# GAMES-UChile/mogptk

Hardware: AMD Instinct MI355X
Metric: log-marginal-likelihood+grad evals/sec, MOSM C=4 N=8192; 1/2/4/8 GPU (higher is better)
Workload: dtype f64

## Files before the change

### mogptk_amd/csrc/exact.hip

```cpp
#include "mogp_model.h"
#include <cstdlib>
#include <limits>

using namespace mogp;

static int wait_stream(hipStream_t st) {
    static const bool spin = !(std::getenv("MOGP_SPIN_WAIT") && std::atoi(std::getenv("MOGP_SPIN_WAIT")) == 0);
    if (!spin) { HIP_TRY(hipStreamSynchronize(st)); return 0; }
    for (;;) {
        const hipError_t e = hipStreamQuery(st);
        if (e == hipSuccess) return 0;
        if (e != hipErrorNotReady) return hip_fail(e, "hipStreamQuery", __FILE__, __LINE__);
    }
}

static hipEvent_t prof_event(mogp_model* m, int idx) {
    if (!m->profiling) return nullptr;
    while ((int)m->ev.size() <= idx) { hipEvent_t e; if (hipEventCreate(&e) != hipSuccess) return nullptr; m->ev.push_back(e); }
    return m->ev[idx];
}

static void kinv_block_ranges(mogp_model* m) {
    std::vector<int> blk;
    tile_blocks(m->sx.off, m->C, blk);
    const int nblk = (int)blk.size() / 2, D = m->D;
    m->blk_cen.assign((size_t)D * nblk, 0.0); m->blk_half.assign((size_t)D * nblk, 0.0);
    for (int b = 0; b < nblk; ++b)
        for (int d = 0; d < D; ++d) {
            const double* x = m->sx.xs.data() + (size_t)d * m->sx.Mpad + blk[2 * b];
            double lo = x[0], hi = x[0];
            for (int i = 1; i < blk[2 * b + 1]; ++i) { lo = std::fmin(lo, x[i]); hi = std::fmax(hi, x[i]); }
            m->blk_cen[(size_t)d * nblk + b] = 0.5 * (lo + hi); m->blk_half[(size_t)d * nblk + b] = 0.5 * (hi - lo);
        }
}

static int kinv_plan(mogp_model* m, bool want) {
    static const bool full = std::getenv("MOGP_FULL_INVERSE") && std::atoi(std::getenv("MOGP_FULL_INVERSE")) != 0;
    m->kinv_sparse = false; m->kinv_fraction = 1.0;
    if (!want || full || m->sh_n > 1 || m->tiles.empty() || m->radial) return 0;
    const int nb = m->nb, D = m->D, T = m->T, W = m->Wt;
    const int64_t ld = m->Npad;
    if (m->blk_cen.empty()) kinv_block_ranges(m);
    const int nblk = (int)(m->blk_cen.size() / std::max(D, 1));
    std::vector<char> need((size_t)nb * nb, 0);
    for (const GTile& t : m->tiles) {
        const double* tab = m->table.data() + (size_t)t.pair * T * W;
        bool read = false;
        for (int k = 0; k < T && !read; ++k) {
            const double* row = tab + (size_t)k * W;
            double emin = 0.0;
            for (int d = 0; d < D; ++d) {
                const double sd = (m->blk_cen[(size_t)d * nblk + t.rb] - m->blk_cen[(size_t)d * nblk + t.cb]) + row[2 + 2 * D + d];
                const double mu = std::fmax(0.0, std::fabs(sd) - m->blk_half[(size_t)d * nblk + t.rb] - m->blk_half[(size_t)d * nblk + t.cb]);
                emin += row[2 + d] * mu * mu;
            }
            read = !(0.5 * emin > 52.0);
        }
        if (!read) continue;
        const int i0 = t.r0 / MOGP_TILE, i1 = (t.r0 + t.nr - 1) / MOGP_TILE, j0 = t.c0 / MOGP_TILE, j1 = (t.c0 + t.nc - 1) / MOGP_TILE;
        for (int i = i0; i <= i1; ++i) for (int j = j0; j <= j1; ++j) if (j <= i) need[(size_t)i * nb + j] = 1;
    }
    for (int i = 0; i < nb; ++i) need[(size_t)i * nb + i] = 1;
    std::vector<GemmTask> acc, lau;
    std::vector<int> prefix(nb + 1, 0);
    for (int i = 0; i < nb; ++i) {
        for (int j = 0; j <= i; ++j) {
            if (!need[(size_t)i * nb + j]) continue;
            GemmTask a;
            a.a_off = (int64_t)i * MOGP_TILE; a.b_off = (int64_t)j * MOGP_TILE; a.c_off = (int64_t)i * MOGP_TILE * ld + (int64_t)j * MOGP_TILE;
            a.kt = 4 * MOGP_TILE / 16; a.pad = i + 1;
            acc.push_back(a);
            GemmTask l;
            l.a_off = (int64_t)i * MOGP_TILE * ld + (int64_t)i * MOGP_TILE; l.b_off = (int64_t)i * MOGP_TILE * ld + (int64_t)j * MOGP_TILE;
            l.c_off = a.c_off; l.kt = (int)((ld - (int64_t)i * MOGP_TILE) / 16); l.pad = 0;
            lau.push_back(l);
        }
        prefix[i + 1] = (int)acc.size();
    }
    const double frac = (double)acc.size() / ((double)nb * (nb + 1) / 2);
    m->kinv_fraction = frac;
    if (frac > 0.85) return 0;
    const bool same = acc.size() == m->kinv_acc_tasks.size() && (acc.empty() || std::memcmp(acc.data(), m->kinv_acc_tasks.data(), acc.size() * sizeof(GemmTask)) == 0);
    if (!same || m->d_kinv_acc.n < acc.size()) {
        int rc;
        if ((rc = m->d_kinv_acc.ensure(std::max<size_t>(acc.size(), 1)))) return rc;
        if ((rc = m->d_kinv_lauum.ensure(std::max<size_t>(lau.size(), 1)))) return rc;
        HIP_TRY(hipMemcpyAsync(m->d_kinv_acc.p, acc.data(), acc.size() * sizeof(GemmTask), hipMemcpyHostToDevice, m->st));
        HIP_TRY(hipMemcpyAsync(m->d_kinv_lauum.p, lau.data(), lau.size() * sizeof(GemmTask), hipMemcpyHostToDevice, m->st));
        HIP_TRY(hipStreamSynchronize(m->st));
        m->kinv_acc_tasks.swap(acc); m->kinv_lauum_tasks.swap(lau);
    }
    m->kinv_prefix.swap(prefix);
    m->kinv_sparse = true;
    return 0;
}

static int pin_ensure(mogp_model* m, size_t n) {
    if (n <= m->h_pin_n) return 0;
    if (m->h_pin) { hipError_t e = hipHostFree(m->h_pin); (void)e; m->h_pin = nullptr; m->h_pin_n = 0; }
    HIP_TRY(hipHostMalloc(reinterpret_cast<void**>(&m->h_pin), n * sizeof(double), hipHostMallocDefault));
    m->h_pin_n = n;
    return 0;
}
struct PinLayout {
    size_t nzz, logdet = 0, zz, info, moments, diagG, pivots, total, score, mu, var, fold_info;
    PinLayout(int nb, int64_t Npad, int C, int T, int Wt) : nzz((size_t)((Npad + 3) / 4)) {
        zz = (size_t)nb; info = zz + nzz; moments = info + 1; diagG = moments + (size_t)(C * (C + 1) / 2) * T * Wt; pivots = diagG + C; total = pivots + 2;
        score = total; mu = score + 1; var = mu + (size_t)Npad; fold_info = var + (size_t)Npad;
    }
    explicit PinLayout(const mogp_model* m) : PinLayout(m->nb, m->Npad, m->C, m->T, m->Wt) {}
    size_t held_out_total(bool folds) const { return fold_info + (folds ? 1 : 0); }
};

namespace mogp {
int begin_call(mogp_model* m, int64_t* info, bool one_gpu) {
    m->mean_w = nullptr;
    if (int rc = use_device(m->ctx)) return rc;
    if (info) *info = 0;
    if (one_gpu) one_gpu_call(m);
    return 0;
}

int exact_begin(mogp_model* m, const double* noise_var, const double* data_var, double jitter, GramArgs& ga, double& jabs) {
    const int C = m->C;
    const int64_t N = m->N, Npad = m->Npad;
    if (m->T <= 0) return fail(MOGP_EINVAL, "mogp_model_set_terms must be called before an evaluation");
    if (!noise_var) return fail(MOGP_EINVAL, "noise_var is null");
    { int r__ = ensure_system(m); if (r__) return r__; }
    m->have_W = m->have_Kinv = false;
    m->gemm_ev_used = 0; m->gemm_launches = 0; m->gemm_flops = 0.0;

    double dsum = 0.0;
    if (!m->point_diag.empty()) {
        for (int c = 0; c < C; ++c)
            for (int k = m->sx.off[c]; k < m->sx.off[c + 1]; ++k) dsum += m->point_diag[k] + noise_var[c];
    } else if (m->radial && m->point_kinds) {
        dsum = table_diag_points(m, m->sx);
        for (int c = 0; c < C; ++c) dsum += (double)(m->sx.off[c + 1] - m->sx.off[c]) * noise_var[c];
    } else
    for (int c = 0; c < C; ++c) dsum += (double)(m->sx.off[c + 1] - m->sx.off[c]) * (table_diag(m, c) + noise_var[c]);
    if (data_var) {
        std::vector<double> dv(Npad, 0.0);
        for (int64_t pos = 0; pos < N; ++pos) { dv[pos] = data_var[m->sx.perm[pos]]; dsum += dv[pos]; }
        { int r__ = m->d_dvar.ensure(Npad); if (r__) return r__; }
        HIP_TRY(hipMemcpyAsync(m->d_dvar.p, dv.data(), Npad * sizeof(double), hipMemcpyHostToDevice, m->st));
    }
    jabs = jitter * dsum / (double)N;
    HIP_TRY(hipMemcpyAsync(m->d_noise.p, noise_var, C * sizeof(double), hipMemcpyHostToDevice, m->st));
    static const unsigned long long big = std::numeric_limits<unsigned long long>::max();
    HIP_TRY(hipMemcpyAsync(m->d_info.p, &big, sizeof(big), hipMemcpyHostToDevice, m->st));
    int rc;
    if ((rc = mark(m, 0))) return rc;
    ga = GramArgs{};
    ga.tiles = m->d_tiles.p; ga.xr = m->d_x.p; ga.xc = m->d_x.p; ga.ldxr = ga.ldxc = Npad; ga.nrows = ga.ncols = N;
    if ((rc = m->ph_xx.prepare(m->sx.off, m->sx.off, C, m->T, Npad, Npad, m->st, ga.ph))) return rc;
    ga.table = m->d_table.p; ga.T = m->T; ga.D = m->D; ga.C = C; ga.W = m->Wt;
    ga.out = m->k.A.p; ga.ldo = Npad; ga.noise = m->d_noise.p; ga.dvar = data_var ? m->d_dvar.p : nullptr;
    ga.jitter_abs = jabs; ga.mirror = 0;
    if (m->radial) { ga.kind = m->d_kind.p; ga.shape = m->d_shape.p; }
    return 0;
}
}

namespace mogp { int chain_fallback(mogp_model* m) {
    if (m->flow_ran) {
        m->no_flow = true; m->flow_ran = false;
        m->flow_timeouts++;
        m->flow_retry_at = m->n_fact + m->flow_backoff;
        m->flow_backoff = std::min(m->flow_backoff * 4, 16384);
        for (hipStream_t q : {m->st, m->st2, m->st3, m->st4, m->ctx->st5, m->st_priv}) if (q) HIP_TRY(hipStreamSynchronize(q));
        static bool said_flow = false;
        if (!said_flow) {
            said_flow = true;
            unsigned code = 0;
            if (m->k.flow_flags.p && m->k.flow_cur && m->k.flow_cur->base_err > 0) { hipError_t e = hipMemcpy(&code, m->k.flow_flags.p + m->k.flow_cur->base_err, sizeof(code), hipMemcpyDeviceToHost); (void)e; }
            fprintf(stderr, "mogp: the dataflow kernel timed out (wait 0x%x; GPU shared with another process?); using the stream schedule for the next %d evaluations (said once)\n", code, (int)(m->flow_retry_at - m->n_fact));
            fprintf(stderr, "mogp: the host enqueued that evaluation in %.0f us (longest so far %.0f us)\n", m->flow_enqueue_us, m->flow_enqueue_us_max);
        }
        if (std::getenv("MOGP_FLOW_DEBUG")) { fprintf(stderr, "mogp: dataflow time-out %d of this model\n", m->flow_timeouts); flow_debug_dump(m); }
        return 0;
    }
    if (m->no_chain) return fail(MOGP_EHIP, "chain kernel: a hand-off timed out although the model is on the launch-per-step chain");
    m->no_chain = true;
    for (hipStream_t q : {m->st, m->st2, m->st3, m->st4, m->ctx->st5, m->st_priv}) if (q) HIP_TRY(hipStreamSynchronize(q));
    static bool said = false;
    if (!said) { said = true; fprintf(stderr, "mogp: the persistent chain kernel timed out (GPU shared with another process?); using the launch-per-step chain\n"); }
    return 0;
} }

template <typename F> static int retry_on_streams(mogp_model* m, int rc, F again) {
    if (rc != MOGP_RETRY_NO_CHAIN) return rc;
    if ((rc = chain_fallback(m))) return rc;
    return again();
}

namespace mogp { int report_not_pd(unsigned long long hinfo, int64_t* info) {
    if (info) *info = (int64_t)hinfo;
    return fail(MOGP_ENOTPD, "linalg.cholesky: The factorization could not be completed because the input is not "
                             "positive-definite (the leading minor of order " + std::to_string(hinfo) + " is not positive-definite).");
} }

static int factorize_finish(mogp_model* m, const GramArgs& ga, double* lml, int64_t* info) {
    const int64_t N = m->N, Npad = m->Npad;
    const PinLayout pl(m);
    const unsigned long long big = std::numeric_limits<unsigned long long>::max();
    unsigned long long hinfo = 0;
    std::memcpy(&hinfo, m->h_pin + pl.info, sizeof(hinfo));
    int rc;
    if (hinfo == MOGP_INFO_CHAIN_TIMEOUT) return MOGP_RETRY_NO_CHAIN;
    if (hinfo != big) {
        if (info) *info = (int64_t)hinfo;
        int flag = 0;
        HIP_TRY(hipMemsetAsync(m->d_flag.p, 0, sizeof(int), m->st));
        if ((rc = launch_gram(ga, (int)m->tiles.size(), m->st, m->radial ? m->gate_kinds : 0))) return rc;
        if ((rc = launch_nonfinite_scan(m->k.A.p, Npad, N, m->d_flag.p, m->st))) return rc;
        HIP_TRY(hipMemcpyAsync(&flag, m->d_flag.p, sizeof(int), hipMemcpyDeviceToHost, m->st));
        HIP_TRY(hipStreamSynchronize(m->st));
        if (flag & 1) return fail(MOGP_ENONFINITE, "linalg.cholesky: kernel matrix has NaNs!");
        if (flag & 2) return fail(MOGP_ENONFINITE, "linalg.cholesky: kernel matrix has infinities!");
        return report_not_pd(hinfo, info);
    }
    m->pivot_min = m->h_pin[pl.pivots]; m->pivot_max = m->h_pin[pl.pivots + 1];
    double logdet = 0.0, zz = 0.0;
    for (int i = 0; i < m->nb; ++i) logdet += m->h_pin[pl.logdet + i];
    for (size_t i = 0; i < pl.nzz; ++i) zz += m->h_pin[pl.zz + i];
    if (lml) *lml = -0.5 * (double)N * std::log(2.0 * M_PI) - logdet - 0.5 * zz;
    m->have_W = !m->factor_only && !m->accurate_ran;
    return 0;
}

struct FactorPlan {
    enum Schedule { Fused, Phases, FactorOnly } schedule = Phases;
    bool defer = false;
    bool want_inverse = true;
    bool refine = false;
};

static int factorize(mogp_model* m, const double* noise_var, const double* data_var, double jitter, const FactorPlan& plan,
                     double* lml, double* jitter_abs, int64_t* info, GramArgs* ga_out = nullptr) {
    const bool fuse_inverse = plan.schedule == FactorPlan::Fused, factor_only = plan.schedule == FactorPlan::FactorOnly;
    const int64_t N = m->N, Npad = m->Npad;
    GramArgs ga{};
    double jabs = 0.0;
    int rc = exact_begin(m, noise_var, data_var, jitter, ga, jabs);
    if (rc) return rc;
    if (jitter_abs) *jitter_abs = jabs;
    m->n_fact++;
    if (m->no_flow && m->n_fact >= m->flow_retry_at) m->no_flow = false;
    m->factor_only = factor_only;
    ga.ev0 = prof_event(m, 7); ga.ev1 = prof_event(m, 8);
    m->strip.attach(ga);
    const bool split = fuse_inverse && flow_enabled(m, m->k) && !m->tiles_head.empty() && !m->tiles_tail.empty() && m->st2;
    if (split) {
        GramArgs gh = ga, gt = ga;
        gh.tiles = m->d_tiles_head.p; m->strip_head.attach(gh); gh.ev1 = nullptr;
        gt.tiles = m->d_tiles_tail.p; m->strip_tail.attach(gt); gt.ev0 = nullptr; gt.phases_ready = 1;
        if ((rc = launch_gram(gh, (int)m->tiles_head.size(), m->st, m->radial ? m->gate_kinds : 0))) return rc;
        if ((rc = launch_pad_identity(m->k.A.p, Npad, N, Npad, m->st))) return rc;
        if (!m->gram_ev) HIP_TRY(hipEventCreateWithFlags(&m->gram_ev, hipEventDisableTiming));
        HIP_TRY(hipEventRecord(m->gram_ev, m->st));
        HIP_TRY(hipStreamWaitEvent(m->st2, m->gram_ev, 0));
        if ((rc = launch_gram(gt, (int)m->tiles_tail.size(), m->st2, m->radial ? m->gate_kinds : 0))) return rc;
        if (!m->gram_tail_ev) HIP_TRY(hipEventCreateWithFlags(&m->gram_tail_ev, hipEventDisableTiming));
        HIP_TRY(hipEventRecord(m->gram_tail_ev, m->st2));
        m->k.tail_ready = m->gram_tail_ev;
    } else {
        if ((rc = launch_gram(ga, (int)m->tiles.size(), m->st, m->radial ? m->gate_kinds : 0))) return rc;
        if ((rc = launch_pad_identity(m->k.A.p, Npad, N, Npad, m->st))) return rc;
    }
    ga.ev0 = ga.ev1 = nullptr;
    if ((rc = mark(m, 1))) return rc;

    const PinLayout pl(m);
    if ((rc = pin_ensure(m, pl.total))) return rc;
    if ((rc = m->d_pivots.ensure(2))) return rc;
    if (m->accurate && (rc = m->acc_rhs.ensure((size_t)Npad * MOGP_TILE))) return rc;
    m->k.flow_used = false;
    m->flow_ran = false;
    m->k.want_vec = fuse_inverse;
    m->k.vec_y = m->d_y.p; m->k.vec_z = m->d_z.p; m->k.vec_zz = m->d_zz.p; m->k.vec_part = m->d_alpha.p + Npad;
    const bool accurate = m->accurate && plan.schedule == FactorPlan::Phases;
    m->accurate_ran = accurate;
    m->k.keep_L = m->k.refine_panels = plan.refine || accurate;
    if (factor_only && m->rhs_job && flow_enabled(m, m->k)) rc = spd_potri_flow(m, m->k, m->rhs_job);
    else rc = fuse_inverse ? spd_potri_fused(m, m->k) : spd_potrf(m, m->k);
    m->k.keep_L = m->k.refine_panels = false;
    m->k.want_vec = false; m->k.tail_ready = nullptr;
    if (rc) return rc;
    if ((rc = mark(m, 2))) return rc;
    if (accurate) {
        hipStream_t ms = (plan.want_inverse && m->st2u) ? m->st2u : m->st;
        if (plan.want_inverse) {
            if (ms != m->st) {
                while ((int)m->k.inv_ev.size() < 4) { hipEvent_t e; HIP_TRY(hipEventCreateWithFlags(&e, hipEventDisableTiming)); m->k.inv_ev.push_back(e); }
                HIP_TRY(hipEventRecord(m->k.inv_ev[0], m->st));
                HIP_TRY(hipStreamWaitEvent(ms, m->k.inv_ev[0], 0));
            }
            if ((rc = m->k.Wm.ensure((size_t)Npad * Npad))) return rc;
            HIP_TRY(hipMemsetAsync(m->k.Wm.p, 0, (size_t)Npad * Npad * sizeof(double), ms));
            if ((rc = launch_add_diag(m->k.Wm.p, Npad, Npad, 1.0, ms))) return rc;
            if ((rc = trsm_lower(m, m->k.A.p, Npad, m->nb, m->k.Wm.p, Npad, Npad, false, ms, true))) return rc;
            GemmArgs g{};
            g.A = m->k.Wm.p; g.lda = Npad; g.a_kmajor = 1; g.B = m->k.Wm.p; g.ldb = Npad; g.b_kmajor = 1;
            g.C = m->k.B.p; g.ldc = Npad; g.alpha = 1.0; g.beta = 0.0; g.mode = GM_LAUUM; g.mt = g.nt = m->nb; g.K = (int)Npad;
            if ((rc = gemm_call(m, g, gemm_flops(g, nullptr), ms))) return rc;
            if (ms != m->st) HIP_TRY(hipEventRecord(m->k.inv_ev[1], ms));
        }
        HIP_TRY(hipMemsetAsync(m->acc_rhs.p, 0, (size_t)Npad * MOGP_TILE * sizeof(double), m->st));
        if ((rc = launch_copy2d(m->acc_rhs.p, MOGP_TILE, m->d_y.p, 1, Npad, 1, 1.0, m->st))) return rc;
        if ((rc = trsm_lower(m, m->k.A.p, Npad, m->nb, m->acc_rhs.p, MOGP_TILE, MOGP_TILE, false))) return rc;
        if ((rc = launch_copy2d(m->d_z.p, 1, m->acc_rhs.p, MOGP_TILE, Npad, 1, 1.0, m->st))) return rc;
        HIP_TRY(hipMemsetAsync(m->d_zz.p, 0, pl.nzz * sizeof(double), m->st));
        if ((rc = launch_gemv_rows(m->d_z.p, Npad, 1, Npad, m->d_z.p, m->d_zz.p, m->st))) return rc;
        if ((rc = trsm_lower(m, m->k.A.p, Npad, m->nb, m->acc_rhs.p, MOGP_TILE, MOGP_TILE, true))) return rc;
        if ((rc = launch_copy2d(m->d_alpha.p, 1, m->acc_rhs.p, MOGP_TILE, Npad, 1, 1.0, m->st))) return rc;
        if (plan.want_inverse && ms != m->st) HIP_TRY(hipStreamWaitEvent(m->st, m->k.inv_ev[1], 0));
    } else if (plan.schedule == FactorPlan::Phases && (rc = spd_trtri(m, m->k))) return rc;
    if ((rc = mark(m, 3))) return rc;

    if (factor_only) {
        HIP_TRY(hipMemsetAsync(m->d_zz.p, 0, pl.nzz * sizeof(double), m->st));
    } else if (!accurate) {
        const double* Wp = fuse_inverse ? m->k.Wm.p : m->k.A.p;
        m->w_in_Wm = fuse_inverse;
        if (fuse_inverse && m->k.flow_used && m->k.vec_done) {
            if ((rc = launch_flow_alpha_sum(m->k, m->d_alpha.p, m->st))) return rc;
        } else {
            if ((rc = launch_trmv_lower(Wp, Npad, Npad, m->d_y.p, m->d_z.p, m->d_zz.p, m->st))) return rc;
            if ((rc = launch_trmv_lower_t(Wp, Npad, Npad, m->d_z.p, m->d_alpha.p, m->st))) return rc;
        }
    }
    if (fuse_inverse && (rc = spd_potri_fused_finish(m, m->k))) return rc;
    if ((rc = mark(m, 4))) return rc;
    {
        static const bool fault = std::getenv("MOGP_FLOW_FAULT") && std::atoi(std::getenv("MOGP_FLOW_FAULT")) != 0;
        static const unsigned long long timed_out = MOGP_INFO_CHAIN_TIMEOUT;
        if (fault && m->k.flow_used) HIP_TRY(hipMemcpyAsync(m->d_info.p, &timed_out, sizeof(timed_out), hipMemcpyHostToDevice, m->st));
    }

    const int nzz = (int)pl.nzz;
    if ((rc = launch_pivot_range(m->k.invd.p, N, m->d_pivots.p, m->st))) return rc;
    HIP_TRY(hipMemcpyAsync(m->h_pin + pl.pivots, m->d_pivots.p, 2 * sizeof(double), hipMemcpyDeviceToHost, m->st));
    HIP_TRY(hipMemcpyAsync(m->h_pin + pl.logdet, m->k.logdet.p, m->nb * sizeof(double), hipMemcpyDeviceToHost, m->st));
    constexpr int zz_piece = 2048;
    for (int o = 0; o < nzz; o += zz_piece)
        HIP_TRY(hipMemcpyAsync(m->h_pin + pl.zz + o, m->d_zz.p + o, std::min(zz_piece, nzz - o) * sizeof(double), hipMemcpyDeviceToHost, m->st));
    HIP_TRY(hipMemcpyAsync(m->h_pin + pl.info, m->d_info.p, sizeof(unsigned long long), hipMemcpyDeviceToHost, m->st));
    if (ga_out) *ga_out = ga;
    if (plan.defer) return 0;
    HIP_TRY(hipStreamSynchronize(m->st));
    return factorize_finish(m, ga, lml, info);
}

namespace mogp { void collect_timing(mogp_model* m, int last_mark) {
    if (!m->profiling) return;
    auto el = [&](int a, int b) { float t = 0.f; if (hipEventElapsedTime(&t, m->ev[a], m->ev[b]) != hipSuccess) t = 0.f; return (double)t; };
    std::fill(m->ms, m->ms + MOGP_ST_COUNT, 0.0);
    m->ms[MOGP_ST_GRAM] = el(0, 1);
    m->ms[MOGP_ST_POTRF] = el(1, 2);
    m->ms[MOGP_ST_TRTRI] = el(2, 3);
    m->ms[MOGP_ST_SOLVE] = el(3, 4);
    if (last_mark >= 6) { m->ms[MOGP_ST_LAUUM] = el(4, 5); m->ms[MOGP_ST_MOMENTS] = el(5, 6); }
    m->ms[MOGP_ST_TOTAL] = el(0, last_mark);
    if ((int)m->ev.size() > 8) m->ms[MOGP_ST_GRAM_KERNEL] = el(7, 8);
    if (last_mark >= 6 && (int)m->ev.size() > 10) m->ms[MOGP_ST_MOMENT_KERNEL] = el(9, 10);
    double gsum = 0.0;
    for (size_t i = 0; i + 1 < m->gemm_ev_used; i += 2) {
        float t = 0.f;
        if (hipEventElapsedTime(&t, m->gemm_ev[i], m->gemm_ev[i + 1]) == hipSuccess) gsum += t;
    }
    m->ms[MOGP_ST_GEMM_KERNEL] = gsum;
}

int moment_pass_device(mogp_model* m, const double* kinv, double ksign) {
    const int C = m->C, D = m->D, W = m->Wt, T = m->T, P = C * (C + 1) / 2;
    const int64_t Npad = m->Npad;
    const int rm = m->sh_n > 1 ? m->sh_n : 0;
    const bool own = m->sh_n > 1 && m->own_n == m->sh_n && m->own_rank == m->sh_rank;
    int rc;
    MomentArgs ma{};
    ma.tiles = own ? m->d_tiles_own.p : m->d_tiles.p; ma.ntiles = (int)(own ? m->tiles_own.size() : m->tiles.size());
    ma.x = m->d_x.p; ma.ldx = Npad; ma.nrows = ma.ncols = m->N;
    if ((rc = m->ph_xx.prepare(m->sx.off, m->sx.off, C, T, Npad, Npad, m->st, ma.ph))) return rc;
    ma.table = m->d_table.p; ma.T = T; ma.D = D; ma.C = C; ma.W = W; ma.kinv = kinv; ma.kinv_sign = ksign; ma.ld = Npad; ma.alpha = m->d_alpha.p;
    ma.row_mod = rm; ma.row_rem = m->sh_rank;
    if (m->radial) { ma.kind = m->d_kind.p; ma.shape = m->d_shape.p; }
    ma.partial = m->d_partial.p;
    ma.phases_ready = 1;
    ma.ev0 = prof_event(m, 9); ma.ev1 = prof_event(m, 10);
    if ((rc = launch_moments(ma, m->st, m->radial ? m->gate_kinds : 0))) return rc;
    if ((rc = launch_moment_reduce(m->d_partial.p, own ? m->d_pair_start_own.p : m->d_pair_start.p, P, T, W, D, m->d_moments.p, m->st))) return rc;
    if ((rc = launch_diagG(kinv, Npad, m->d_alpha.p, m->d_chan_off.p, C, m->d_diagG.p, m->st, ksign, rm, m->sh_rank))) return rc;
    if ((rc = mean_grad_enqueue(m, m->d_alpha.p, -1.0))) return rc;
    return mark(m, 6);
}

int moment_pass(mogp_model* m, const double* kinv, double ksign, double* moments, double* diagG) {
    const int C = m->C, W = m->Wt, T = m->T, P = C * (C + 1) / 2;
    int rc;
    if ((rc = moment_pass_device(m, kinv, ksign))) return rc;
    HIP_TRY(hipMemcpyAsync(moments, m->d_moments.p, (size_t)P * T * W * sizeof(double), hipMemcpyDeviceToHost, m->st));
    HIP_TRY(hipMemcpyAsync(diagG, m->d_diagG.p, C * sizeof(double), hipMemcpyDeviceToHost, m->st));
    HIP_TRY(hipStreamSynchronize(m->st));
    return 0;
}

int test_side(mogp_model* m, int64_t S, const double* Xs, const double* kss_diag, int64_t extra_rows, hipStream_t st, TestSide& ts, GramArgs& ga, int R, bool point_diag) {
    const int C = m->C, D = m->D;
    const int64_t Npad = m->Npad;
    SortedX& ss = ts.ss;
    int rc;
    if ((rc = sort_inputs(Xs, S, D, C, MOGP_TILE, ss))) return rc;
    const int64_t Spad = ts.Spad = ss.Mpad, Srow = R * Spad + extra_rows;
    std::vector<GTile> pt;
    build_rect_tiles(ss.off, m->sx.off, C, pt);
    ts.ntiles = (int)pt.size();
    if ((rc = m->d_xs.ensure((size_t)D * Spad))) return rc;
    if ((rc = m->d_Ksf.ensure((size_t)Srow * Npad))) return rc;
    if ((rc = m->d_mu.ensure((size_t)R * Spad))) return rc;
    if ((rc = m->d_kdiag.ensure((size_t)R * Spad))) return rc;
    if ((rc = m->d_ptiles.ensure(std::max<size_t>(pt.size(), 1)))) return rc;
    std::vector<double> kd((size_t)R * Spad, 0.0);
    const bool per_point = point_diag || m->Wt > 2 + 3 * D || (m->radial && m->point_kinds);
    for (int r = 0; r < R; ++r) {
        const double* kr = kss_diag + (size_t)r * (per_point ? S : C);
        for (int c = 0; c < C; ++c)
            for (int pos = ss.off[c]; pos < ss.off[c + 1]; ++pos) kd[(size_t)r * Spad + pos] = per_point ? kr[ss.perm[pos]] : kr[c];
    }
    HIP_TRY(hipMemcpyAsync(m->d_xs.p, ss.xs.data(), (size_t)D * Spad * sizeof(double), hipMemcpyHostToDevice, st));
    HIP_TRY(hipMemcpyAsync(m->d_kdiag.p, kd.data(), (size_t)R * Spad * sizeof(double), hipMemcpyHostToDevice, st));
    HIP_TRY(hipMemcpyAsync(m->d_ptiles.p, pt.data(), pt.size() * sizeof(GTile), hipMemcpyHostToDevice, st));
    HIP_TRY(hipMemsetAsync(m->d_Ksf.p, 0, (size_t)Srow * Npad * sizeof(double), st));
    ga = GramArgs{};
    ga.tiles = m->d_ptiles.p; ga.xr = m->d_xs.p; ga.ldxr = Spad; ga.xc = m->d_x.p; ga.ldxc = Npad; ga.nrows = S; ga.ncols = m->N;
    if ((rc = m->ph_sx.prepare(ss.off, m->sx.off, C, m->T, Spad, Npad, st, ga.ph))) return rc;
    ga.table = m->d_table.p; ga.T = m->T; ga.D = D; ga.C = C; ga.W = m->Wt; ga.out = m->d_Ksf.p; ga.ldo = Npad;
    ga.noise = nullptr; ga.dvar = nullptr; ga.jitter_abs = 0.0; ga.mirror = 0;
    if (m->radial) { ga.kind = m->d_kind.p; ga.shape = m->d_shape.p; }
    return 0;
}
}

static const std::string& grad_path_env() {
    static const std::string grad_path = []() { const char* e = std::getenv("MOGP_GRAD_PATH"); return std::string(e ? e : ""); }();
    return grad_path;
}

static int enqueue_inverse(mogp_model* m, const double* noise_var, const double* data_var, double jitter, bool inverse, bool banded,
                           double* lml, double* jitter_abs, int64_t* info, GramArgs& ga) {
    const std::string& grad_path = grad_path_env();
    int rc;
    if ((rc = ensure_system(m))) return rc;
    if ((rc = kinv_plan(m, inverse && banded && !m->accurate))) return rc;
    const int fused_max = flow_enabled(m, m->k) ? 112 : 80;
    const bool fused = inverse && !m->accurate && (grad_path == "fused" || (grad_path != "phases" && m->nb <= fused_max));
    FactorPlan plan;
    plan.schedule = fused ? FactorPlan::Fused : FactorPlan::Phases; plan.defer = inverse; plan.want_inverse = inverse;
    if ((rc = factorize(m, noise_var, data_var, jitter, plan, lml, jitter_abs, info, &ga))) return rc;
    if (!inverse) return 0;
    if (!fused && !m->accurate_ran && (rc = spd_lauum(m, m->k))) return rc;
    return mark(m, 5);
}

static int grad_enqueue(mogp_model* m, const PinLayout& pl) {
    HIP_TRY(hipMemcpyAsync(m->h_pin + pl.moments, m->d_moments.p, (pl.diagG - pl.moments) * sizeof(double), hipMemcpyDeviceToHost, m->st));
    HIP_TRY(hipMemcpyAsync(m->h_pin + pl.diagG, m->d_diagG.p, m->C * sizeof(double), hipMemcpyDeviceToHost, m->st));
    return 0;
}
static void grad_finish(mogp_model* m, const double* diagG, double* trG) {
    double tr = 0.0;
    for (int c = 0; c < m->C; ++c) tr += diagG[c];
    *trG = tr;
    mean_grad_collect(m);
    collect_timing(m, 6);
}
static void grad_collect(mogp_model* m, const PinLayout& pl, double* moments, double* diagG, double* trG) {
    std::memcpy(moments, m->h_pin + pl.moments, (pl.diagG - pl.moments) * sizeof(double));
    std::memcpy(diagG, m->h_pin + pl.diagG, m->C * sizeof(double));
    grad_finish(m, diagG, trG);
}

static int held_out_eval(mogp_model* m, const double* noise_var, const double* data_var, double jitter, int flags, const int32_t* fold, int64_t nfolds,
                         double* score, double* mu, double* var, double* moments, double* diagG, double* trG, double* jitter_abs, int64_t* info) {
    const bool grad = (flags & MOGP_EVAL_GRAD) != 0, folds = fold != nullptr;
    int rc;
    if ((rc = begin_call(m, info, true))) return rc;
    auto again = [&]() {
        return folds ? mogp_exact_cv(m, noise_var, data_var, jitter, flags, fold, nfolds, score, mu, var, moments, diagG, trG, jitter_abs, info)
                     : mogp_exact_loo(m, noise_var, data_var, jitter, flags, score, mu, var, moments, diagG, trG, jitter_abs, info);
    };
    if ((rc = ensure_system(m))) return rc;
    if ((rc = folds ? cv_workspace(m, fold, nfolds, grad) : loo_workspace(m, grad))) return rc;
    const PinLayout pl(m);
    if ((rc = pin_ensure(m, pl.held_out_total(folds)))) return rc;
    const int64_t N = m->N, Npad = m->Npad;
    GramArgs ga{};
    if ((rc = enqueue_inverse(m, noise_var, data_var, jitter, true, false, nullptr, jitter_abs, info, ga))) return retry_on_streams(m, rc, again);
    if ((rc = held_out_points(m, m->k.B.p, folds, grad))) return rc;
    if (grad) {
        m->have_W = false;
        if ((rc = held_out_adjoint(m, m->k.B.p, m->k.A.p, folds))) return rc;
        if ((rc = loo_moment_pass(m))) return rc;
        if ((rc = grad_enqueue(m, pl))) return rc;
    }
    const double* v = m->loo.vec.p;
    double* h = m->h_pin;
    HIP_TRY(hipMemcpyAsync(h + pl.score, v + LOO_SUM * Npad, sizeof(double), hipMemcpyDeviceToHost, m->st));
    HIP_TRY(hipMemcpyAsync(h + pl.mu, v + LOO_MU * Npad, N * sizeof(double), hipMemcpyDeviceToHost, m->st));
    HIP_TRY(hipMemcpyAsync(h + pl.var, v + LOO_VAR * Npad, N * sizeof(double), hipMemcpyDeviceToHost, m->st));
    if (folds) HIP_TRY(hipMemcpyAsync(h + pl.fold_info, m->d_info.p, sizeof(unsigned long long), hipMemcpyDeviceToHost, m->st));
    if ((rc = wait_stream(m->st))) return rc;
    if ((rc = factorize_finish(m, ga, nullptr, info))) return retry_on_streams(m, rc, again);
    if (grad) m->have_W = false;
    if (folds) {
        unsigned long long finfo = 0;
        std::memcpy(&finfo, h + pl.fold_info, sizeof(finfo));
        if (finfo != std::numeric_limits<unsigned long long>::max()) {
            if (info) *info = (int64_t)(finfo - 1) / 256;
            return fail(MOGP_ENOTPD, "mogp_exact_cv: the block of Kj^-1 over fold " + std::to_string((finfo - 1) / 256) + " is not positive definite (pivot " +
                                     std::to_string((finfo - 1) % 256 + 1) + " of its factorisation): Kj is too ill-conditioned for this fold");
        }
        for (int64_t pos = 0; pos < N; ++pos)
            if (m->cv.label[pos] < 0) h[pl.mu + pos] = h[pl.var + pos] = std::numeric_limits<double>::quiet_NaN();
    }
    *score = h[pl.score];
    scatter_by_perm(m->sx, h + pl.mu, mu);
    scatter_by_perm(m->sx, h + pl.var, var);
    m->have_Kinv = true;
    m->kinv_in_A = false;
    if (!grad) { collect_timing(m, 5); return MOGP_OK; }
    grad_collect(m, pl, moments, diagG, trG);
    return MOGP_OK;
}

extern "C" {

int mogp_exact_eval(mogp_model* m, const double* noise_var, const double* data_var, double jitter, int flags,
                    double* lml, double* moments, double* diagG, double* trG, double* jitter_abs, int64_t* info) {
    if (!m) return fail(MOGP_EINVAL, "mogp_exact_eval: model is null");
    int rc;
    if ((rc = begin_call(m, info, true))) return rc;
    const std::string& grad_path = grad_path_env();
    const bool sweep = grad_path == "sweep" && (flags & MOGP_EVAL_GRAD);
    const bool grad = (flags & MOGP_EVAL_GRAD) != 0;
    GramArgs ga{};
    auto again = [&]() { return mogp_exact_eval(m, noise_var, data_var, jitter, flags, lml, moments, diagG, trG, jitter_abs, info); };
    if (grad && (!moments || !diagG || !trG)) return fail(MOGP_EINVAL, "mogp_exact_eval: gradient outputs are null");
    if (sweep) {
        if ((rc = ensure_system(m))) return rc;
        if ((rc = kinv_plan(m, false))) return rc;
        m->pivot_min = m->pivot_max = 0.0;
        if ((rc = eval_sweep(m, noise_var, data_var, jitter, lml, jitter_abs, info))) return retry_on_streams(m, rc, again);
    }
    else if ((rc = enqueue_inverse(m, noise_var, data_var, jitter, grad, true, lml, jitter_abs, info, ga))) return retry_on_streams(m, rc, again);
    if (!grad) { collect_timing(m, 4); return MOGP_OK; }

    const double* kinv = sweep ? m->k.A.p : m->k.B.p;
    const double ksign = sweep ? -1.0 : 1.0;
    const PinLayout pl(m);
    if (sweep && (rc = mark(m, 5))) return rc;
    if (sweep) {
        if ((rc = moment_pass(m, kinv, ksign, moments, diagG))) return rc;
    } else {
        if ((rc = moment_pass_device(m, kinv, ksign))) return rc;
        if ((rc = grad_enqueue(m, pl))) return rc;
        if ((rc = wait_stream(m->st))) return rc;
        if ((rc = factorize_finish(m, ga, lml, info))) return retry_on_streams(m, rc, again);
    }
    m->have_Kinv = true;
    m->kinv_in_A = sweep;
    if (sweep) grad_finish(m, diagG, trG);
    else grad_collect(m, pl, moments, diagG, trG);
    return MOGP_OK;
}

int mogp_exact_loo(mogp_model* m, const double* noise_var, const double* data_var, double jitter, int flags,
                   double* loo, double* mu, double* var, double* moments, double* diagG, double* trG, double* jitter_abs, int64_t* info) {
    if (!m) return fail(MOGP_EINVAL, "mogp_exact_loo: model is null");
    if (!loo || !mu || !var) return fail(MOGP_EINVAL, "mogp_exact_loo: loo, mu or var is null");
    if ((flags & MOGP_EVAL_GRAD) && (!moments || !diagG || !trG)) return fail(MOGP_EINVAL, "mogp_exact_loo: gradient outputs are null");
    return held_out_eval(m, noise_var, data_var, jitter, flags, nullptr, 0, loo, mu, var, moments, diagG, trG, jitter_abs, info);
}

int mogp_exact_cv(mogp_model* m, const double* noise_var, const double* data_var, double jitter, int flags, const int32_t* fold, int64_t nfolds,
                  double* cv, double* mu, double* var, double* moments, double* diagG, double* trG, double* jitter_abs, int64_t* info) {
    if (!m) return fail(MOGP_EINVAL, "mogp_exact_cv: model is null");
    if (!fold || !cv || !mu || !var) return fail(MOGP_EINVAL, "mogp_exact_cv: fold, cv, mu or var is null");
    if ((flags & MOGP_EVAL_GRAD) && (!moments || !diagG || !trG)) return fail(MOGP_EINVAL, "mogp_exact_cv: gradient outputs are null");
    return held_out_eval(m, noise_var, data_var, jitter, flags, fold, nfolds, cv, mu, var, moments, diagG, trG, jitter_abs, info);
}

int mogp_model_loo_bytes(mogp_model* m, int64_t* bytes) {
    if (!m || !bytes) return fail(MOGP_EINVAL, "mogp_model_loo_bytes: bad argument");
    *bytes = (int64_t)((m->loo.G.n + m->loo.vec.n) * sizeof(double) + cv_bytes(m));
    return MOGP_OK;
}

struct RowBlocks { int R; const double* tables; const char* psi_same; bool jacobian; };
static int predict_core(mogp_model* m, const double* noise_var, const double* data_var, double jitter,
                        const double* kss_diag, int64_t S, const double* Xs, int full,
                        double* mu, double* var, int64_t* info, const double* mean_w, const RowBlocks* blocks = nullptr) {
    int rc;
    if ((rc = begin_call(m, info, true))) return rc;
    const int R = blocks ? blocks->R : 1;
    const bool jac = blocks && blocks->jacobian;
    const RowBlocks* parts = blocks && blocks->tables ? blocks : nullptr;
    if (jac && mean_w) return fail(MOGP_EINVAL, "predict_core: Jacobian row blocks have no mean weights");
    const size_t tab_n = (size_t)m->C * m->C * m->T * m->Wt;
    const int C = m->C, nb = m->nb;
    const int64_t Npad = m->Npad;
    hipStream_t sv = m->st3 ? m->st3 : m->st;
    for (auto& e : m->pred_ev) if (!e) HIP_TRY(hipEventCreateWithFlags(&e, hipEventDisableTiming));
    HIP_TRY(hipEventRecord(m->pred_ev[0], m->st));
    HIP_TRY(hipStreamWaitEvent(sv, m->pred_ev[0], 0));
    TestSide ts; GramArgs ga{};
    if ((rc = test_side(m, S, Xs, kss_diag, MOGP_TILE, sv, ts, ga, R, jac))) return rc;
    const SortedX& ss = ts.ss;
    const int64_t Spad = ts.Spad, Sall = R * Spad, Srow = Sall + MOGP_TILE;
    if ((rc = m->d_Vt.ensure((size_t)Srow * Npad))) return rc;
    if ((rc = m->d_var.ensure(Sall))) return rc;
    if (parts) {
        if ((rc = m->d_parts.ensure(R * tab_n))) return rc;
        HIP_TRY(hipMemcpyAsync(m->d_parts.p, parts->tables, R * tab_n * sizeof(double), hipMemcpyHostToDevice, sv));
    }
    HIP_TRY(hipMemcpyAsync(m->d_Ksf.p + Sall * Npad, m->d_y.p, Npad * sizeof(double), hipMemcpyDeviceToDevice, sv));
    if (jac) {
        if ((rc = launch_gram_dx(ga, ts.ntiles, Spad * Npad, sv))) return rc;
    } else
    for (int p = 0; p < R; ++p) {
        GramArgs gp = ga;
        if (parts) { gp.table = m->d_parts.p + p * tab_n; gp.out = m->d_Ksf.p + (int64_t)p * Spad * Npad; gp.phases_ready = p > 0 && parts->psi_same[p]; }
        if ((rc = launch_gram(gp, ts.ntiles, sv, m->radial ? m->gate_kinds : 0))) return rc;
    }
    if (mean_w) {
        std::vector<double> hw(Npad, 0.0);
        for (int64_t pos = 0; pos < m->N; ++pos) hw[pos] = mean_w[m->sx.perm[pos]];
        if ((rc = m->d_z.ensure(Npad))) return rc;
        HIP_TRY(dev_upload(m->d_z.p, hw.data(), Npad * sizeof(double)));
        if ((rc = launch_gemv_rows(m->d_Ksf.p, Npad, Spad, Npad, m->d_z.p, m->d_mu.p, sv))) return rc;
    }

    if ((rc = ensure_system(m))) return rc;
    const char* fpe = std::getenv("MOGP_FLOW_PREDICT");
    int fp_lo = 48, fp_hi = 160;
    if (fpe && std::strchr(fpe, ':')) { fp_lo = std::atoi(fpe); fp_hi = std::atoi(std::strchr(fpe, ':') + 1); }
    else if (fpe) fp_hi = std::atoi(fpe);
    const bool acc = m->accurate;
    const bool as_flow = !acc && fp_hi > 0 && nb >= fp_lo && nb <= fp_hi && Srow / MOGP_TILE <= 4096 && flow_enabled(m, m->k) && !m->kinv_sparse;
    FlowRhs job{m->d_Ksf.p, m->d_Vt.p, (int)(Srow / MOGP_TILE), nullptr};
    if (as_flow) {
        HIP_TRY(hipEventRecord(m->pred_ev[1], sv));
        job.ready = m->pred_ev[1];
        m->rhs_job = &job;
    }
    GramArgs gaK{};
    FactorPlan plan;
    plan.schedule = FactorPlan::FactorOnly; plan.defer = true; plan.refine = acc;
    rc = factorize(m, noise_var, data_var, jitter, plan, nullptr, nullptr, info, &gaK);
    m->rhs_job = nullptr;
    if (rc) return rc;
    const bool flowed = as_flow && m->k.flow_used;

    if (!flowed) {
        constexpr int OB = MOGP_OUTER, KD = OB * MOGP_TILE;
        const int nouter = (nb + OB - 1) / OB, mt = (int)(Srow / MOGP_TILE);
        Spd& w = m->k;
        if (w.Wd.n < (size_t)nouter * KD * KD) {
            if ((rc = w.Wd.ensure((size_t)nouter * KD * KD))) return rc;
            HIP_TRY(hipMemsetAsync(w.Wd.p, 0, (size_t)nouter * KD * KD * sizeof(double), sv));
        }
        for (int kb = 0; kb < nouter; ++kb) {
            const int k0 = kb * OB, nk = std::min(OB, nb - k0), k1 = k0 + nk, rem = nb - k1;
            const int64_t c0 = (int64_t)k0 * MOGP_TILE;
            HIP_TRY(hipStreamWaitEvent(sv, w.sync_ev[2 * kb], 0));
            double* Wk = w.Wd.p + (int64_t)kb * KD * KD;
            if ((rc = launch_wkk(w.A.p + c0 * (Npad + 1), Npad, w.invd.p + (int64_t)k0 * MOGP_TILE * MOGP_TILE, nk, Wk, KD, sv))) return rc;
            GemmArgs g{};
            g.A = m->d_Ksf.p + c0; g.lda = Npad; g.a_kmajor = 0; g.B = Wk; g.ldb = KD; g.b_kmajor = 0;
            g.C = m->d_Vt.p + c0; g.ldc = Npad; g.alpha = 1.0; g.beta = 0.0;
            g.mode = GM_KHI_J; g.small = 1; g.mt = 2 * mt; g.nt = nk; g.K = nk * MOGP_TILE;
            if ((rc = gemm_call(m, g, gemm_flops(g, nullptr), sv))) return rc;
            if (acc) {
                GemmArgs r1 = g;
                r1.A = m->d_Vt.p + c0; r1.B = w.A.p + c0 * (Npad + 1); r1.ldb = Npad; r1.C = m->d_Ksf.p + c0; r1.alpha = -1.0; r1.beta = 1.0;
                if ((rc = gemm_call(m, r1, gemm_flops(r1, nullptr), sv))) return rc;
                GemmArgs r2 = g;
                r2.A = m->d_Ksf.p + c0; r2.C = m->d_Vt.p + c0; r2.alpha = 1.0; r2.beta = 1.0;
                if ((rc = gemm_call(m, r2, gemm_flops(r2, nullptr), sv))) return rc;
            }
            if (rem > 0) {
                GemmArgs u{};
                u.A = m->d_Vt.p + c0; u.lda = Npad; u.a_kmajor = 0;
                u.B = w.A.p + (int64_t)k1 * MOGP_TILE * Npad + c0; u.ldb = Npad; u.b_kmajor = 0;
                u.C = m->d_Ksf.p + (int64_t)k1 * MOGP_TILE; u.ldc = Npad; u.alpha = -1.0; u.beta = 1.0;
                u.mode = GM_RECT; u.mt = mt; u.nt = rem; u.K = nk * MOGP_TILE;
                if ((rc = gemm_call(m, u, gemm_flops(u, nullptr), sv))) return rc;
            }
        }
        HIP_TRY(hipEventRecord(m->pred_ev[1], sv));
        HIP_TRY(hipStreamWaitEvent(m->st, m->pred_ev[1], 0));
    }
    if (!mean_w && (rc = launch_gemv_rows(m->d_Vt.p, Npad, Sall, Npad, m->d_Vt.p + Sall * Npad, m->d_mu.p, m->st))) return rc;

    std::vector<double> hmu(Sall);
    HIP_TRY(hipMemcpyAsync(hmu.data(), m->d_mu.p, Sall * sizeof(double), hipMemcpyDeviceToHost, m->st));
    auto again = [&]() { return predict_core(m, noise_var, data_var, jitter, kss_diag, S, Xs, full, mu, var, info, mean_w, blocks); };
    if (!full) {
        if ((rc = launch_row_sqnorm_sub(m->d_Vt.p, Npad, Sall, Npad, m->d_kdiag.p, m->d_var.p, m->st))) return rc;
        std::vector<double> hv(Sall);
        HIP_TRY(hipMemcpyAsync(hv.data(), m->d_var.p, Sall * sizeof(double), hipMemcpyDeviceToHost, m->st));
        if ((rc = mark(m, 5))) return rc;
        HIP_TRY(hipStreamSynchronize(m->st));
        if ((rc = factorize_finish(m, gaK, nullptr, info))) return retry_on_streams(m, rc, again);
        collect_timing(m, 5);
        for (int p = 0; p < R; ++p) { scatter_by_perm(ss, hmu.data() + p * Spad, mu + p * S); scatter_by_perm(ss, hv.data() + p * Spad, var + p * S); }
        return MOGP_OK;
    }
    std::vector<GTile> st_tiles;
    std::vector<int> ps;
// ... 154 lines not shown
```

### mogptk_amd/csrc/flow.hip

```cpp
#include "mogp_model.h"
#include <unistd.h>
#include <chrono>
#include <set>

#include <cstdio>
#include <cstdlib>

namespace mogp {

typedef double d4_t __attribute__((ext_vector_type(4)));
typedef double d2_t __attribute__((ext_vector_type(2)));

#define FL_BK 16
#define FL_ROWK 18
#define FL_WTM 4
#define FL_WTN 2
#define FL_NWJ 4
#define FL_NWI 2
#define FL_NT 512
#define FL_COLK (MOGP_TILE + 16)
#define FL_OPER (MOGP_TILE * FL_ROWK)
#define FL_LDS_DOUBLES (2 * 2 * FL_OPER)
#define FL_LDS_BYTES (FL_LDS_DOUBLES * 8 + 16 + 3 * 64 * 4 + 16)
static_assert(MOGP_TILE * FL_ROWK == 16 * FL_COLK, "one LDS operand slot serves both layouts");
// ... 559 lines not shown
    auto xs = [&](int b, int i, int c) {
        FlowTask t = mk(b, PH_XS, 0 | 4, KB * (c + 1));
        opA(t, BUF_WT, i, k0(b)); opB(t, BUF_WM, k0(b) + c, k0(b)); opC(t, BUF_B, i, k0(b) + c);
        dep(t, CH(b), chain_wgs(b));
        dep(t, TR(i, b), (unsigned)(nk(b) * b));
        t.sig[0] = XN(b, i);
        tiles_k += t.kt;
        return t;
    };
    auto tu = [&](int b, int i, int j) {
        FlowTask t = mk(b, PH_TU, 0 | 8, KB * nk(b));
        opA(t, BUF_B, i, k0(b)); opB(t, BUF_L, j, k0(b)); opC(t, BUF_WT, i, j);
        dep(t, XN(b, i), (unsigned)nk(b));
        dep(t, PN(b, j), pn_need(b, j));
        dep(t, TS(i, j), (unsigned)b);
        t.sig[0] = TS(i, j); t.sig[1] = TR(i, blk(j));
        tiles_k += t.kt;
        return t;
    };
    std::vector<FlowTask> rrest;

    p.chain.resize(no);
    for (int b = 0; b < no; ++b) {
        const int a0 = k1(b), a1 = std::min(nb, a0 + ob), a2 = std::min(nb, a1 + ob);
        FlowPlan::Chain& c = p.chain[b];
        c = FlowPlan::Chain{};
        c.done_idx = CH(b); c.expect = chain_wgs(b);
        c.t1_nwait = 0;
        for (int i = a0; i < a1 && b > 0; ++i) { c.t1_widx[c.t1_nwait] = R(i, b); c.t1_wval[c.t1_nwait] = (uint32_t)(nk(b) * b); ++c.t1_nwait; }
        c.t1_sig_base = PN(b, a0); c.t1_sig_per_row = 2u * (uint32_t)nk(b);
        if (a1 > a0) { const int n1 = a1 - a0; c.t2_widx = DG(b + 1); c.t2_wval = (uint32_t)(n1 * (n1 + 1) / 2 * b); }
        if (replay) {
            for (int i = a0; i < a1; ++i) for (int cc = 0; cc < nk(b); ++cc) q[Q_LOOK2].push_back(panel(b, i, cc, true));
            for (int i = a0; i < a1; ++i) for (int j = a0; j <= i; ++j) q[Q_LOOK2].push_back(update(b, i, j, true));
        }
        for (int i = a1; i < a2; ++i) for (int cc = 0; cc < nk(b); ++cc) q[Q_LOOK2].push_back(panel(b, i, cc, true));
        for (int i = a1; i < a2; ++i) for (int j = a0; j < a1; ++j) q[Q_LOOK2].push_back(update(b, i, j, true));
        for (int i = a1; i < a2; ++i) for (int j = a1; j <= i; ++j) q[Q_LOOK2].push_back(update(b, i, j, true));
        for (int i = a2; i < nb; ++i) for (int cc = 0; cc < nk(b); ++cc) q[Q_SEMI].push_back(panel(b, i, cc, false));
        for (int i = a2; i < nb; ++i) for (int j = a0; j < a2; ++j) q[Q_SEMI].push_back(update(b, i, j, false));
        for (int i = a2; i < nb; ++i) for (int j = a2; j <= i; ++j) trail[b].push_back(update(b, i, j, false));
        if (rhs_nt > 0) {
            for (int i = 0; i < rhs_nt; ++i) for (int cc = 0; cc < nk(b); ++cc) q[Q_INVCRIT].push_back(xs(b, i, cc));
            for (int i = 0; i < rhs_nt; ++i) for (int j = a0; j < a1; ++j) q[Q_INVCRIT].push_back(tu(b, i, j));
            for (int i = 0; i < rhs_nt; ++i) for (int j = a1; j < nb; ++j) rrest.push_back(tu(b, i, j));
            continue;
        }
        for (int j = 0; j < k0(b); ++j) for (int ti = 0; ti < nk(b); ++ti) q[Q_INVCRIT].push_back(t6(b, ti, j));
        for (int i = a0; i < a1; ++i) for (int cc = 0; cc < nk(b); ++cc) q[Q_INVCRIT].push_back(t7(b, i, cc));
        for (int i = a0; i < a1; ++i) for (int j = 0; j < k0(b); ++j) q[Q_INVCRIT].push_back(t8(b, i, j));
        for (int bs = 0; bs + 2 <= b; ++bs) {
            for (int i = k0(b); i < k1(b); ++i) for (int cc = 0; cc < nk(bs); ++cc) into[b].push_back(t7(bs, i, cc));
            for (int i = k0(b); i < k1(b); ++i) for (int j = 0; j < k0(bs); ++j) into[b].push_back(t8(bs, i, j));
        }
        for (int i = 0; i < k1(b); ++i) for (int j = 0; j <= i; ++j) acc.push_back(t9(b, i, j));
        for (int i = k0(b); i < k1(b); ++i) {
            FlowTask t = mk(b, PH_ZROW, 32, 1);
            t.ar = (uint16_t)i;
            dep(t, CH(b), chain_wgs(b));
            dep(t, WR(b), (unsigned)(nk(b) * k0(b)));
            t.sig[0] = ZR(b);
            vec.push_back(t);
        }
        for (int jg = 0; jg * 4 < k1(b); ++jg) {
            FlowTask t = mk(b, PH_APART, 32 | 1, nk(b));
            t.ar = (uint16_t)k0(b); t.br = (uint16_t)b; t.ac = (uint16_t)jg;
            dep(t, ZR(b), (unsigned)nk(b));
            vec.push_back(t);
        }
    }
    std::vector<const std::vector<FlowTask>*> order = {&q[Q_LOOK2], &q[Q_SEMI], &q[Q_INVCRIT], &vec};
    for (int d = 2; d < no + 3; ++d) {
        if (d < no && !into[d].empty()) order.push_back(&into[d]);
        if (d - 3 >= 0 && d - 3 < no && !trail[d - 3].empty()) order.push_back(&trail[d - 3]);
    }
    order.push_back(rhs_nt > 0 ? &rrest : &acc);
    for (size_t k = order.size(); k-- > 1;) if (order[k]->empty()) order.erase(order.begin() + (long)k);
    if ((int)order.size() > FLOW_MAXQ) {
        std::vector<FlowTask> rest;
        std::vector<const std::vector<FlowTask>*> tail(order.begin() + (FLOW_MAXQ - 2), order.end() - 1);
        for (auto* v : tail) rest.insert(rest.end(), v->begin(), v->end());
        std::stable_sort(rest.begin(), rest.end(), [](const FlowTask& x, const FlowTask& y) { return x.key < y.key; });
        p.folded = rest;
        order.erase(order.begin() + (FLOW_MAXQ - 2), order.end() - 1);
        order.insert(order.end() - 1, &p.folded);
    }
    p.nq = (int)order.size();
    for (int qi = 0; qi < p.nq; ++qi) {
        p.qbase[qi] = (int)p.tasks.size(); p.qsize[qi] = (int)order[qi]->size();
        p.tasks.insert(p.tasks.end(), order[qi]->begin(), order[qi]->end());
    }
    p.flops = 2.0 * MOGP_TILE * MOGP_TILE * FL_BK * tiles_k;
}

__global__ void k_alpha_sum(const double* __restrict__ part, int64_t npad, int no, int ob, double* __restrict__ out) {
    const int64_t col = (int64_t)blockIdx.x * blockDim.x + threadIdx.x;
    if (col >= npad) return;
    double s = 0.0;
    for (int r = (int)(col / MOGP_TILE) / ob; r < no; ++r) s += part[(int64_t)r * npad + col];
    out[col] = s;
}
int launch_flow_alpha_sum(const Spd& w, double* alpha, hipStream_t st) {
    const FlowPlan& p = w.flow_cur ? *w.flow_cur : w.flow;
    hipLaunchKernelGGL(k_alpha_sum, dim3((unsigned)((w.Npad + 255) / 256)), dim3(256), 0, st, w.vec_part, w.Npad, p.nouter, p.ob, alpha);
    HIP_TRY(hipGetLastError());
    return 0;
}

bool flow_enabled(const mogp_model* m, const Spd& w) {
    const char* eo = std::getenv("MOGP_FLOW");
    const char* en = std::getenv("MOGP_FLOW_MIN");
    const int on = eo ? std::atoi(eo) : 1, nmin = en ? std::atoi(en) : 8;
    if (!on || (m->no_flow && m->n_fact < m->flow_retry_at) || !chain_enabled(m) || !m->ctx->st_priv) return false;
    if (m->kinv_sparse && &w == &m->k) return false;
    return w.nb >= nmin && w.nb <= 0xfff0;
}

int spd_potri_flow(mogp_model* m, Spd& w, const FlowRhs* rhs) {
    const int nb = w.nb, ob = 4;
    const int64_t ld = w.Npad;
    int rc;
    const auto host_t0 = std::chrono::steady_clock::now();
    hipStream_t crit = m->st, priv = m->st_priv, bulk = m->st2;
    if (w.Wm.n < (size_t)ld * ld) {
        if ((rc = w.Wm.ensure((size_t)ld * ld))) return rc;
        HIP_TRY(hipMemsetAsync(w.Wm.p, 0, (size_t)ld * ld * sizeof(double), crit));
    }
    if ((rc = w.Lm.ensure((size_t)ld * ld))) return rc;
    if (!rhs && (rc = w.Wt.ensure((size_t)ld * ld))) return rc;
    const bool replay = m->replay_flow && !rhs && &w == &m->k;
    FlowPlan& plan = rhs ? w.flow_rhs : replay ? w.flow_replay : w.flow;
    DevBuf<FlowTask>& d_tasks = rhs ? w.flow_tasks_rhs : replay ? w.flow_tasks_replay : w.flow_tasks;
    DevBuf<int>& d_qmeta = rhs ? w.flow_qmeta_rhs : replay ? w.flow_qmeta_replay : w.flow_qmeta;
    const int rhs_nt = rhs ? rhs->nt : 0;
    if (plan.nb != nb || plan.ob != ob || plan.rhs_nt != rhs_nt) {
        flow_build(nb, ob, plan, rhs_nt, replay);
        if ((rc = d_tasks.ensure(plan.tasks.size()))) return rc;
        if ((rc = d_qmeta.ensure(2 * FLOW_MAXQ))) return rc;
        int qm[2 * FLOW_MAXQ] = {0};
        for (int q = 0; q < plan.nq; ++q) { qm[2 * q] = plan.qbase[q]; qm[2 * q + 1] = plan.qsize[q]; }
        HIP_TRY(hipStreamSynchronize(crit));
        HIP_TRY(dev_upload(d_tasks.p, plan.tasks.data(), plan.tasks.size() * sizeof(FlowTask)));
        HIP_TRY(dev_upload(d_qmeta.p, qm, sizeof(qm)));
    }
    if ((rc = w.flow_flags.ensure((size_t)plan.nflags))) return rc;
    if (!w.flow_diag.p) {
        if ((rc = w.flow_diag.ensure(FLOW_DIAG_WORDS))) return rc;
        HIP_TRY(hipMemsetAsync(w.flow_diag.p, 0, FLOW_DIAG_WORDS * sizeof(unsigned), crit));
    }
    w.flow_cur = &plan;
    const FlowPlan& p = plan;
    const int nouter = p.nouter;
    if ((rc = w.chain_flags.ensure((size_t)(nouter + 1) * MOGP_CHAIN_FLAGS))) return rc;
    HIP_TRY(hipMemsetAsync(w.chain_flags.p, 0, (size_t)(nouter + 1) * MOGP_CHAIN_FLAGS * sizeof(unsigned), crit));
    HIP_TRY(hipMemsetAsync(w.flow_flags.p, 0, (size_t)p.nflags * sizeof(unsigned), crit));
    if (replay) {
        std::vector<unsigned> preset((size_t)p.nflags, 0u);
        for (const FlowPlan::Chain& c : p.chain) preset[c.done_idx] = c.expect;
        HIP_TRY(hipMemcpyAsync(w.flow_flags.p, preset.data(), preset.size() * sizeof(unsigned), hipMemcpyHostToDevice, crit));
        HIP_TRY(hipStreamSynchronize(crit));
    }
    if (!rhs && w.want_vec && w.vec_zz) HIP_TRY(hipMemsetAsync(w.vec_zz, 0, (size_t)((ld + 3) / 4) * sizeof(double), crit));
    static const bool want_trace = std::getenv("MOGP_FLOW_TRACE") && std::atoi(std::getenv("MOGP_FLOW_TRACE")) != 0;
    if (want_trace) {
        if ((rc = w.flow_trace.ensure(FLOW_TRACE_W * p.tasks.size() + 4 * (size_t)nouter))) return rc;
        HIP_TRY(hipMemsetAsync(w.flow_trace.p, 0, w.flow_trace.n * sizeof(unsigned long long), crit));
    }
    while ((int)w.inv_ev.size() < 4) {
        hipEvent_t e;
        HIP_TRY(hipEventCreateWithFlags(&e, hipEventDisableTiming));
        w.inv_ev.push_back(e);
    }
    hipEvent_t start = w.inv_ev[0], e_flow = w.inv_ev[1], e_chain = w.inv_ev[2];
    HIP_TRY(hipEventRecord(start, crit));
    HIP_TRY(hipStreamWaitEvent(bulk, start, 0));
    HIP_TRY(hipStreamWaitEvent(priv, start, 0));

    static std::atomic<unsigned long long> attr_done{0ull};
    static std::atomic<unsigned long long> attr_done_dbg{0ull};
    { int r__ = set_max_dynamic_lds(reinterpret_cast<const void*>(k_flow<false>), FL_LDS_BYTES, attr_done); if (r__) return r__; }
    { int r__ = set_max_dynamic_lds(reinterpret_cast<const void*>(k_flow<true>), FL_LDS_BYTES, attr_done_dbg); if (r__) return r__; }
    static const int wg_per_cu = std::getenv("MOGP_FLOW_WGS") ? std::max(1, std::atoi(std::getenv("MOGP_FLOW_WGS"))) : 2;
    int cus = (m->ctx->ncu > 0 ? m->ctx->ncu : 256) - m->ctx->ncu_reserved;
    { static const int drop = std::getenv("MOGP_FLOW_DROP_CUS") ? std::atoi(std::getenv("MOGP_FLOW_DROP_CUS")) : 16;
      if (drop > 0 && drop < cus) cus -= drop; }
    FlowArgs g{};
    g.bA = w.A.p; g.bL = w.Lm.p; g.bWt = rhs ? rhs->T : w.Wt.p; g.bWm = w.Wm.p; g.bB = rhs ? rhs->X : w.B.p; g.ld = ld;
    g.tasks = d_tasks.p; g.qmeta = d_qmeta.p; g.flags = w.flow_flags.p;
    g.nq = p.nq; g.ncas = FLOW_NCAS; g.base_heads = p.base_heads; g.base_err = p.base_err; g.info = m->d_info.p;
    g.trace = want_trace ? w.flow_trace.p : nullptr;
    g.diag = w.flow_diag.p;
    static const bool want_post = std::getenv("MOGP_FLOW_DEBUG") && std::atoi(std::getenv("MOGP_FLOW_DEBUG")) != 0;
    if (want_post) {
        const size_t nwg = (size_t)wg_per_cu * ((size_t)cus + (size_t)m->ctx->ncu_reserved);
        if ((rc = w.flow_post.ensure(nwg * FLOW_POST_W))) return rc;
        HIP_TRY(hipMemsetAsync(w.flow_post.p, 0, w.flow_post.n * sizeof(unsigned), bulk));
        g.post = w.flow_post.p;
        if ((rc = w.flow_done.ensure(p.tasks.size()))) return rc;
        HIP_TRY(hipMemsetAsync(w.flow_done.p, 0, p.tasks.size(), bulk));
        g.done = w.flow_done.p;
    }
    g.npad = ld;
    { const char* e = std::getenv("MOGP_FLOW_REFILL"); g.refill = e ? std::atoi(e) : 0; }
    { const char* e = std::getenv("MOGP_FLOW_CLAIM1"); g.claim_one = e ? std::atoi(e) : 0; }
    { const char* e = std::getenv("MOGP_FLOW_NHI"); g.nhi = e ? std::atoi(e) : 0; }
    { const char* e = std::getenv("MOGP_FLOW_NAP"); g.nap_max = e ? (unsigned)std::max(0, std::atoi(e)) : 4u; }
    { const char* e = std::getenv("MOGP_FLOW_NAP_CALM"); g.nap_calm = e ? (unsigned)std::max(0, std::atoi(e)) : 0u; if (g.nap_calm < g.nap_max) g.nap_calm = g.nap_max; }
    w.vec_done = false;
    if (!rhs && w.want_vec && w.vec_y && w.vec_z && w.vec_zz && w.vec_part) {
        g.vy = w.vec_y; g.vz = w.vec_z; g.vzz = w.vec_zz; g.vpart = w.vec_part;
        w.vec_done = true;
    }
    hipEvent_t pe0 = nullptr, pe1 = nullptr;
    if (m->profiling) {
        if (m->gemm_ev_used + 2 > m->gemm_ev.size())
            for (int i = 0; i < 64; ++i) { hipEvent_t e; HIP_TRY(hipEventCreate(&e)); m->gemm_ev.push_back(e); }
        pe0 = m->gemm_ev[m->gemm_ev_used++]; pe1 = m->gemm_ev[m->gemm_ev_used++];
        HIP_TRY(hipEventRecord(pe0, bulk));
    }
    if (rhs && rhs->ready) HIP_TRY(hipStreamWaitEvent(bulk, rhs->ready, 0));
    const bool dbg_kernel = g.post != nullptr || g.trace != nullptr;
    static_assert(sizeof(FlowArgs) <= 512, "Spd::flow_args slots");
    if ((rc = w.flow_args.ensure(1024))) return rc;
    if (w.flow_args_h.size() != 2048) w.flow_args_h.assign(2048, (char)0xff);
    auto upload = [&](size_t slot, const FlowArgs& a, hipStream_t st) -> int {
        char* held = w.flow_args_h.data() + slot;
        char* fresh_ = w.flow_args_h.data() + 1024 + slot;
        std::memset(fresh_, 0, 512);
        std::memcpy(fresh_, &a, sizeof(a));
        if (std::memcmp(held, fresh_, 512) == 0) return 0;
        HIP_TRY(hipStreamSynchronize(st));
        HIP_TRY(dev_upload(w.flow_args.p + slot, fresh_, 512));
        std::memcpy(held, fresh_, 512);
        return 0;
    };
    if ((rc = upload(0, g, bulk))) return rc;
    const FlowArgs* d_g = reinterpret_cast<const FlowArgs*>(w.flow_args.p);
    FlowHot hot{};
    hot.bA = g.bA; hot.bL = g.bL; hot.bWt = g.bWt; hot.bWm = g.bWm; hot.bB = g.bB; hot.ld = g.ld; hot.tasks = g.tasks; hot.qmeta = g.qmeta; hot.flags = g.flags;
    hot.nq = g.nq; hot.ncas = g.ncas; hot.base_heads = g.base_heads; hot.base_err = g.base_err; hot.nap_max = g.nap_max; hot.nap_calm = g.nap_calm;
    if (dbg_kernel) hipLaunchKernelGGL(k_flow<true>, dim3(wg_per_cu * cus), dim3(FL_NT), FL_LDS_BYTES, bulk, d_g, hot);
    else hipLaunchKernelGGL(k_flow<false>, dim3(wg_per_cu * cus), dim3(FL_NT), FL_LDS_BYTES, bulk, d_g, hot);
    HIP_TRY(hipGetLastError());
    if (pe1) HIP_TRY(hipEventRecord(pe1, bulk));
    HIP_TRY(hipEventRecord(e_flow, bulk));
    m->gemm_launches += 1;
    m->gemm_flops += p.flops;

    unsigned* ferr = w.flow_flags.p + p.base_err;
    for (int kb = 0; kb < nouter && !replay; ++kb) {
        const int k0 = kb * ob, k1 = std::min(k0 + ob, nb), nk = k1 - k0, na = std::min(ob, nb - k1);
        const FlowPlan::Chain& pc = p.chain[kb];
        ChainFlow cf{};
        cf.done_flag = w.flow_flags.p + pc.done_idx; cf.write_through = 1;
        cf.trace = want_trace ? w.flow_trace.p + FLOW_TRACE_W * p.tasks.size() + 4 * (size_t)kb : nullptr;
        cf.diag = w.flow_diag.p;
        if ((rc = launch_chain(w.A.p, ld, k0, nk, w.invd.p, w.logdet.p, m->d_info.p, 0, w.Wm.p + (int64_t)k0 * MOGP_TILE * (ld + 1), ld,
                               w.chain_flags.p + (size_t)kb * MOGP_CHAIN_FLAGS, ferr, priv, &cf))) return rc;
        if (na <= 0) continue;
        GemmArgs t1{};
        t1.A = w.A.p + (int64_t)k1 * MOGP_TILE * ld + (int64_t)k0 * MOGP_TILE; t1.lda = ld; t1.a_kmajor = 0;
        t1.B = w.Wm.p + (int64_t)k0 * MOGP_TILE * (ld + 1); t1.ldb = ld; t1.b_kmajor = 0;
        t1.C = w.Lm.p + (int64_t)k1 * MOGP_TILE * ld + (int64_t)k0 * MOGP_TILE; t1.ldc = ld; t1.alpha = 1.0; t1.beta = 0.0;
        t1.mode = GM_KHI_J; t1.small = 1; t1.mt = 2 * na; t1.nt = nk; t1.K = nk * MOGP_TILE;
        t1.fl_flags = w.flow_flags.p; t1.fl_nwait = pc.t1_nwait;
        for (int k = 0; k < pc.t1_nwait; ++k) { t1.fl_widx[k] = pc.t1_widx[k]; t1.fl_wval[k] = pc.t1_wval[k]; }
        static const unsigned hook_spins = std::getenv("MOGP_FLOW_HOOK_SPINS") ? (unsigned)std::atoll(std::getenv("MOGP_FLOW_HOOK_SPINS")) : 0u;
        t1.fl_spins = hook_spins; t1.fl_diag = w.flow_diag.p;
        t1.fl_wt = 1; t1.fl_sig = 1; t1.fl_sig_base = pc.t1_sig_base; t1.fl_sig_shift = 1; t1.fl_err = ferr; t1.sk_info = m->d_info.p;
        if ((rc = launch_gemm(t1, priv))) return rc;
        if (kb == 0 && w.tail_ready) HIP_TRY(hipStreamWaitEvent(priv, w.tail_ready, 0));
        GemmArgs t2{};
        t2.A = t1.C; t2.lda = ld; t2.a_kmajor = 0; t2.B = t1.C; t2.ldb = ld; t2.b_kmajor = 0;
        t2.C = w.A.p + (int64_t)k1 * MOGP_TILE * (ld + 1); t2.ldc = ld; t2.alpha = -1.0; t2.beta = 1.0;
        t2.mode = GM_RECT_LOWER; t2.small = 2; t2.mt = 2 * na; t2.nt = 2 * na; t2.K = nk * MOGP_TILE;
        t2.fl_flags = w.flow_flags.p; t2.fl_nwait = pc.t2_wval ? 1 : 0; t2.fl_widx[0] = pc.t2_widx; t2.fl_wval[0] = pc.t2_wval;
        t2.fl_err = ferr; t2.sk_info = m->d_info.p; t2.fl_spins = hook_spins; t2.fl_diag = w.flow_diag.p;
        if ((rc = launch_gemm(t2, priv))) return rc;
        m->gemm_flops += gemm_flops(t1, nullptr) + gemm_flops(t2, nullptr);
    }
    static const bool tail_on = !(std::getenv("MOGP_FLOW_TAIL") && std::atoi(std::getenv("MOGP_FLOW_TAIL")) == 0);
    if (tail_on && m->ctx->ncu_reserved > 0 && !replay) {
        if (rhs && rhs->ready) HIP_TRY(hipStreamWaitEvent(priv, rhs->ready, 0));
        g.post_base = wg_per_cu * cus;
        if ((rc = upload(512, g, priv))) return rc;
        const FlowArgs* d_g2 = reinterpret_cast<const FlowArgs*>(w.flow_args.p + 512);
        if (dbg_kernel) hipLaunchKernelGGL(k_flow<true>, dim3(wg_per_cu * m->ctx->ncu_reserved), dim3(FL_NT), FL_LDS_BYTES, priv, d_g2, hot);
        else hipLaunchKernelGGL(k_flow<false>, dim3(wg_per_cu * m->ctx->ncu_reserved), dim3(FL_NT), FL_LDS_BYTES, priv, d_g2, hot);
        HIP_TRY(hipGetLastError());
    }
    HIP_TRY(hipEventRecord(e_chain, priv));
    HIP_TRY(hipStreamWaitEvent(crit, e_flow, 0));
    HIP_TRY(hipStreamWaitEvent(crit, e_chain, 0));
    w.fused_last_inv = nullptr; w.fused_last_wt = nullptr;
    w.flow_used = true;
    m->flow_ran = true;
    m->flow_enqueue_us = std::chrono::duration<double, std::micro>(std::chrono::steady_clock::now() - host_t0).count();
    m->flow_enqueue_us_max = std::max(m->flow_enqueue_us_max, m->flow_enqueue_us);
    { const char* e = std::getenv("MOGP_FLOW_DEBUG");
      if (e && std::atoi(e) == 2 && &w == &m->k) { usleep(60000); fprintf(stderr, "mogp: dataflow state 60 ms after the evaluation was enqueued\n"); flow_debug_dump(m); } }
    return 0;
}

}

namespace mogp { void flow_debug_dump(mogp_model* m) {
    if (!m->k.flow_flags.p || !m->k.flow_cur) return;
    const FlowPlan& p = *m->k.flow_cur;
    std::vector<unsigned> fl((size_t)p.nflags);
    hipError_t e = hipMemcpy(fl.data(), m->k.flow_flags.p, fl.size() * sizeof(unsigned), hipMemcpyDeviceToHost); (void)e;
    std::vector<unsigned long long> tr;
    if (m->k.flow_trace.p && m->k.flow_trace.n >= FLOW_TRACE_W * p.tasks.size()) {
        tr.resize(FLOW_TRACE_W * p.tasks.size());
        e = hipMemcpy(tr.data(), m->k.flow_trace.p, tr.size() * sizeof(unsigned long long), hipMemcpyDeviceToHost); (void)e;
    }
// ... 208 lines not shown
```

### mogptk_amd/csrc/gram.hip

```cpp
#include "mogp_internal.h"

#include <algorithm>
#include <vector>
#include <cstdlib>

#ifdef MOGP_GRAM_DEBUG
#define GRAM_DBG(a, bit) ((a).dbg & (bit))
#else
#define GRAM_DBG(a, bit) 0
#endif

namespace mogp {

typedef double d2_t __attribute__((ext_vector_type(2)));

__device__ __forceinline__ double frac_turn(double p) { return p - rint(p); }

#define GT_SKIP (-1)
#define GT_GENERAL 0
#define GT_SKIP_EXPONENT 50.0
#define GT_DEGREE(zmax) ((zmax) <= 1.19e-3 ? 4 : (zmax) <= 4.93e-3 ? 5 : (zmax) <= 0.0139 ? 6 : (zmax) <= 0.0308 ? 7 : (zmax) <= 0.0578 ? 8 : (zmax) <= 0.0968 ? 9 : \
                         (zmax) <= 0.149 ? 10 : (zmax) <= 0.2147 ? 11 : (zmax) <= 0.294 ? 12 : 14)
#define GT_DEGREE_CASES(X) X(4) X(5) X(6) X(7) X(8) X(9) X(10) X(11) X(12) X(14)

__device__ __forceinline__ double fast_exp(double x) {
    const double n = rint(x * 1.44269504088896338700e+00);
    double r = fma(-n, 6.93147180369123816490e-01, x);
    r = fma(-n, 1.90821492927058770002e-10, r);
    double p = 1.6059043836821613e-10;
    p = fma(p, r, 2.08767569878681e-09);
    p = fma(p, r, 2.505210838544172e-08);
    p = fma(p, r, 2.755731922398589e-07);
    p = fma(p, r, 2.7557319223985893e-06);
    p = fma(p, r, 2.48015873015873e-05);
    p = fma(p, r, 1.984126984126984e-04);
    p = fma(p, r, 1.388888888888889e-03);
    p = fma(p, r, 8.333333333333333e-03);
    p = fma(p, r, 4.1666666666666664e-02);
    p = fma(p, r, 1.6666666666666666e-01);
    p = fma(p, r, 0.5);
    p = fma(p, r, 1.0);
    p = fma(p, r, 1.0);
    return ldexp(p, (int)n);
}

template <int N>
__device__ __forceinline__ double exp_taylor(double z) {
    constexpr double c[15] = {1.0, 1.0, 0.5, 1.6666666666666666e-01, 4.1666666666666664e-02, 8.333333333333333e-03,
                              1.388888888888889e-03, 1.984126984126984e-04, 2.48015873015873e-05, 2.7557319223985893e-06,
                              2.755731922398589e-07, 2.505210838544172e-08, 2.08767569878681e-09, 1.6059043836821613e-10,
                              1.1470745597729725e-11};
    double p = c[N];
#pragma unroll
    for (int k = N - 1; k >= 0; --k) p = fma(p, z, c[k]);
    return p;
}

struct PhaseArgs {
    const double* x; int64_t ld; const int* off; const double* table; int T, D, C, W, role; double* cs; double* sn;
};
__global__ __launch_bounds__(256) void k_phase_table(PhaseArgs a) {
    const int64_t pt = (int64_t)blockIdx.x * 256 + threadIdx.x;
    if (pt >= a.off[a.C]) return;
    const int o = blockIdx.y, t = blockIdx.z, D = a.D, W = a.W;
    int c = 0;
    while (pt >= a.off[c + 1]) ++c;
    const int pair = a.role == 0 ? c * a.C + o : o * a.C + c;
    const double* row = a.table + ((size_t)pair * a.T + t) * W;
    double ph = a.role == 0 ? row[1] : 0.0;
    for (int d = 0; d < D; ++d) {
        const double m = row[2 + D + d], xv = a.x[(size_t)d * a.ld + pt];
        ph = a.role == 0 ? fma(m, xv + row[2 + 2 * D + d], ph) : fma(m, xv, ph);
    }
    double sn, cs;
    sincospi(2.0 * frac_turn(ph), &sn, &cs);
    const size_t idx = ((size_t)o * a.T + t) * a.ld + pt;
    a.cs[idx] = cs;
    a.sn[idx] = sn;
}

struct CentreArgs { const double* x; int64_t ld; const int* off; int C, D; double* cen; double* half; };
__global__ __launch_bounds__(64) void k_block_centres(CentreArgs a) {
    int b = blockIdx.x, c = 0;
    for (; c < a.C; ++c) {
        const int nb = (a.off[c + 1] - a.off[c] + MOGP_GT - 1) / MOGP_GT;
        if (b < nb) break;
        b -= nb;
    }
    if (c >= a.C) return;
    const int start = a.off[c] + b * MOGP_GT, n = min(MOGP_GT, a.off[c + 1] - start), lane = threadIdx.x;
    for (int d = 0; d < a.D; ++d) {
        const double v = a.x[(size_t)d * a.ld + start + (lane < n ? lane : 0)];
        double lo = v, hi = v;
#pragma unroll
        for (int off = 32; off > 0; off >>= 1) { lo = fmin(lo, __shfl_xor(lo, off, 64)); hi = fmax(hi, __shfl_xor(hi, off, 64)); }
        if (lane == 0) { a.cen[(size_t)d * a.ld + start] = 0.5 * (lo + hi); a.half[(size_t)d * a.ld + start] = 0.5 * (hi - lo); }
    }
}

size_t phase_ws_doubles(int C, int T, int64_t ldr, int64_t ldc) { return (size_t)2 * (C * T + MOGP_MAXD) * (size_t)(ldr + ldc); }

struct PhaseView {
    const double *rcs, *rsn, *ccs, *csn, *rcen, *rhalf, *ccen, *chalf;
};
__host__ __device__ static inline PhaseView phase_view(double* ws, int C, int T, int D, int64_t ldr, int64_t ldc) {
    PhaseView v;
    double* p = ws;
    v.rcs = p; p += (size_t)C * T * ldr; v.rsn = p; p += (size_t)C * T * ldr;
    v.ccs = p; p += (size_t)C * T * ldc; v.csn = p; p += (size_t)C * T * ldc;
    v.rcen = p; p += (size_t)D * ldr; v.rhalf = p; p += (size_t)D * ldr;
    v.ccen = p; p += (size_t)D * ldc; v.chalf = p;
    return v;
}

static int launch_phase_tables(const PhaseRef& ph, const double* xr, int64_t ldxr, int64_t nr, const double* xc, int64_t ldxc, int64_t nc,
                               const double* table, int T, int D, int C, int W, hipStream_t s) {
    if (!ph.ws || !ph.offr || !ph.offc) { set_error("Gram / moment launch without a phase workspace"); return -1; }
    const PhaseView v = phase_view(ph.ws, C, T, D, ldxr, ldxc);
    PhaseArgs a;
    a.table = table; a.T = T; a.D = D; a.C = C; a.W = W;
    a.x = xr; a.ld = ldxr; a.off = ph.offr; a.role = 0; a.cs = const_cast<double*>(v.rcs); a.sn = const_cast<double*>(v.rsn);
    if (nr > 0) hipLaunchKernelGGL(k_phase_table, dim3((unsigned)((nr + 255) / 256), C, T), dim3(256), 0, s, a);
    a.x = xc; a.ld = ldxc; a.off = ph.offc; a.role = 1; a.cs = const_cast<double*>(v.ccs); a.sn = const_cast<double*>(v.csn);
    if (nc > 0) hipLaunchKernelGGL(k_phase_table, dim3((unsigned)((nc + 255) / 256), C, T), dim3(256), 0, s, a);
    CentreArgs c;
    c.C = C; c.D = D;
    c.x = xr; c.ld = ldxr; c.off = ph.offr; c.cen = const_cast<double*>(v.rcen); c.half = const_cast<double*>(v.rhalf);
    if (nr > 0) hipLaunchKernelGGL(k_block_centres, dim3((unsigned)((nr + MOGP_GT - 1) / MOGP_GT + C)), dim3(64), 0, s, c);
    c.x = xc; c.ld = ldxc; c.off = ph.offc; c.cen = const_cast<double*>(v.ccen); c.half = const_cast<double*>(v.chalf);
    if (nc > 0) hipLaunchKernelGGL(k_block_centres, dim3((unsigned)((nc + MOGP_GT - 1) / MOGP_GT + C)), dim3(64), 0, s, c);
    HIP_TRY(hipGetLastError());
    return 0;
}

template <int DM>
struct TileLds {
    double cu[MOGP_TC][MOGP_GT], su[MOGP_TC][MOGP_GT], cw[MOGP_TC][MOGP_GT], sw[MOGP_TC][MOGP_GT];
    double V[MOGP_TC][DM], s[MOGP_TC][DM], M[MOGP_TC][DM], A[MOGP_TC];
    double Kp[MOGP_TC][DM];
    double L[MOGP_TC][DM], e[MOGP_TC][DM];
    int deg[MOGP_TC];
};
template <int DM>
struct TileCtx { double cr[DM], cc[DM], hr[DM], hc[DM]; };

template <int DM>
__device__ __forceinline__ void tile_centres(TileCtx<DM>& X, const GTile& tl, int D, const PhaseView& v, int64_t ldxr, int64_t ldxc) {
    for (int d = 0; d < D; ++d) {
        X.cr[d] = v.rcen[(size_t)d * ldxr + tl.r0]; X.hr[d] = v.rhalf[(size_t)d * ldxr + tl.r0];
        X.cc[d] = v.ccen[(size_t)d * ldxc + tl.c0]; X.hc[d] = v.chalf[(size_t)d * ldxc + tl.c0];
    }
}

template <int DM>
__device__ __forceinline__ void tile_context(TileCtx<DM>& X, double (&p)[4][DM], double (&q)[4][DM], const GTile& tl, int D,
                                             const PhaseView& v, const double* __restrict__ xr, int64_t ldxr,
                                             const double* __restrict__ xc, int64_t ldxc, int rg, int cg) {
    tile_centres<DM>(X, tl, D, v, ldxr, ldxc);
#pragma unroll
    for (int m = 0; m < 4; ++m)
        for (int d = 0; d < D; ++d) {
            p[m][d] = xr[(size_t)d * ldxr + tl.r0 + min(rg * 4 + m, tl.nr - 1)] - X.cr[d];
            q[m][d] = xc[(size_t)d * ldxc + tl.c0 + min(cg * 4 + m, tl.nc - 1)] - X.cc[d];
        }
}

constexpr int STAGE_ITEMS = MOGP_TC * MOGP_GT * 2 / 256;
template <int DM>
struct StageItem { double x[DM], cs, sn; };

template <int DM>
__device__ __forceinline__ void stage_item_load(StageItem<DM>& I, int which, int t, int pnt, const GTile& tl, int D, int C, int T, int t0,
                                                const PhaseView& v, const double* __restrict__ xr, int64_t ldxr,
                                                const double* __restrict__ xc, int64_t ldxc) {
    const int i = tl.pair / C, j = tl.pair - i * C;
    if (which == 0) {
        const int64_t g = tl.r0 + min(pnt, tl.nr - 1);
        const size_t k = ((size_t)j * T + t0 + t) * ldxr + g;
        I.cs = v.rcs[k]; I.sn = v.rsn[k];
        for (int d = 0; d < D; ++d) I.x[d] = xr[(size_t)d * ldxr + g];
    } else {
        const int64_t g = tl.c0 + min(pnt, tl.nc - 1);
        const size_t k = ((size_t)i * T + t0 + t) * ldxc + g;
        I.cs = v.ccs[k]; I.sn = v.csn[k];
        for (int d = 0; d < D; ++d) I.x[d] = xc[(size_t)d * ldxc + g];
    }
}

template <int DM, bool AMP, bool RAD = false, int GATE = 0, bool SPLIT = true>
__device__ __forceinline__ void stage_item_compute(TileLds<DM>& L, const StageItem<DM>& I, const TileCtx<DM>& X, const double* tab, int W,
                                                   int which, int t, int pnt, int D, int t0, const int* kinds = nullptr) {
    const double* row = tab + (size_t)(t0 + t) * W;
    const double A = row[0];
    if constexpr (RAD) {
        const int kd = kinds[t0 + t] & MOGP_KIND_MASK;
        const bool per = kd == MOGP_KIND_PERIODIC, dot = kd == MOGP_KIND_DOT;
        const int deg = (AMP && A == 0.0 && !dot) ? GT_SKIP : GT_GENERAL;
        if (pnt == 0 && which == 0) {
            L.deg[t] = deg; L.A[t] = A;
            for (int d = 0; d < D; ++d) {
                L.V[t][d] = row[2 + d]; L.M[t][d] = row[2 + D + d];
                L.s[t][d] = (X.cr[d] - X.cc[d]) + row[2 + 2 * D + d];
                L.Kp[t][d] = X.cr[d]; L.L[t][d] = X.cc[d];
            }
            L.e[t][0] = row[1];
        }
        if (deg == GT_SKIP) return;
        if (dot) return;
        if (GATE > 1 && (kd == MOGP_KIND_WDOT || kd == MOGP_KIND_WHITE)) return;
        if (GATE && kd == MOGP_KIND_GATE) {
            const double z = row[2] * (I.x[0] - row[2 + D]);
            const double e = exp(-fabs(z)), r = 1.0 / (1.0 + e);
            const double h = z >= 0.0 ? r : e * r, hc = z >= 0.0 ? e * r : r;
            if (which == 0) { L.cu[t][pnt] = (AMP ? A : 1.0) * h; L.su[t][pnt] = hc; }
            else { L.cw[t][pnt] = h; L.sw[t][pnt] = hc; }
            return;
        }
        const double f = (AMP && !per) ? A : 1.0;
        if (which == 0) { L.cu[t][pnt] = f * I.cs; L.su[t][pnt] = f * I.sn; }
        else { L.cw[t][pnt] = I.cs; L.sw[t][pnt] = I.sn; }
        return;
    }
    const bool env = W > 2 + 3 * D;
    double zmax = 0.0, es = 0.0, emin = 0.0, efac = 0.0, s[DM], V[DM], Lv[DM], er[DM], ec[DM];
    for (int d = 0; d < D; ++d) {
        V[d] = row[2 + d];
        Lv[d] = env ? row[2 + 3 * D + d] : 0.0;
        const double cn = env ? row[2 + 4 * D + d] : 0.0;
        er[d] = X.cr[d] - cn; ec[d] = X.cc[d] - cn;
        const double hr = X.hr[d], hc = X.hc[d];
        s[d] = (X.cr[d] - X.cc[d]) + row[2 + 2 * D + d];
        zmax += fabs(V[d] - 0.25 * Lv[d]) * hr * hc;
        es += V[d] * s[d] * s[d];
        const double mu = fmax(0.0, fabs(s[d]) - hr - hc);
        emin += V[d] * mu * mu;
        const double amax = 0.5 * (fabs(er[d]) + hr + fabs(ec[d]) + hc);
        efac += fabs(V[d]) * (hr * hr + hc * hc + 2.0 * (hr + hc) * fabs(s[d])) + Lv[d] * amax * amax;
    }
    int deg;
    if ((AMP && A == 0.0) || 0.5 * emin > GT_SKIP_EXPONENT) deg = GT_SKIP;
    else if (!SPLIT || !(zmax <= 0.45) || !(0.5 * es < 600.0) || !(0.5 * efac < 600.0)) deg = GT_GENERAL;
    else deg = GT_DEGREE(zmax);
    if (pnt == 0 && which == 0) {
        L.deg[t] = deg; L.A[t] = A;
        for (int d = 0; d < D; ++d) {
            L.V[t][d] = V[d]; L.s[t][d] = s[d]; L.M[t][d] = row[2 + D + d];
            L.Kp[t][d] = V[d] - 0.25 * Lv[d]; L.L[t][d] = Lv[d]; L.e[t][d] = 0.5 * (er[d] + ec[d]);
        }
    }
    if (deg == GT_SKIP) return;
    double f = 1.0;
    if (deg != GT_GENERAL) {
        double e = 0.0;
        if (which == 0) {
            for (int d = 0; d < D; ++d) {
                const double pp = I.x[d] - X.cr[d];
                e = fma(V[d], fma(pp, pp, s[d] * s[d]) + 2.0 * pp * s[d], e);
                const double pe = pp + er[d];
                e = fma(0.25 * Lv[d], pe * pe + 2.0 * ec[d] * pe, e);
            }
        } else {
            for (int d = 0; d < D; ++d) {
                const double qq = I.x[d] - X.cc[d];
                e = fma(V[d], qq * qq - 2.0 * qq * s[d], e);
                const double qe = qq + ec[d];
                e = fma(0.25 * Lv[d], qe * qe + 2.0 * qq * er[d], e);
            }
        }
        f = fast_exp(-0.5 * e);
    }
    if (which == 0) {
        if (AMP) f *= A;
        L.cu[t][pnt] = f * I.cs; L.su[t][pnt] = f * I.sn;
    } else {
        L.cw[t][pnt] = f * I.cs; L.sw[t][pnt] = f * I.sn;
    }
}

#define STAGE_MAP(tid) const int st_wave = __builtin_amdgcn_readfirstlane((tid) >> 6), st_which = st_wave & 1, st_tb = st_wave >> 1, st_pnt = (tid) & 63

template <int DM, bool AMP, bool BATCH, bool RAD = false, int GATE = 0, bool SPLIT = true>
__device__ __forceinline__ void stage_chunk(TileLds<DM>& L, const TileCtx<DM>& X, const GTile& tl, const double* tab, int W, int D,
                                            int C, int T, int t0, int nt, const PhaseView& v, const double* __restrict__ xr, int64_t ldxr,
// ... 1739 lines not shown
            const int deg = __builtin_amdgcn_readfirstlane(L.deg[t]);
            if (deg == GT_SKIP) continue;
            const double V = L.V[t][0], sft = L.s[t][0];
            double cu[2], su[2], cw[4], sw[4];
#pragma unroll
            for (int m = 0; m < 2; ++m) { cu[m] = L.cu[t][2 * rg + m]; su[m] = L.su[t][2 * rg + m]; }
#pragma unroll
            for (int n = 0; n < 4; ++n) { cw[n] = L.cw[t][4 * cg + n]; sw[n] = L.sw[t][4 * cg + n]; }
            switch (deg) {
                #define GT_CASE(N) case N: mx_term<N>(mom[t], g, p, q, V, sft, cu, su, cw, sw); break;
                GT_DEGREE_CASES(GT_CASE)
#undef GT_CASE
                default: mx_term<0>(mom[t], g, p, q, V, sft, cu, su, cw, sw); break;
            }
        }
        if (!flush) {
            if (tid < T * 5) outp[tid] = 0.0;
        } else {
#pragma unroll
            for (int t = 0; t < TT; ++t) {
                if (t >= T) break;
#pragma unroll
                for (int w = 0; w < 5; ++w) { s_red[(t * 5 + w) * MXS + tid + (tid >> 4)] = mom[t][w]; mom[t][w] = 0.0; }
            }
            asm volatile("s_waitcnt lgkmcnt(0)\n\ts_barrier" ::: "memory");
            for (int e = tid; e < T * 5 * 32; e += 512) {
                const int w = e >> 5, i = e & 31;
                const double* src = s_red + w * MXS + i * 17;
                double x = 0.0;
#pragma unroll
                for (int k = 0; k < 16; ++k) x += src[k];
#pragma unroll
                for (int off = 16; off > 0; off >>= 1) x += __shfl_xor(x, off, 64);
                if (i == 0) outp[w] = x;
            }
            asm volatile("s_waitcnt lgkmcnt(0)\n\ts_barrier" ::: "memory");
        }
        if (!more) break;
        tile = nxt;
        buf ^= 1;
    }
}

__global__ __launch_bounds__(256) void k_gz_reduce(const double* __restrict__ gzp, int nminor, int D, const int* __restrict__ blk,
                                                   double* __restrict__ out, int64_t ld) {
    const int b = blockIdx.x, pnt = threadIdx.x & 63, part = threadIdx.x >> 6;
    const int first = blk[2 * b], n = blk[2 * b + 1];
    __shared__ double red[4][MOGP_GT], redc[4][MOGP_GT];
    const double* base = gzp + (size_t)b * nminor * D * MOGP_GT;
    for (int d = 0; d < D; ++d) {
        double s = 0.0, c = 0.0;
        for (int k = part; k < nminor; k += 4) {
            const double x = base[((size_t)k * D + d) * MOGP_GT + pnt];
            const double t = s + x;
            c += fabs(s) >= fabs(x) ? (s - t) + x : (x - t) + s;
            s = t;
        }
        __syncthreads();
        red[part][pnt] = s; redc[part][pnt] = c;
        __syncthreads();
        if (part == 0 && pnt < n) {
            double hs = 0.0, hc = 0.0;
#pragma unroll
            for (int q = 0; q < 4; ++q) {
                const double x = red[q][pnt];
                const double t = hs + x;
                hc += fabs(hs) >= fabs(x) ? (hs - t) + x : (x - t) + hs;
                hs = t;
                hc += redc[q][pnt];
            }
            out[(size_t)d * ld + first + pnt] += hs + hc;
        }
    }
}

template <bool DENSE, bool ZG, bool ENV>
static int launch_moments_t(const MomentArgs& a, hipStream_t s) {
    switch (a.D) {
        case 1: hipLaunchKernelGGL((k_moments<1, DENSE, ZG, ENV>), dim3(a.ntiles), dim3(256), 0, s, a); break;
        case 2: hipLaunchKernelGGL((k_moments<2, DENSE, ZG, ENV>), dim3(a.ntiles), dim3(256), 0, s, a); break;
        case 3: hipLaunchKernelGGL((k_moments<3, DENSE, ZG, ENV>), dim3(a.ntiles), dim3(256), 0, s, a); break;
        default: hipLaunchKernelGGL((k_moments<0, DENSE, ZG, ENV>), dim3(a.ntiles), dim3(256), 0, s, a); break;
    }
    HIP_TRY(hipGetLastError());
    return 0;
}

template <bool DENSE>
static void launch_moments_radial(const MomentArgs& a, hipStream_t s, int rows) {
    if (rows == 1) {
        hipLaunchKernelGGL((k_moments<1, DENSE, false, false, true, 1>), dim3(a.ntiles), dim3(256), 0, s, a);
    } else if (rows > 1) {
        switch (a.D) {
            case 1: hipLaunchKernelGGL((k_moments<1, DENSE, false, false, true, 2>), dim3(a.ntiles), dim3(256), 0, s, a); break;
            case 2: hipLaunchKernelGGL((k_moments<2, DENSE, false, false, true, 2>), dim3(a.ntiles), dim3(256), 0, s, a); break;
            case 3: hipLaunchKernelGGL((k_moments<3, DENSE, false, false, true, 2>), dim3(a.ntiles), dim3(256), 0, s, a); break;
            default: hipLaunchKernelGGL((k_moments<0, DENSE, false, false, true, 2>), dim3(a.ntiles), dim3(256), 0, s, a); break;
        }
    } else {
        switch (a.D) {
            case 1: hipLaunchKernelGGL((k_moments<1, DENSE, false, false, true>), dim3(a.ntiles), dim3(256), 0, s, a); break;
            case 2: hipLaunchKernelGGL((k_moments<2, DENSE, false, false, true>), dim3(a.ntiles), dim3(256), 0, s, a); break;
            case 3: hipLaunchKernelGGL((k_moments<3, DENSE, false, false, true>), dim3(a.ntiles), dim3(256), 0, s, a); break;
            default: hipLaunchKernelGGL((k_moments<0, DENSE, false, false, true>), dim3(a.ntiles), dim3(256), 0, s, a); break;
        }
    }
}

int launch_moments(const MomentArgs& a0, hipStream_t s, int rows) {
    if (a0.ntiles <= 0) return 0;
    MomentArgs a = a0;
    if (a.W <= 0) a.W = 2 + 3 * a.D;
    const bool env = a.W > 2 + 3 * a.D;
    const double* xc = a.xc ? a.xc : a.x;
    const int64_t ldxc = a.xc ? a.ldxc : a.ldx;
    int rc = a.phases_ready ? 0 : launch_phase_tables(a.ph, a.x, a.ldx, a.nrows, xc, ldxc, a.xc ? a.ncols : a.nrows, a.table, a.T, a.D, a.C, a.W, s);
    if (rc) return rc;
    if (a.kind) {
        if (!a.shape) { set_error("launch_moments: kinds without shapes"); return -1; }
        if (env || (a.G != nullptr && (!a.sym || a.ru || a.gzr || a.gzc || a.xc))) { set_error("launch_moments: radial profiles take the exact mode or a dense symmetric adjoint, without an envelope"); return -1; }
        if (a.ev0) HIP_TRY(hipEventRecord(a.ev0, s));
        if (rows == 1 && a.D != 1) { set_error("launch_moments: gate rows take one input dimension"); return -1; }
        if (a.G != nullptr) launch_moments_radial<true>(a, s, rows); else launch_moments_radial<false>(a, s, rows);
        HIP_TRY(hipGetLastError());
        if (a.ev1) HIP_TRY(hipEventRecord(a.ev1, s));
        return 0;
    }
    if (a.G == nullptr) {
        if (a.ev0) HIP_TRY(hipEventRecord(a.ev0, s));
        if (!env && a.D == 1 && a.W == 5 && a.T <= 4 && a.row_mod <= 1 && a.xc == nullptr) {
            static const int ncu = []() { int dev = 0; hipDeviceProp_t pr; if (hipGetDevice(&dev) != hipSuccess || hipGetDeviceProperties(&pr, dev) != hipSuccess) return 256; return pr.multiProcessorCount; }();
            if (a.T <= 3) hipLaunchKernelGGL(k_moments_x<3>, dim3(std::min(a.ntiles, ncu)), dim3(512), 0, s, a);
            else hipLaunchKernelGGL(k_moments_x<4>, dim3(std::min(a.ntiles, ncu)), dim3(512), 0, s, a);
            HIP_TRY(hipGetLastError());
            rc = 0;
        } else
        rc = env ? launch_moments_t<false, false, true>(a, s) : launch_moments_t<false, false, false>(a, s);
        if (!rc && a.ev1) HIP_TRY(hipEventRecord(a.ev1, s));
        return rc;
    }
    if (a.gzr || a.gzc) {
        if (!a.gzp || !a.rblk || !a.cblk || a.nrb <= 0 || a.ncb <= 0) { set_error("launch_moments: the input-gradient pass needs its scratch and block tables"); return -1; }
        const size_t half = (size_t)a.nrb * a.ncb * a.D * MOGP_GT;
        HIP_TRY(hipMemsetAsync(a.gzp, 0, 2 * half * sizeof(double), s));
        if ((rc = env ? launch_moments_t<true, true, true>(a, s) : launch_moments_t<true, true, false>(a, s))) return rc;
        if (a.gzr) hipLaunchKernelGGL(k_gz_reduce, dim3(a.nrb), dim3(256), 0, s, a.gzp, a.ncb, a.D, a.rblk, a.gzr, a.ldgz);
        if (a.gzc) hipLaunchKernelGGL(k_gz_reduce, dim3(a.ncb), dim3(256), 0, s, a.gzp + half, a.nrb, a.D, a.cblk, a.gzc, a.ldgz);
        HIP_TRY(hipGetLastError());
        return 0;
    }
    return env ? launch_moments_t<true, false, true>(a, s) : launch_moments_t<true, false, false>(a, s);
}

__global__ __launch_bounds__(256) void k_moment_reduce(const double* __restrict__ partial, const int* __restrict__ pair_start,
                                                       int TW, int W, int D, int lower_pairs, double* __restrict__ out) {
    const int p = blockIdx.x, tw = blockIdx.y;
    const int b = pair_start[p], e = pair_start[p + 1];
    __shared__ double red[256];
    double s = 0.0;
    for (int t = b + threadIdx.x; t < e; t += 256) s += partial[(size_t)t * TW + tw];
    red[threadIdx.x] = s;
    __syncthreads();
    for (int off = 128; off > 0; off >>= 1) {
        if (threadIdx.x < off) red[threadIdx.x] += red[threadIdx.x + off];
        __syncthreads();
    }
    if (threadIdx.x == 0) {
        int i = (int)((sqrt(8.0 * (double)p + 1.0) - 1.0) * 0.5);
        while ((i + 1) * (i + 2) / 2 <= p) ++i;
        while (i * (i + 1) / 2 > p) --i;
        const bool diag = lower_pairs && (p - i * (i + 1) / 2) == i;
        const int w = tw % W;
        double v = red[0];
        if (diag && (w == 1 || (w >= 2 + D && w < 2 + 2 * D))) v = 0.0;
        out[(size_t)p * TW + tw] = v;
    }
}

int launch_moment_reduce(const double* partial, const int* pair_start, int npairs, int T, int W, int D, double* out, hipStream_t s, int lower_pairs) {
    hipLaunchKernelGGL(k_moment_reduce, dim3(npairs, T * W), dim3(256), 0, s, partial, pair_start, T * W, W, D, lower_pairs, out);
    HIP_TRY(hipGetLastError());
    return 0;
}

__global__ void k_diagG(const double* __restrict__ kinv, int64_t ld, const double* __restrict__ alpha,
                        const int* __restrict__ chan_off, double* __restrict__ out, double kinv_sign, int row_mod, int row_rem) {
    const int c = blockIdx.x;
    __shared__ double red[256];
    double s = 0.0;
    for (int64_t k = chan_off[c] + threadIdx.x; k < chan_off[c + 1]; k += 256)
        if (row_mod <= 1 || (int)((k / MOGP_TILE) % row_mod) == row_rem) s += 0.5 * (alpha[k] * alpha[k] - kinv_sign * kinv[k * ld + k]);
    red[threadIdx.x] = s;
    __syncthreads();
    for (int off = 128; off > 0; off >>= 1) {
        if (threadIdx.x < off) red[threadIdx.x] += red[threadIdx.x + off];
        __syncthreads();
    }
    if (threadIdx.x == 0) out[c] = red[0];
}

int launch_diagG(const double* kinv, int64_t ld, const double* alpha, const int* chan_off, int C, double* out, hipStream_t s,
                 double kinv_sign, int row_mod, int row_rem) {
    hipLaunchKernelGGL(k_diagG, dim3(C), dim3(256), 0, s, kinv, ld, alpha, chan_off, out, kinv_sign, row_mod, row_rem);
    HIP_TRY(hipGetLastError());
    return 0;
}

}
```

### mogptk_amd/csrc/mogp_api.hip

```cpp
#include "mogp_model.h"

#include <algorithm>
#include <cmath>
#include <cstring>
#include <cstdlib>

namespace mogp {

static thread_local std::string g_err;
void set_error(const std::string& msg) { g_err = msg; }
int hip_fail(hipError_t e, const char* what, const char* file, int line) {
    g_err = std::string("HIP error '") + hipGetErrorString(e) + "' in " + what + " (" + file + ":" + std::to_string(line) + ")";
    return MOGP_EHIP;
}
int launch_potrf_trtri_tile(double* A, int64_t ld, int t, double* invd, double* logdet, unsigned long long* info, hipStream_t s,
                            long long info_base = 0, int store_L = 0);

int fail(int code, const std::string& msg) { g_err = msg; return code; }

int sort_inputs(const double* X, int64_t M, int D, int C, int64_t pad_to, SortedX& o) {
    o.M = M;
    o.Mpad = round_up(std::max<int64_t>(M, 1), pad_to);
    o.perm.resize(M);
    o.off.assign(C + 1, 0);
// ... 534 lines not shown
    for (int c = 0; c < C; ++c) {
        const double* tab = m->table.data() + (size_t)(c * C + c) * m->T * W;
        for (int pos = pts.off[c]; pos < pts.off[c + 1]; ++pos)
            for (int t = 0; t < m->T; ++t) {
                const double* r = tab + (size_t)t * W;
                double arg = 0.0, ph = r[1], env = 0.0;
                for (int d = 0; d < D; ++d) {
                    arg += r[2 + d] * r[2 + 2 * D + d] * r[2 + 2 * D + d];
                    ph += r[2 + D + d] * r[2 + 2 * D + d];
                    const double a = pts.xs[(size_t)d * pts.Mpad + pos] - r[2 + 4 * D + d];
                    env += r[2 + 3 * D + d] * a * a;
                }
                s += r[0] * std::exp(-0.5 * (arg + env)) * std::cos(2.0 * M_PI * ph);
            }
    }
    return s;
}
}

namespace mogp { void one_gpu_call(mogp_model* m) { m->sh_n = 1; m->sh_rank = 0; m->sh_owned = false; } }

namespace mogp { int ensure_system(mogp_model* m) {
    int rc;
    if (m->tiles.empty()) {
        build_sym_tiles(m->sx.off, m->C, m->tiles, m->pair_start);
        if ((rc = m->d_tiles.ensure(m->tiles.size()))) return rc;
        if ((rc = m->d_pair_start.ensure(m->pair_start.size()))) return rc;
        HIP_TRY(dev_upload(m->d_tiles.p, m->tiles.data(), m->tiles.size() * sizeof(GTile)));
        if ((rc = m->strip.build(m->tiles))) return rc;
        for (const GTile& t : m->tiles) (t.c0 < 4 * MOGP_TILE ? m->tiles_head : m->tiles_tail).push_back(t);
        if (!m->tiles_head.empty() && !m->tiles_tail.empty()) {
            if ((rc = m->d_tiles_head.ensure(m->tiles_head.size()))) return rc;
            if ((rc = m->d_tiles_tail.ensure(m->tiles_tail.size()))) return rc;
            HIP_TRY(dev_upload(m->d_tiles_head.p, m->tiles_head.data(), m->tiles_head.size() * sizeof(GTile)));
            HIP_TRY(dev_upload(m->d_tiles_tail.p, m->tiles_tail.data(), m->tiles_tail.size() * sizeof(GTile)));
            if ((rc = m->strip_head.build(m->tiles_head))) return rc;
            if ((rc = m->strip_tail.build(m->tiles_tail))) return rc;
        }
        HIP_TRY(dev_upload(m->d_pair_start.p, m->pair_start.data(), m->pair_start.size() * sizeof(int)));
    }
    if ((rc = m->d_partial.ensure(m->tiles.size() * (size_t)std::max(m->T, 1) * (size_t)std::max(m->Wt, 1)))) return rc;
    if (m->k.Npad == m->Npad) return (m->k.owned_rows && !m->sh_owned) ? spd_make_whole(m->k) : 0;
    return spd_alloc(m->k, m->Npad, m->sh_owned ? m->ctx->device : -1);
} }

extern "C" {

static int ctx_streams(mogp_ctx* ctx) {
    if (ctx->streams_ready) return 0;
    int lo_prio = 0;
    {
        int lo = 0, hi = 0;
        HIP_TRY(hipDeviceGetStreamPriorityRange(&lo, &hi));
        lo_prio = lo;
        HIP_TRY(hipStreamCreateWithPriority(&ctx->st, hipStreamNonBlocking, hi));
        const char* er = std::getenv("MOGP_RESERVE_CUS");
        const int reserve = er ? std::atoi(er) : 2;
        hipDeviceProp_t prop;
        HIP_TRY(hipGetDeviceProperties(&prop, ctx->device));
        const int ncu = prop.multiProcessorCount;
        const bool masked = reserve > 0 && 16 * reserve < ncu;
        ctx->ncu = ncu; ctx->ncu_reserved = masked ? 8 * reserve : 0;
        ctx->chain_ok = !masked || 8 * reserve >= 13;
        if (masked) {
            std::vector<uint32_t> bulk((ncu + 31) / 32, 0u), priv((ncu + 31) / 32, 0u);
            for (int i = 0; i < ncu; ++i) (i < 8 * reserve ? priv : bulk)[i / 32] |= 1u << (i % 32);
            HIP_TRY(hipExtStreamCreateWithCUMask(&ctx->st_priv, (uint32_t)priv.size(), priv.data()));
            HIP_TRY(hipExtStreamCreateWithCUMask(&ctx->st2, (uint32_t)bulk.size(), bulk.data()));
            HIP_TRY(hipExtStreamCreateWithCUMask(&ctx->st3, (uint32_t)bulk.size(), bulk.data()));
            HIP_TRY(hipExtStreamCreateWithCUMask(&ctx->st4, (uint32_t)bulk.size(), bulk.data()));
        } else {
            HIP_TRY(hipStreamCreateWithPriority(&ctx->st2, hipStreamNonBlocking, (lo + hi) / 2));
            HIP_TRY(hipStreamCreateWithPriority(&ctx->st3, hipStreamNonBlocking, lo));
            HIP_TRY(hipStreamCreateWithPriority(&ctx->st4, hipStreamNonBlocking, lo));
        }
    }
    {
        hipDeviceProp_t prop;
        HIP_TRY(hipGetDeviceProperties(&prop, ctx->device));
        std::vector<uint32_t> all((prop.multiProcessorCount + 31) / 32, 0u);
        for (int i = 0; i < prop.multiProcessorCount; ++i) all[i / 32] |= 1u << (i % 32);
        if (ctx->st_priv) HIP_TRY(hipExtStreamCreateWithCUMask(&ctx->st2u, (uint32_t)all.size(), all.data()));
        else HIP_TRY(hipStreamCreateWithPriority(&ctx->st2u, hipStreamNonBlocking, lo_prio));
    }
    ctx->streams_ready = true;
    return 0;
}

int mogp_model_create(mogp_ctx* ctx, int64_t N, int D, int C, const double* X, const double* y, mogp_model** out) {
    if (!ctx || !X || !y || !out) return fail(MOGP_EINVAL, "mogp_model_create: null argument");
    *out = nullptr;
    if (N <= 0 || D <= 0 || D > MOGP_MAXD || C <= 0) return fail(MOGP_EINVAL, "mogp_model_create: need N > 0, 0 < D <= 8, C > 0");
    int rc;
    if ((rc = use_device(ctx))) return rc;
    mogp_model* m = new mogp_model();
    m->ctx = ctx; m->N = N; m->D = D; m->C = C;
    if ((rc = sort_inputs(X, N, D, C, MOGP_TILE, m->sx))) { delete m; return rc; }
    m->Npad = m->sx.Mpad;
    m->nb = (int)(m->Npad / MOGP_TILE);
    const int64_t Npad = m->Npad;
    const int nchunks = (int)((Npad + 511) / 512);
#define TRY_RC(x) do { int r__ = (x); if (r__) { mogp_model_destroy(m); return r__; } } while (0)
#define TRY_HIP(x) do { hipError_t e__ = (x); if (e__ != hipSuccess) { int r__ = hip_fail(e__, #x, __FILE__, __LINE__); mogp_model_destroy(m); return r__; } } while (0)
    TRY_RC(ctx_streams(ctx));
    m->st = ctx->st; m->st2 = ctx->st2; m->st2u = ctx->st2u; m->st3 = ctx->st3; m->st4 = ctx->st4; m->st_priv = ctx->st_priv;
    TRY_RC(m->d_x.ensure((size_t)D * Npad));
    TRY_RC(m->d_y.ensure(Npad));
    TRY_RC(m->d_noise.ensure(C));
    TRY_RC(m->d_z.ensure(Npad));
    TRY_RC(m->d_alpha.ensure((size_t)(1 + nchunks) * Npad));
    TRY_RC(m->d_zz.ensure((Npad + 3) / 4));
    TRY_RC(m->d_diagG.ensure(C));
    TRY_RC(m->d_info.ensure(2));
    TRY_RC(m->d_flag.ensure(1));
    TRY_RC(m->d_chan_off.ensure(C + 1));
    TRY_HIP(dev_upload(m->d_x.p, m->sx.xs.data(), (size_t)D * Npad * sizeof(double)));
    TRY_HIP(dev_upload(m->d_chan_off.p, m->sx.off.data(), (C + 1) * sizeof(int)));
    TRY_RC(mogp_model_set_y(m, y));
#undef TRY_RC
#undef TRY_HIP
    *out = m;
    return MOGP_OK;
}

int mogp_model_destroy(mogp_model* m) {
    if (!m) return MOGP_OK;
    if (m->ctx) { hipError_t e = hipSetDevice(m->ctx->device); (void)e; }
    if (m->st) { hipError_t e = hipStreamSynchronize(m->st); (void)e; }
    for (auto e : m->ev) { hipError_t r = hipEventDestroy(e); (void)r; }
    for (auto e : m->gemm_ev) { hipError_t r = hipEventDestroy(e); (void)r; }
    for (auto& e : m->pred_ev) if (e) { hipError_t r = hipEventDestroy(e); (void)r; e = nullptr; }
    for (hipStream_t q : {m->st2, m->st2u, m->st3, m->st4, m->ctx->st5, m->st_priv}) if (q) { hipError_t e = hipStreamSynchronize(q); (void)e; }
    m->k.release(); m->ws.release(); m->ws_tail.release();
    for (int b = 0; b < 2; ++b) { m->swU[b].release(); m->swUr[b].release(); m->swXr[b].release(); }
    for (auto e : m->sw_ev) { hipError_t r = hipEventDestroy(e); (void)r; }
    for (auto e : m->sh_prof) { hipError_t r = hipEventDestroy(e); (void)r; }
    m->d_symv.release(); m->sh_send.release(); m->sh_recv.release(); m->sh_send1.release(); m->sh_recv1.release(); m->sh_fact.release();
    for (auto e : m->sh_ev) { hipError_t r = hipEventDestroy(e); (void)r; }
    if (m->tw) { m->tw->release(); delete m->tw; m->tw = nullptr; }
    m->oa.release();
    m->loo.release();
    m->cv.release();
    m->d_x.release(); m->d_y.release(); m->d_table.release(); m->d_kind.release(); m->d_shape.release();
    m->d_noise.release(); m->d_dvar.release(); m->d_z.release(); m->d_alpha.release(); m->d_zz.release();
    m->d_partial.release(); m->d_moments.release(); m->d_diagG.release(); m->d_tiles.release(); m->d_pair_start.release(); m->strip.release(); m->strip_own.release();
    m->d_tiles_head.release(); m->d_tiles_tail.release(); m->strip_head.release(); m->strip_tail.release();
    if (m->gram_ev) { hipError_t r = hipEventDestroy(m->gram_ev); (void)r; m->gram_ev = nullptr; }
    if (m->gram_tail_ev) { hipError_t r = hipEventDestroy(m->gram_tail_ev); (void)r; m->gram_tail_ev = nullptr; }
    m->d_chan_off.release(); m->d_flag.release(); m->d_info.release(); m->d_pivots.release(); m->acc_rhs.release();
    m->d_xs.release(); m->d_Ksf.release(); m->d_Vt.release(); m->d_mu.release(); m->d_var.release(); m->d_kdiag.release();
    m->d_Kss.release(); m->d_parts.release(); m->d_ptiles.release(); m->d_pred_tasks.release();
    m->ph_xx.release(); m->ph_sx.release(); m->ph_ss.release();
    if (m->h_pin) { hipError_t e = hipHostFree(m->h_pin); (void)e; m->h_pin = nullptr; }
    mean_release(m);

    delete m;
    return MOGP_OK;
}

int mogp_model_set_y(mogp_model* m, const double* y) {
    if (!m || !y) return fail(MOGP_EINVAL, "mogp_model_set_y: null argument");
    int rc;
    if ((rc = use_device(m->ctx))) return rc;
    std::vector<double> ys(m->Npad, 0.0);
    for (int64_t pos = 0; pos < m->N; ++pos) ys[pos] = y[m->sx.perm[pos]];
    if (m->mean_on) {
        HIP_TRY(dev_upload(m->d_y0.p, ys.data(), m->Npad * sizeof(double)));
        m->hy0 = ys;
        m->mean_g_valid = m->mean_g_pending = false;
        return mean_apply(m);
    }
    HIP_TRY(dev_upload(m->d_y.p, ys.data(), m->Npad * sizeof(double)));
    m->hy = ys;
    return MOGP_OK;
}

int mogp_model_set_terms_ex(mogp_model* m, int T, int width, const double* table) {
    if (!m || !table || T <= 0) return fail(MOGP_EINVAL, "mogp_model_set_terms: bad argument");
    if (width != 2 + 3 * m->D && width != 2 + 5 * m->D) return fail(MOGP_EINVAL, "mogp_model_set_terms: the row width must be 2 + 3 D or 2 + 5 D");
    int rc;
    if ((rc = use_device(m->ctx))) return rc;
    const int W = width;
    const size_t n = (size_t)m->C * m->C * T * W;
    for (size_t i = 0; i < n; ++i)
        if (!std::isfinite(table[i])) return fail(MOGP_ENONFINITE, "spectral term table has non-finite entries (kernel parameters diverged)");
    if (T != m->T) { m->radial = m->point_kinds = false; m->gate_kinds = 0; }
    m->T = T;
    m->Wt = W;
    if (m->tw) m->tw->pred_valid = false;
    m->table.assign(table, table + n);
    if ((rc = m->d_table.ensure(n))) return rc;
    if ((rc = m->d_moments.ensure((size_t)(m->C * (m->C + 1) / 2) * T * W))) return rc;
    HIP_TRY(hipMemcpyAsync(m->d_table.p, m->table.data(), n * sizeof(double), hipMemcpyHostToDevice, m->st));
    return MOGP_OK;
}

int mogp_model_set_terms(mogp_model* m, int T, const double* table) {
    if (!m) return fail(MOGP_EINVAL, "mogp_model_set_terms: bad argument");
    return mogp_model_set_terms_ex(m, T, 2 + 3 * m->D, table);
}

int mogp_model_set_kinds(mogp_model* m, int T, const int* kind, const double* shape) {
    if (!m) return fail(MOGP_EINVAL, "mogp_model_set_kinds: model is null");
    if (T != m->T || T <= 0) return fail(MOGP_EINVAL, "mogp_model_set_kinds: T must be that of the last mogp_model_set_terms");
    const size_t n = (size_t)m->C * m->C * T;
    bool any = false;
    if (const char* bad = check_kinds(kind, shape, m->C, m->D, T, &any)) return fail(MOGP_EINVAL, std::string("mogp_model_set_kinds: ") + bad);
    m->radial = false; m->point_kinds = false; m->gate_kinds = 0;
    if (!any) return MOGP_OK;
    if (m->Wt != 2 + 3 * m->D) return fail(MOGP_EINVAL, "mogp_model_set_kinds: radial profiles do not combine with enveloped term rows");
    m->hkind.assign(kind, kind + n);
    m->hshape.assign(shape, shape + n);
    for (size_t i = 0; i < n; ++i) {
        const int k = kind[i] & MOGP_KIND_MASK;
        m->point_kinds |= k == MOGP_KIND_DOT || k == MOGP_KIND_GATE || k == MOGP_KIND_WDOT;
    }
    m->gate_kinds = extra_rows(kind, n);
    int rc;
    if ((rc = use_device(m->ctx))) return rc;
    if ((rc = m->d_kind.ensure(n))) return rc;
    if ((rc = m->d_shape.ensure(n))) return rc;
    HIP_TRY(hipMemcpyAsync(m->d_kind.p, kind, n * sizeof(int), hipMemcpyHostToDevice, m->st));
    HIP_TRY(hipMemcpyAsync(m->d_shape.p, shape, n * sizeof(double), hipMemcpyHostToDevice, m->st));
    m->radial = true;
    return MOGP_OK;
}

int mogp_model_set_point_diag(mogp_model* m, const double* kdiag) {
    if (!m) return fail(MOGP_EINVAL, "mogp_model_set_point_diag: model is null");
    m->point_diag.clear();
    if (kdiag) {
        m->point_diag.resize(m->N);
        for (int64_t pos = 0; pos < m->N; ++pos) m->point_diag[pos] = kdiag[m->sx.perm[pos]];
    }
    return MOGP_OK;
}

int mogp_gram(mogp_ctx* ctx, int C, int D, int T, const double* table, int64_t M1, const double* X1,
              int64_t M2, const double* X2, double* K_out) {
    return mogp_gram_ex(ctx, C, D, T, 2 + 3 * D, table, M1, X1, M2, X2, K_out);
}

int mogp_gram_ex(mogp_ctx* ctx, int C, int D, int T, int width, const double* table, int64_t M1, const double* X1,
                 int64_t M2, const double* X2, double* K_out) {
    return mogp_gram_kinds(ctx, C, D, T, width, table, nullptr, nullptr, M1, X1, M2, X2, K_out);
}

int mogp_gram_kinds(mogp_ctx* ctx, int C, int D, int T, int width, const double* table, const int* kind, const double* shape,
                    int64_t M1, const double* X1, int64_t M2, const double* X2, double* K_out) {
    if (!ctx || !table || !X1 || !K_out || M1 <= 0 || T <= 0 || C <= 0 || D <= 0 || D > MOGP_MAXD || (width != 2 + 3 * D && width != 2 + 5 * D))
        return fail(MOGP_EINVAL, "mogp_gram: bad argument");
    bool radial = false;
    if (const char* bad = check_kinds(kind, shape, C, D, T, &radial)) return fail(MOGP_EINVAL, std::string("mogp_gram_kinds: ") + bad);
    if (radial && width != 2 + 3 * D) return fail(MOGP_EINVAL, "mogp_gram_kinds: kinds need shapes and rows of width 2 + 3 D");
    int rc;
    if ((rc = use_device(ctx))) return rc;
    const bool sym = (X2 == nullptr);
    SortedX s1, s2;
    if ((rc = sort_inputs(X1, M1, D, C, 1, s1))) return rc;
    if (!sym && (rc = sort_inputs(X2, M2, D, C, 1, s2))) return rc;
    const SortedX& sc = sym ? s1 : s2;
    const int64_t R = s1.M, Cc = sc.M;
    std::vector<GTile> tiles;
    std::vector<int> ps;
    if (sym) build_sym_tiles(s1.off, C, tiles, ps); else build_rect_tiles(s1.off, s2.off, C, tiles);
    const int W = width;
    DevBuf<double> dx1, dx2, dtab, dout;
    DevBuf<GTile> dt;
    DevBuf<int> dkind;
    DevBuf<double> dshape;
    PhaseWs ph;
    auto cleanup = [&]() { dx1.release(); dx2.release(); dtab.release(); dout.release(); dt.release(); dkind.release(); dshape.release(); ph.release(); };
#define G_TRY(x) do { int r__ = (x); if (r__) { cleanup(); return r__; } } while (0)
#define G_HIP(x) do { hipError_t e__ = (x); if (e__ != hipSuccess) { cleanup(); return hip_fail(e__, #x, __FILE__, __LINE__); } } while (0)
    G_TRY(dx1.ensure((size_t)D * s1.Mpad));
    G_TRY(dtab.ensure((size_t)C * C * T * W));
    G_TRY(dout.ensure((size_t)R * Cc));
    G_TRY(dt.ensure(std::max<size_t>(tiles.size(), 1)));
    G_HIP(dev_upload(dx1.p, s1.xs.data(), (size_t)D * s1.Mpad * sizeof(double)));
    if (!sym) {
        G_TRY(dx2.ensure((size_t)D * s2.Mpad));
        G_HIP(dev_upload(dx2.p, s2.xs.data(), (size_t)D * s2.Mpad * sizeof(double)));
    }
    G_HIP(dev_upload(dtab.p, table, (size_t)C * C * T * W * sizeof(double)));
    G_HIP(dev_upload(dt.p, tiles.data(), tiles.size() * sizeof(GTile)));
    GramArgs ga{};
    ga.tiles = dt.p; ga.xr = dx1.p; ga.ldxr = s1.Mpad; ga.xc = sym ? dx1.p : dx2.p; ga.ldxc = sc.Mpad; ga.nrows = R; ga.ncols = Cc;
    G_TRY(ph.prepare(s1.off, sc.off, C, T, s1.Mpad, sc.Mpad, nullptr, ga.ph));
    ga.table = dtab.p; ga.T = T; ga.D = D; ga.C = C; ga.W = W; ga.out = dout.p; ga.ldo = Cc;
    ga.noise = nullptr; ga.dvar = nullptr; ga.jitter_abs = 0.0; ga.mirror = 1;
    if (radial) {
        G_TRY(dkind.ensure((size_t)C * C * T));
        G_TRY(dshape.ensure((size_t)C * C * T));
        G_HIP(dev_upload(dkind.p, kind, (size_t)C * C * T * sizeof(int)));
        G_HIP(dev_upload(dshape.p, shape, (size_t)C * C * T * sizeof(double)));
        ga.kind = dkind.p; ga.shape = dshape.p;
    }
    G_TRY(launch_gram(ga, (int)tiles.size(), nullptr, radial ? extra_rows(kind, (size_t)C * C * T) : 0));
    G_HIP(hipDeviceSynchronize());
    if (s1.identity && sc.identity) {
        G_HIP(hipMemcpy(K_out, dout.p, (size_t)R * Cc * sizeof(double), hipMemcpyDeviceToHost));
    } else {
        std::vector<double> h((size_t)R * Cc);
        G_HIP(hipMemcpy(h.data(), dout.p, h.size() * sizeof(double), hipMemcpyDeviceToHost));
        for (int64_t a = 0; a < R; ++a)
            for (int64_t b = 0; b < Cc; ++b) K_out[s1.perm[a] * Cc + sc.perm[b]] = h[(size_t)a * Cc + b];
    }
    cleanup();
#undef G_TRY
#undef G_HIP
    return MOGP_OK;
}

int mogp_model_work_bytes(mogp_model* m, int64_t* backed, int64_t* whole) {
    if (!m || !backed || !whole) return fail(MOGP_EINVAL, "mogp_model_work_bytes: bad argument");
    const int64_t one = (int64_t)m->k.Npad * m->k.Npad * (int64_t)sizeof(double);
    *whole = one;
    *backed = m->k.Npad == 0 ? 0 : (m->k.owned_rows || m->k.Arows.base ? (int64_t)m->k.Arows.backed_bytes() : one);
    return MOGP_OK;
}

int mogp_model_set_accurate(mogp_model* m, int on) {
    if (!m) return fail(MOGP_EINVAL, "mogp_model_set_accurate: model is null");
    m->accurate = on != 0;
    return MOGP_OK;
}

int mogp_model_pivot_range(mogp_model* m, double* lmin, double* lmax) {
    if (!m || !lmin || !lmax) return fail(MOGP_EINVAL, "mogp_model_pivot_range: bad argument");
    *lmin = m->pivot_min; *lmax = m->pivot_max;
    return MOGP_OK;
}

int mogp_model_inverse_fraction(mogp_model* m, double* fraction) {
    if (!m || !fraction) return fail(MOGP_EINVAL, "mogp_model_inverse_fraction: bad argument");
    *fraction = m->kinv_sparse ? m->kinv_fraction : 1.0;
    return MOGP_OK;
}

int mogp_model_schedule(mogp_model* m, int* flags) {
    if (!m || !flags) return fail(MOGP_EINVAL, "mogp_model_schedule: null argument");
    *flags = (m->k.flow_used ? MOGP_SCHED_DATAFLOW : 0) | (chain_enabled(m) ? MOGP_SCHED_CHAIN_KERNEL : 0) |
             (m->no_flow ? MOGP_SCHED_DATAFLOW_FELL_BACK : 0) | (m->no_chain ? MOGP_SCHED_CHAIN_FELL_BACK : 0) |
             (std::min(m->flow_timeouts, 0xffff) << MOGP_SCHED_TIMEOUTS_SHIFT);
    return MOGP_OK;
}

int mogp_model_flow_replay(mogp_model* m, int on) {
// ... 119 lines not shown
```

### mogptk_amd/csrc/mogp_internal.h

```cpp
#pragma once
#include <hip/hip_runtime.h>
#include <stdint.h>
#include <atomic>
#include <string>
#include <vector>

#define MOGP_TILE 128
#define MOGP_GT 64
#define MOGP_TC 8
#define MOGP_MAXD 8

#define MOGP_KIND_GAUSS 0
#define MOGP_KIND_RQ 1
#define MOGP_KIND_MATERN12 2
#define MOGP_KIND_MATERN32 3
#define MOGP_KIND_MATERN52 4
#ifndef MOGP_KIND_PERIODIC
#define MOGP_KIND_PERIODIC 5
#endif
#ifndef MOGP_KIND_SINC
#define MOGP_KIND_SINC 6
#define MOGP_KIND_DOT 7
#define MOGP_DOT_DEGREE_MAX 8
#endif
#ifndef MOGP_KIND_GATE
#define MOGP_KIND_GATE 8
#endif
#ifndef MOGP_KIND_WDOT
#define MOGP_KIND_WDOT 9
#define MOGP_KIND_WHITE 10
#endif
#ifndef MOGP_KIND_TIMES
#define MOGP_KIND_TIMES (1 << 8)
#endif
#define MOGP_KIND_MASK 0xff
#define MOGP_GROUP_MAX 4

namespace mogp {
const char* check_kinds(const int* kind, const double* shape, int C, int D, int T, bool* any);
}

namespace mogp {

void set_error(const std::string& msg);
int hip_fail(hipError_t e, const char* what, const char* file, int line);
#define HIP_TRY(x)                                                        \
    do {                                                                  \
        hipError_t e__ = (x);                                             \
        if (e__ != hipSuccess) return mogp::hip_fail(e__, #x, __FILE__, __LINE__); \
    } while (0)

inline int set_max_dynamic_lds(const void* fn, int bytes, std::atomic<unsigned long long>& done) {
    int dev = 0;
    HIP_TRY(hipGetDevice(&dev));
    const unsigned long long bit = 1ull << (dev & 63);
    if (done.load(std::memory_order_acquire) & bit) return 0;
    HIP_TRY(hipFuncSetAttribute(fn, hipFuncAttributeMaxDynamicSharedMemorySize, bytes));
    done.fetch_or(bit, std::memory_order_release);
    return 0;
}

struct GTile {
    int r0, c0;
    int nr, nc;
    int pair;
    int flags;
    int rb, cb;
};
struct GSeg { int r0, c0, n, pair; int diag, pad[3]; };
enum { GT_MIRROR = 1,
       GT_DIAG = 2 };

struct PhaseRef {
    const int* offr = nullptr;
    const int* offc = nullptr;
    double* ws = nullptr;
};
size_t phase_ws_doubles(int C, int T, int64_t ldr, int64_t ldc);

struct GramArgs {
    const GTile* tiles;
    const double* xr;
    const double* xc;
    int64_t ldxr, ldxc;
    int64_t nrows, ncols;
    PhaseRef ph;
    const double* table;
    int T, D, C;
    int W;
    double* out;
    int64_t ldo;
    double* out2;
    const double* noise;
    const double* dvar;
    double jitter_abs;
    int mirror;
    hipEvent_t ev0, ev1;
    const GSeg* segs; int nsegs;
    const GTile* rest; int nrest;
    int dbg;
    int tab_lds;
    int phases_ready;
    const int* kind;
    const double* shape;
};

struct MomentArgs {
    const GTile* tiles;
    int ntiles;
    const double* x;
    int64_t ldx;
    const double* xc;
    int64_t ldxc;
    int64_t nrows, ncols;
    PhaseRef ph;
    const double* table;
    int T, D, C;
    int W;
    const double* kinv;
    int64_t ld;
    const double* alpha;
    double kinv_sign;
    int row_mod, row_rem;
    const double* G;
    int64_t ldg;
    const double* ru;
    const double* rw;
    double rcoef;
    int sym;
    double* gzr;
    double* gzc;
    int64_t ldgz;
    double* gzp;
    int nrb, ncb;
    const int* rblk;
    const int* cblk;
    double* partial;
    hipEvent_t ev0, ev1;
    int tab_lds;
    int phases_ready;
    const int* kind;
    const double* shape;
};

int launch_gram(const GramArgs& a, int ntiles, hipStream_t s, int rows = 0);
int launch_gram_dx(const GramArgs& a, int ntiles, int64_t dstride, hipStream_t s);
int launch_gram_dxdx(const GramArgs& a, int ntiles, int64_t bstride, hipStream_t s);
void split_strip_tiles(const std::vector<GTile>& tiles, int maxrun, std::vector<GSeg>& segs, std::vector<GTile>& rest);
int launch_moments(const MomentArgs& a, hipStream_t s, int rows = 0);
inline int extra_rows(const int* kind, size_t n) {
    int rows = 0;
    for (size_t i = 0; i < n; ++i) {
        const int k = kind[i] & MOGP_KIND_MASK;
        if (k == MOGP_KIND_WDOT || k == MOGP_KIND_WHITE) return 2;
        if (k == MOGP_KIND_GATE) rows = 1;
    }
    return rows;
}
inline size_t gz_scratch_doubles(int nrb, int ncb, int D) { return (size_t)2 * nrb * ncb * D * MOGP_GT; }
void tile_blocks(const std::vector<int>& off, int C, std::vector<int>& blk);
int launch_moment_reduce(const double* partial, const int* pair_start, int npairs, int T, int W, int D, double* out, hipStream_t s,
                         int lower_pairs = 1);
int launch_diagG(const double* kinv, int64_t ld, const double* alpha, const int* chan_off, int C, double* out, hipStream_t s,
                 double kinv_sign = 1.0, int row_mod = 0, int row_rem = 0);

enum GemmMode { GM_RECT = 0,
                GM_LOWER = 1,
                GM_LAUUM = 2,
                GM_KHI_J = 3,
                GM_TASKS = 4,
                GM_RECT_LOWER = 5,
                GM_KHI_I = 6,
                GM_KLO_J = 7,
                GM_KLO_I = 8 };

struct GemmTask {
    int64_t a_off, b_off, c_off;
    int kt;
    int pad;
};

struct GemmArgs {
    const double* A; int64_t lda; int a_kmajor;
    const double* B; int64_t ldb; int b_kmajor;
    double* C; int64_t ldc;
    double alpha, beta;
    int mode, mt, nt, K;
    const GemmTask* tasks; int ntasks;
    int task_chunked;
    int small;
    int beta0_from;
    int ksplit; int64_t c_split;
    int ksplit_xcd;
    int col_major;
    int row_mod, row_rem, row_off, row_shift;
    int sk_hint;
    int sk_spans;
    double* sk_ws;
    unsigned* sk_flags;
    unsigned sk_epoch;
    unsigned long long* sk_info;
    unsigned* fl_flags; int fl_nwait; unsigned fl_widx[4]; unsigned fl_wval[4];
    int fl_wt, fl_sig; unsigned fl_sig_base; int fl_sig_shift; unsigned* fl_err; unsigned fl_spins; unsigned* fl_diag;
};
int launch_gemm(const GemmArgs& a, hipStream_t s);
double gemm_flops(const GemmArgs& a, const std::vector<GemmTask>* host_tasks);

int launch_potrf_tile(double* A, int64_t ld, int t, double* logdet, unsigned long long* info, hipStream_t s);
int launch_trtri_tiles(const double* A, int64_t ld, int t0, int nt, double* invd, hipStream_t s);
int launch_put_diag_tiles(double* A, int64_t ld, int nt, const double* invd, hipStream_t s);
int launch_wkk(const double* Ablk, int64_t ld, const double* invd, int nk, double* Wk, int64_t ldw, hipStream_t s);
#define MOGP_CHAIN_FLAGS 32
#define MOGP_INFO_CHAIN_TIMEOUT 0ull
struct ChainFlow {
    unsigned* wait_flag; unsigned wait_val;
    unsigned* done_flag;
    int write_through;
    unsigned long long* trace;
    unsigned* diag;
};
int launch_chain(double* A, int64_t ld, int t0, int nk, double* invd, double* logdet, unsigned long long* info, long long info_base,
                 double* Wk, int64_t ldw, unsigned* flags, unsigned* err, hipStream_t s, const ChainFlow* flow = nullptr);

#define FLOW_MAXQ 48
#define FLOW_NCAS 1
#define FLOW_TRACE_W 6
#define FLOW_POST_W 96
#define FLOW_KEY_STEP 1024
#define FLOW_NOSIG 0xffffffffu
struct FlowTask {
    uint16_t ar, ac, br, bc, cr, cc;
    uint8_t abuf, bbuf, cbuf, var;
    uint16_t kt, ndep;
    uint32_t dep[4];
    uint16_t need[4];
    uint32_t sig[2];
    uint32_t key;
    uint32_t pad[2];
};
static_assert(sizeof(FlowTask) == 64, "FlowTask layout");
enum { FLOW_DIAG_DEEP = 0, FLOW_DIAG_HEAD_STALE = 1, FLOW_DIAG_DEP_STALE = 2, FLOW_DIAG_WAIT_DEEP = 3, FLOW_DIAG_WAIT_STALE = 4, FLOW_DIAG_LAST = 5, FLOW_DIAG_WORDS = 8 };
struct FlowPlan {
    int nb = 0, ob = 0, nouter = 0, nq = 0, rhs_nt = 0;
    bool replay = false;
    std::vector<FlowTask> tasks;
    std::vector<FlowTask> folded;
    int qbase[FLOW_MAXQ] = {0}, qsize[FLOW_MAXQ] = {0};
    int nflags = 0, base_heads = 0, base_err = 0;
    struct Chain { uint32_t done_idx, expect; int t1_nwait; uint32_t t1_widx[4], t1_wval[4], t1_sig_base, t1_sig_per_row; uint32_t t2_widx, t2_wval; };
    std::vector<Chain> chain;
    double flops = 0.0;
};
void flow_build(int nb, int ob, FlowPlan& p, int rhs_nt = 0, bool replay = false);
int launch_pad_identity(double* A, int64_t ld, int64_t N, int64_t Npad, hipStream_t s);
int launch_trmv_lower(const double* W, int64_t ld, int64_t n, const double* y, double* z, double* zz_partial, hipStream_t s,
                      int row_mod = 0, int row_rem = 0);
int launch_trmv_lower_t(const double* W, int64_t ld, int64_t n, const double* z, double* a, hipStream_t s, int row_mod = 0, int row_rem = 0);
int launch_gemv_rows(const double* M, int64_t ld, int64_t rows, int64_t n, const double* v, double* out, hipStream_t s);
int launch_row_sqnorm_sub(const double* M, int64_t ld, int64_t rows, int64_t n, const double* base, double* out, hipStream_t s);
int launch_symv_lower(const double* A, int64_t ld, int64_t n, const double* y, double* out, double* scratch, double sign, hipStream_t s,
                      int row_mod = 0, int row_rem = 0);
int launch_copy2d(double* dst, int64_t ldd, const double* src, int64_t lds, int64_t rows, int64_t cols, double scale, hipStream_t s);
int launch_add_diag(double* A, int64_t ld, int64_t n, double val, hipStream_t s);
int launch_symmetrize(double* A, int64_t ld, int64_t n, hipStream_t s);
int launch_combine(double* out, const double* P, const double* Q, int64_t ld, int64_t n, double ca, double cp, double cq, hipStream_t s);
int launch_gemv_cols(const double* M, int64_t ld, int64_t rows, int64_t n, const double* v, double* out, double* scratch, hipStream_t s);
int launch_get_diag(const double* A, int64_t ld, int64_t n, double* out, hipStream_t s);
int launch_axpby(int64_t n, double a, const double* x, double b, const double* y, double* out, hipStream_t s);
int launch_sum_slices(const double* slices, int64_t n, int ks, double* out, hipStream_t s);
int launch_info_rearm(unsigned long long* info, hipStream_t s);
int launch_info_stash(unsigned long long* info, hipStream_t s);
int launch_nonfinite_scan(const double* A, int64_t ld, int64_t n, int* flag, hipStream_t s);
int launch_pivot_range(const double* invd, int64_t n, double* out, hipStream_t s);

}
```

### mogptk_amd/csrc/mogp_model.h

```cpp
#pragma once
#include "../../include/mogp_hip.h"
#include "mogp_internal.h"

#include <algorithm>
#include <cmath>
#include <cstring>
#include <string>
#include <map>
#include <vector>

namespace mogp {

inline int dev_fill_zero(void* p, size_t bytes) {
    HIP_TRY(hipMemset(p, 0, bytes));
    HIP_TRY(hipStreamSynchronize(nullptr));
    return 0;
}

inline hipError_t dev_upload(void* dst, const void* src, size_t bytes) {
    hipError_t e = hipMemcpy(dst, src, bytes, hipMemcpyHostToDevice);
    return e != hipSuccess ? e : hipStreamSynchronize(nullptr);
}

template <typename T>
struct DevBuf {
    T* p = nullptr;
    size_t n = 0;
    bool borrowed = false;
    int ensure(size_t count) {
        if (count <= n) return 0;
        if (borrowed) { set_error("DevBuf: a borrowed range cannot grow"); return -1; }
        if (p) { hipError_t e = hipFree(p); (void)e; p = nullptr; n = 0; }
        HIP_TRY(hipMalloc(reinterpret_cast<void**>(&p), count * sizeof(T)));
        n = count;
        return 0;
    }
    void release() { if (p && !borrowed) { hipError_t e = hipFree(p); (void)e; } p = nullptr; n = 0; borrowed = false; }
};

struct RowBacked {
    static constexpr size_t GRAN = (size_t)2 << 20;
    char* base = nullptr;
    size_t bytes = 0, gran = GRAN;
    int device = 0;
    std::vector<hipMemGenericAllocationHandle_t> handle;
    std::vector<char> have;
    size_t nbacked = 0;
    int reserve(size_t nbytes, int dev) {
        release();
        bytes = (nbytes + gran - 1) / gran * gran;
        void* q = nullptr;
        HIP_TRY(hipMemAddressReserve(&q, bytes, gran, nullptr, 0));
        base = static_cast<char*>(q); device = dev;
        have.assign(bytes / gran, 0);
        handle.resize(bytes / gran);
        return 0;
    }
    int back(size_t off, size_t len) {
        if (len == 0) return 0;
        if (!base || off + len > bytes) { set_error("RowBacked::back: outside the reserved range"); return -1; }
        const size_t g_lo = off / gran, g_hi = (off + len - 1) / gran;
        hipMemAllocationProp prop{};
        prop.type = hipMemAllocationTypePinned; prop.location.type = hipMemLocationTypeDevice; prop.location.id = device;
        hipMemAccessDesc acc{};
        acc.location.type = hipMemLocationTypeDevice; acc.location.id = device; acc.flags = hipMemAccessFlagsProtReadWrite;
        for (size_t g = g_lo; g <= g_hi;) {
            if (have[g]) { ++g; continue; }
            size_t e = g;
            for (; e <= g_hi && !have[e]; ++e) {
                HIP_TRY(hipMemCreate(&handle[e], gran, &prop, 0));
                hipError_t me = hipMemMap(base + e * gran, gran, 0, handle[e], 0);
                if (me == hipSuccess) me = hipMemSetAccess(base + e * gran, gran, &acc, 1);
                if (me != hipSuccess) { hipError_t x = hipMemUnmap(base + e * gran, gran); x = hipMemRelease(handle[e]); (void)x; HIP_TRY(me); }
                have[e] = 1; ++nbacked;
            }
            { int z__ = dev_fill_zero(base + g * gran, (e - g) * gran); if (z__) return z__; }
            g = e;
        }
        return 0;
    }
    size_t backed_bytes() const { return nbacked * gran; }
    void release() {
        for (size_t g = 0; g < have.size(); ++g)
            if (have[g]) {
                hipError_t e = hipMemUnmap(base + g * gran, gran); (void)e;
                e = hipMemRelease(handle[g]); (void)e;
            }
        have.clear(); handle.clear(); nbacked = 0;
        if (base) { hipError_t e = hipMemAddressFree(base, bytes); (void)e; }
        base = nullptr; bytes = 0;
    }
};

struct PhaseWs {
    DevBuf<double> ws;
    DevBuf<int> offr, offc;
    std::vector<int> hr, hc;
    int prepare(const std::vector<int>& r, const std::vector<int>& c, int C, int T, int64_t ldr, int64_t ldc, hipStream_t s, PhaseRef& out) {
        int rc;
        if ((rc = ws.ensure(phase_ws_doubles(C, T, ldr, ldc)))) return rc;
        if (hr != r) {
            if ((rc = offr.ensure(r.size()))) return rc;
            hr = r;
            HIP_TRY(hipMemcpyAsync(offr.p, hr.data(), hr.size() * sizeof(int), hipMemcpyHostToDevice, s));
        }
        if (hc != c) {
            if ((rc = offc.ensure(c.size()))) return rc;
            hc = c;
            HIP_TRY(hipMemcpyAsync(offc.p, hc.data(), hc.size() * sizeof(int), hipMemcpyHostToDevice, s));
        }
        out.offr = offr.p; out.offc = offc.p; out.ws = ws.p;
        return 0;
    }
    void release() { ws.release(); offr.release(); offc.release(); hr.clear(); hc.clear(); }
};

struct SortedX {
    int64_t M = 0, Mpad = 0;
    std::vector<int64_t> perm;
    std::vector<int> off;
    std::vector<double> xs;
    bool identity = true;
};


int fail(int code, const std::string& msg);
static inline int64_t round_up(int64_t v, int64_t m) { return (v + m - 1) / m * m; }
int sort_inputs(const double* X, int64_t M, int D, int C, int64_t pad_to, SortedX& o);
void build_sym_tiles(const std::vector<int>& off, int C, std::vector<GTile>& tiles, std::vector<int>& pair_start);
void build_rect_tiles(const std::vector<int>& offr, const std::vector<int>& offc, int C, std::vector<GTile>& tiles,
                      std::vector<int>* pair_start = nullptr);

}

using namespace mogp;

enum { MOGP_COMM_NONE = 0, MOGP_COMM_RCCL = 1, MOGP_COMM_EXTERNAL = 2 };
struct mogp_comm {
    int kind = MOGP_COMM_NONE, rank = 0, n = 1;
    void* nccl = nullptr;
    mogp_allgather_cb allgather = nullptr;
    mogp_allreduce_cb allreduce = nullptr;
    void* user = nullptr;
};

struct mogp_ctx {
    int device = 0;
    mogp_comm comm;
    std::string name;
    hipStream_t st = nullptr, st2 = nullptr, st3 = nullptr, st4 = nullptr, st5 = nullptr, st_priv = nullptr, st2u = nullptr;
    bool streams_ready = false;
    bool chain_ok = true;
    struct SkWs { DevBuf<double> ws; DevBuf<unsigned> flags; unsigned epoch = 0; };
    std::map<hipStream_t, SkWs> sk;
    int ncu = 0, ncu_reserved = 0;
};

struct TrtriLevel {
    std::vector<GemmTask> h1, h2;
    DevBuf<GemmTask> d1, d2;
    double flops1 = 0, flops2 = 0;
};

#define MOGP_CHAIN_BOUND_TILES 160
#define MOGP_OUTER 4
#define MOGP_NPANEL 4
struct Spd {
    int64_t Npad = 0;
    int nb = 0;
    bool keep_L = false;
    bool refine_panels = false;
    DevBuf<double> pscr;
    DevBuf<double> A, B, invd, logdet;
    RowBacked Arows;
    bool owned_rows = false;
    DevBuf<double> Wm;
    std::vector<TrtriLevel> levels;
    std::vector<hipEvent_t> sync_ev;
    std::vector<hipEvent_t> row_ev;
    bool want_row_ev = false;
    std::vector<hipEvent_t> inv_ev;
    hipEvent_t fused_last_inv = nullptr, fused_last_wt = nullptr;
    DevBuf<double> Wd;
    DevBuf<double> Pb[MOGP_NPANEL];
    DevBuf<unsigned> chain_flags;
    DevBuf<double> Lm, Wt;
    FlowPlan flow;
    DevBuf<FlowTask> flow_tasks;
    DevBuf<int> flow_qmeta;
    FlowPlan flow_replay;
    DevBuf<FlowTask> flow_tasks_replay;
    DevBuf<int> flow_qmeta_replay;
    FlowPlan flow_rhs;
    DevBuf<FlowTask> flow_tasks_rhs;
    DevBuf<int> flow_qmeta_rhs;
    const FlowPlan* flow_cur = nullptr;
    DevBuf<unsigned> flow_flags;
    DevBuf<char> flow_args;
    std::vector<char> flow_args_h;
    DevBuf<unsigned char> flow_done;
    DevBuf<unsigned> flow_post;
    DevBuf<unsigned> flow_diag;
    DevBuf<unsigned long long> flow_trace;
    hipEvent_t tail_ready = nullptr;
    bool flow_used = false;
    bool want_vec = false, vec_done = false;
    const double* vec_y = nullptr; double* vec_z = nullptr; double* vec_zz = nullptr; double* vec_part = nullptr;
    void release() {
        for (auto& lv : levels) { lv.d1.release(); lv.d2.release(); }
        for (auto e : sync_ev) { hipError_t r = hipEventDestroy(e); (void)r; }
        for (auto e : row_ev) { hipError_t r = hipEventDestroy(e); (void)r; }
        row_ev.clear();
        for (auto e : inv_ev) { hipError_t r = hipEventDestroy(e); (void)r; }
        inv_ev.clear(); Wm.release(); Wd.release(); chain_flags.release(); for (auto& b : Pb) b.release();
        Lm.release(); Wt.release(); flow_tasks.release(); flow_qmeta.release(); flow_flags.release(); flow_args.release(); flow_args_h.clear(); flow_diag.release(); flow_post.release(); flow_done.release(); flow_trace.release(); flow = FlowPlan();
        flow_tasks_rhs.release(); flow_qmeta_rhs.release(); flow_rhs = FlowPlan(); flow_cur = nullptr;
        flow_tasks_replay.release(); flow_qmeta_replay.release(); flow_replay = FlowPlan();
        levels.clear(); sync_ev.clear();
        A.release(); B.release(); invd.release(); logdet.release(); pscr.release();
        Arows.release(); owned_rows = false;
    }
};

struct StripTiles {
    std::vector<mogp::GSeg> segs;
    std::vector<mogp::GTile> rest;
    mogp::DevBuf<mogp::GSeg> d_segs;
    mogp::DevBuf<mogp::GTile> d_rest;
    int build(const std::vector<mogp::GTile>& tiles);
    void attach(mogp::GramArgs& ga) const { ga.segs = d_segs.p; ga.nsegs = (int)segs.size(); ga.rest = d_rest.p; ga.nrest = (int)rest.size(); }
    void release() { d_segs.release(); d_rest.release(); }
};

struct TitsiasWork {
    int64_t Mpad = 0;
    int64_t Mrows = 0;
    Spd a, q;
    DevBuf<double> zx, B, v, GB, Qs, E, R, T1, GA, Hm;
    DevBuf<double> vec, scratch, gz, partial_uu, partial_uf, mom_uu, mom_uf, zero_noise;
    DevBuf<GTile> tiles_uu, tiles_uf;
    DevBuf<int> ps_uu, ps_uf;
    StripTiles strip_uf;
    std::vector<int> tile_key;
    size_t n_tuu = 0, n_tuf = 0;
    DevBuf<double> Kus, Aus, Bus;
    DevBuf<double> zero_col;
    DevBuf<double> kslices;
    DevBuf<double> red;
    const double* Wq = nullptr;
    SortedX pred_ss;
    bool pred_valid = false;
    hipEvent_t side_ev[2] = {nullptr, nullptr};
    DevBuf<int> blk_z, blk_x;
    std::vector<int> hblk_z, hblk_x;
    DevBuf<double> gzp;
    SortedX sv_sz; bool sv_dense = false, sv_valid = false;
    DevBuf<double> kd_point;
    DevBuf<double> nvec;
    PhaseWs ph_zz, ph_zx, ph_zs;
    void release() {
        ph_zz.release(); ph_zx.release(); ph_zs.release();
        a.release(); q.release();
        zx.release(); B.release(); v.release(); GB.release(); Qs.release(); E.release(); R.release(); T1.release(); GA.release(); Hm.release();
        vec.release(); scratch.release(); gz.release(); partial_uu.release(); partial_uf.release(); mom_uu.release(); mom_uf.release();
        zero_noise.release(); tiles_uu.release(); tiles_uf.release(); ps_uu.release(); ps_uf.release(); strip_uf.release(); tile_key.clear();
        Kus.release(); Aus.release(); Bus.release(); zero_col.release(); kslices.release(); nvec.release(); kd_point.release(); red.release();
        blk_z.release(); blk_x.release(); gzp.release(); hblk_z.clear(); hblk_x.clear();
        for (auto& e : side_ev) if (e) { hipError_t r = hipEventDestroy(e); (void)r; e = nullptr; }
    }
};

struct OaWork {
    mogp::DevBuf<double> K, Sc, Y, vec;
    bool valid = false;
    void release() { K.release(); Sc.release(); Y.release(); vec.release(); valid = false; }
};

struct LooWork {
    mogp::DevBuf<double> G, vec;
    void release() { G.release(); vec.release(); }
};

struct CvWork {
    mogp::DevBuf<int> off, idx;
    mogp::DevBuf<long long> foff;
    mogp::DevBuf<double> fac;
    std::vector<int> label;
    int64_t nfolds = 0;
    int mmax = 0;
    size_t fac_doubles = 0;
    hipEvent_t ev[4] = {nullptr, nullptr, nullptr, nullptr};
    bool timed = false;
    void release() {
        off.release(); idx.release(); foff.release(); fac.release(); label.clear(); nfolds = 0; mmax = 0; fac_doubles = 0;
        for (auto& e : ev) if (e) { hipError_t r = hipEventDestroy(e); (void)r; e = nullptr; }
        timed = false;
    }
};

struct FlowRhs { double* T; double* X; int nt; hipEvent_t ready; };
struct mogp_model {
    mogp_ctx* ctx = nullptr;
    int64_t N = 0, Npad = 0;
    int nb = 0, D = 0, C = 0, T = 0;
    int Wt = 0;
    std::vector<double> point_diag;
    SortedX sx;
    std::vector<GTile> tiles;
    std::vector<int> pair_start;
    std::vector<double> table;
    int gate_kinds = 0;
    bool radial = false;
    mogp::DevBuf<int> d_kind;
    std::vector<int> hkind;
    mogp::DevBuf<double> d_shape;
    std::vector<double> hshape;
    bool point_kinds = false;
    hipStream_t st = nullptr;
    hipStream_t st2 = nullptr;
    hipStream_t st2u = nullptr;
    hipStream_t st3 = nullptr;
    hipStream_t st4 = nullptr;
    hipStream_t st_priv = nullptr;
    Spd k;
    Spd ws, ws_tail;
    DevBuf<double> swU[2], swUr[2];
    DevBuf<double> swXr[2];
    std::vector<hipEvent_t> sw_ev;
    int sh_rank = 0, sh_n = 1;
    bool sh_owned = false;
    int backed_rank = -1, backed_n = 0;
    std::vector<GTile> tiles_own;
    std::vector<int> pair_start_own;
    DevBuf<GTile> d_tiles_own;
    bool factor_only = false;
    hipEvent_t pred_ev[2] = {nullptr, nullptr};
    StripTiles strip, strip_own;
    std::vector<GTile> tiles_head, tiles_tail;
    DevBuf<GTile> d_tiles_head, d_tiles_tail;
    StripTiles strip_head, strip_tail;
    hipEvent_t gram_ev = nullptr, gram_tail_ev = nullptr;
    DevBuf<int> d_pair_start_own;
    int own_rank = -1, own_n = 0;
    DevBuf<double> sh_send, sh_recv;
    DevBuf<double> sh_send1, sh_recv1;
    DevBuf<double> sh_fact;
    bool sh_factor_once = false;
    bool sh_split = false;
    std::vector<hipEvent_t> sh_ev;
    std::vector<hipEvent_t> sh_prof;
    double sh_ms[6] = {0, 0, 0, 0, 0, 0};
    int sh_prof_blocks = 0;
    double sh_jabs = 0.0;
    bool sh_dvar = false;

    std::vector<double> hy;
    DevBuf<double> d_symv;
    DevBuf<double> d_x, d_y, d_table, d_noise, d_dvar, d_z, d_alpha, d_zz, d_partial, d_moments, d_diagG;
    DevBuf<GTile> d_tiles;
    std::vector<GemmTask> kinv_acc_tasks, kinv_lauum_tasks;
    std::vector<int> kinv_prefix;
    DevBuf<GemmTask> d_kinv_acc, d_kinv_lauum;
    std::vector<double> blk_cen, blk_half;
    bool kinv_sparse = false;
    double kinv_fraction = 1.0;
    DevBuf<int> d_pair_start, d_chan_off, d_flag;
    DevBuf<double> d_pivots;
    bool accurate = false, accurate_ran = false;
    DevBuf<double> acc_rhs;
    double pivot_min = 0.0, pivot_max = 0.0;
    DevBuf<unsigned long long> d_info;

    DevBuf<double> d_xs, d_Ksf, d_Vt, d_mu, d_var, d_kdiag, d_Kss;
    DevBuf<double> d_parts;
    DevBuf<GTile> d_ptiles;
    DevBuf<GemmTask> d_pred_tasks;
    PhaseWs ph_xx, ph_sx, ph_ss;

    double* h_pin = nullptr;
    size_t h_pin_n = 0;

    bool profiling = false;
    std::vector<hipEvent_t> ev;
    std::vector<hipEvent_t> gemm_ev;
    size_t gemm_ev_used = 0;
    double ms[MOGP_ST_COUNT] = {0};
    int64_t gemm_launches = 0;
    double gemm_flops = 0.0;
    bool have_W = false, have_Kinv = false, kinv_in_A = false, w_in_Wm = false;
    bool flow_ran = false;
    const FlowRhs* rhs_job = nullptr;
    bool replay_flow = false;
    bool no_flow = false;
    long long n_fact = 0, flow_retry_at = 0;
    int flow_backoff = 64, flow_timeouts = 0;
    double flow_enqueue_us = 0.0, flow_enqueue_us_max = 0.0;
    bool no_chain = false;
    TitsiasWork* tw = nullptr;
    OaWork oa;
    LooWork loo;
    CvWork cv;

    bool mean_on = false, mean_g_valid = false, mean_g_pending = false;
    std::vector<double> mean_coef, mean_g, hy0;
    DevBuf<double> d_y0, d_mean_coef, d_mean_part, d_mean_g;
    double* h_mean_pin = nullptr;
    hipEvent_t mean_ev = nullptr;
    const double* mean_w = nullptr;
    double mean_w_scale = 0.0;
};


namespace mogp {
int use_device(mogp_ctx* c);
int gemm_call(mogp_model* m, const GemmArgs& g, double flops, hipStream_t st = nullptr);
int mark(mogp_model* m, int idx);
double table_diag(const mogp_model* m, int c);
double table_diag_points(const mogp_model* m, const SortedX& pts);
int mean_apply(mogp_model* m);
int mean_grad_enqueue(mogp_model* m, const double* w, double scale);
void mean_grad_collect(mogp_model* m);
void mean_release(mogp_model* m);
int spd_alloc(Spd& w, int64_t Npad, int owned_rows_device = -1);
int spd_make_whole(Spd& w);
inline GemmArgs make_gemm(const double* A, int64_t lda, int akm, const double* B, int64_t ldb, int bkm, double* C, int64_t ldc,
                          double alpha, int mode, int mt, int nt, int64_t K) {
    GemmArgs g{};
    g.A = A; g.lda = lda; g.a_kmajor = akm; g.B = B; g.ldb = ldb; g.b_kmajor = bkm; g.C = C; g.ldc = ldc;
    g.alpha = alpha; g.beta = 0.0; g.mode = mode; g.mt = mt; g.nt = nt; g.K = (int)K;
    return g;
}
int side_fork(mogp_model* m, TitsiasWork& t, hipStream_t* side);
int side_join(mogp_model* m, TitsiasWork& t, hipStream_t side);
int gz_prepare(mogp_model* m, TitsiasWork& t, const std::vector<int>& offz, int D);
void gz_attach(const TitsiasWork& t, MomentArgs& ma, bool zx);
int spd_check_info(mogp_model* m, const char* which, int64_t* info);
int spd_info_verdict(mogp_model* m, const char* which, unsigned long long hinfo, int64_t* info);
int sparse_timeout_check(mogp_model* m);
bool chain_enabled(const mogp_model* m);
int chain_fallback(mogp_model* m);
int spd_invert(mogp_model* m, Spd& w, const char* which, int64_t* info, const double** W, bool defer_check = false);
int mm_lower_splitk(mogp_model* m, TitsiasWork& t, const double* A, const double* B, double* out, int mt, int64_t Mpad, int64_t ldk, int64_t K,
                    double alpha = 1.0);
int launch_scale_cols(const double* in, double* out, int64_t ld, int64_t rows, int64_t n, const double* s, hipStream_t st);
int sparse_workspace(mogp_model* m, TitsiasWork& t, int64_t Mpad, int64_t M);
int sparse_tiles(mogp_model* m, TitsiasWork& t, const SortedX& sz, bool want_uf);
int sparse_kuu(mogp_model* m, int64_t M, const double* Z, double jitter, bool want_uf, SortedX& sz, double* jit, const char* need_grouped = nullptr);
int sparse_kuf(mogp_model* m, TitsiasWork& t, const SortedX& sz, hipStream_t stream, bool use_strips, double* out2);
int refined_apply(mogp_model* m, TitsiasWork& t, const double* P, const double* Q, const double* rhs, double* out);
int allreduce_vec_scalars(mogp_model* m, TitsiasWork& t, double* vec, int64_t n, double* hs, int k);
int adjoint_GA(mogp_model* m, TitsiasWork& t, double scale, hipStream_t stream);
int solve_with_rider(mogp_model* m, TitsiasWork& t, double* panel, const double* r, double* beta);
struct MomentSpec { const double* G; int64_t ldg; const double* ru; const double* rw; double rcoef; bool dz; };
int sparse_moments(mogp_model* m, TitsiasWork& t, const SortedX& sz, const MomentSpec* uf, const MomentSpec& uu, bool sharded, hipStream_t side);
int sparse_predict_panels(mogp_model* m, TitsiasWork& t, const SortedX& sz, int64_t S, const double* Xs, SortedX& ss);
int sparse_point_stats(mogp_model* m, TitsiasWork& t, const SortedX& pts, const double* a, const double* b, const double* mu_panel,
                       const double* mu_vec, double mu_div, const double* kdiag, double* mu, double* var);
int sparse_predict_finish(mogp_model* m, TitsiasWork& t, const SortedX& ss, const double* mu_panel, const double* mu_vec, double mu_div,
                          const double* kss_diag, double* mu, double* var);
#define MOGP_RETRY_NO_CHAIN 0x7e7e
int begin_call(mogp_model* m, int64_t* info, bool one_gpu);
int exact_begin(mogp_model* m, const double* noise_var, const double* data_var, double jitter, GramArgs& ga, double& jabs);
int report_not_pd(unsigned long long hinfo, int64_t* info);
struct TestSide { SortedX ss; int64_t Spad = 0; int ntiles = 0; };
int test_side(mogp_model* m, int64_t S, const double* Xs, const double* kss_diag, int64_t extra_rows, hipStream_t st, TestSide& ts, GramArgs& ga, int R = 1, bool point_diag = false);
inline void scatter_by_perm(const SortedX& ss, const double* sorted, double* out) { for (int64_t pos = 0; pos < ss.M; ++pos) out[ss.perm[pos]] = sorted[pos]; }
int moment_pass_device(mogp_model* m, const double* kinv, double ksign);
int moment_pass(mogp_model* m, const double* kinv, double ksign, double* moments, double* diagG);
void collect_timing(mogp_model* m, int last_mark);
enum { LOO_MU = 0, LOO_VAR, LOO_A, LOO_B, LOO_SA, LOO_TERM, LOO_RHO, LOO_SUM, LOO_COUNT };
int loo_workspace(mogp_model* m, bool grad);
int held_out_points(mogp_model* m, double* kinv, bool folds, bool grad);
int held_out_adjoint(mogp_model* m, const double* kinv, double* scratch, bool folds);
int loo_moment_pass(mogp_model* m);
int cv_workspace(mogp_model* m, const int32_t* fold, int64_t nfolds, bool grad);
int cv_folds(mogp_model* m, const double* kinv, const double* y, bool grad);
int cv_fill_S(mogp_model* m, const double* kinv, double* scratch);
size_t cv_bytes(const mogp_model* m);
int eval_sweep(mogp_model* m, const double* noise_var, const double* data_var, double jitter, double* lml, double* jitter_abs, int64_t* info);
void one_gpu_call(mogp_model* m);
int ensure_system(mogp_model* m);
int spd_potrf(mogp_model* m, Spd& w, long long info_base = 0);
int spd_potri_fused(mogp_model* m, Spd& w);
bool flow_enabled(const mogp_model* m, const Spd& w);
int launch_flow_alpha_sum(const Spd& w, double* alpha, hipStream_t st);
int spd_potri_flow(mogp_model* m, Spd& w, const FlowRhs* rhs = nullptr);
void flow_debug_dump(mogp_model* m);
int spd_potri_fused_finish(mogp_model* m, Spd& w);
int spd_trtri(mogp_model* m, Spd& w);
int spd_lauum(mogp_model* m, Spd& w);
int spd_sweep(mogp_model* m, Spd& w);
int sweep_prepare(mogp_model* m, Spd& w);
int sweep_nblocks(const Spd& w);
int sweep_block(mogp_model* m, Spd& w, int kb, hipEvent_t* prof = nullptr, hipEvent_t panel_ready = nullptr, hipEvent_t* stall = nullptr);
int sweep_finish(mogp_model* m, Spd& w);
int trsm_lower(mogp_model* m, const double* L, int64_t ldl, int nb, double* B, int64_t ldb, int64_t ncols, bool trans, hipStream_t st = nullptr, bool tri = false,
               const hipEvent_t* row_ready = nullptr);
int launch_transpose(double* dst, const double* src, int64_t ld, int64_t n, hipStream_t s);
int launch_sym_lower_avg(double* A, int64_t ld, int64_t n, double scale, hipStream_t s);
int comm_allgather(mogp_ctx* ctx, const double* send, double* recv, int64_t count, hipStream_t st);
int comm_allreduce(mogp_ctx* ctx, double* buf, int64_t count, hipStream_t st);
int shard_pack(mogp_model* m, Spd& w, int kb, double** send, double** recv, int64_t* count);
int shard_unpack(mogp_model* m, Spd& w, int kb);
int shard_pack_part(mogp_model* m, Spd& w, int kb, int part, DevBuf<double>& sendb, DevBuf<double>& recvb, int64_t* count, hipStream_t st);
int shard_unpack_part(mogp_model* m, Spd& w, int kb, int part, DevBuf<double>& recvb, hipStream_t st);
int shard_factor_bcast(mogp_model* m, Spd& w, Spd& s, int k0, int nk, bool mine, hipStream_t st);
}
```

### mogptk_amd/csrc/step.hip

```cpp
#include "mogp_model.h"

using namespace mogp;

extern "C" {

int mogp_exact_step(mogp_model* m, int C, int Q, int D, int nscale, const double* raw, const int* tkind, const double* lower, const double* upper,
                    const double* beta, const double* threshold, const double* lp, const double* en, double twopi, double phase_scale,
                    const double* data_var, double jitter,
                    const double* counts, const int* trained, double* cons, double* dcons, double* table, double* noise_var, double* moments,
                    double* diagG, double* out5, double* graw, int64_t* info) {
    if (!m || !out5) return fail(MOGP_EINVAL, "mogp_exact_step: null argument");
    if (C != m->C || D != m->D) return fail(MOGP_EINVAL, "mogp_exact_step: C and D must be the model's");
    int rc;
    if ((rc = mogp_mosm_step_forward(C, Q, D, nscale, raw, tkind, lower, upper, beta, threshold, lp, en, twopi, phase_scale, cons, dcons, table, noise_var)))
        return fail(rc, "mogp_exact_step: bad argument (forward)");
    if ((rc = mogp_model_set_terms(m, Q, table))) return rc;
    double lml = 0.0, trG = 0.0, jit = 0.0;
    if ((rc = mogp_exact_eval(m, noise_var, data_var, jitter, MOGP_EVAL_GRAD, &lml, moments, diagG, &trG, &jit, info))) return rc;
    out5[0] = lml; out5[1] = trG; out5[2] = jit;
    out5[3] = m->pivot_min; out5[4] = m->pivot_max;
    if ((rc = mogp_mosm_step_backward(C, Q, D, nscale, cons, dcons, table, moments, diagG, trG, jitter, counts, m->N, twopi, phase_scale, trained, graw)))
        return fail(rc, "mogp_exact_step: bad argument (backward)");
    return MOGP_OK;
}

}
```

Measured before the change: 97.83.

## Trim per-evaluation launch and copy overhead at the step seam

Adds a lean path on single-GPU exact steps. Several memsets and small host-to-device copies (chain flags, flow flags, zz vector, info sentinel) are replaced by one reset kernel issued at step start. The term table and noise variances go up in a single pinned upload. Symmetric phase tables are computed by one fused kernel, with block centres cached. The moment reduce and diagG are fused into one tail kernel that writes straight into mapped pinned host memory, replacing the separate readback. This cuts launch and transfer latency per evaluation, at the cost of more state tracking (armed reset keys, in-flight pinned buffers) and extra fallback paths.

```diff
diff --git a/mogptk_amd/csrc/exact.hip b/mogptk_amd/csrc/exact.hip
--- a/mogptk_amd/csrc/exact.hip
+++ b/mogptk_amd/csrc/exact.hip
@@ -100,6 +100,7 @@
     if (m->h_pin) { hipError_t e = hipHostFree(m->h_pin); (void)e; m->h_pin = nullptr; m->h_pin_n = 0; }
     HIP_TRY(hipHostMalloc(reinterpret_cast<void**>(&m->h_pin), n * sizeof(double), hipHostMallocDefault));
     m->h_pin_n = n;
+    HIP_TRY(hipHostGetDevicePointer(reinterpret_cast<void**>(&m->d_pin), m->h_pin, 0));
     return 0;
 }
 struct PinLayout {
@@ -113,8 +114,30 @@
 };
 
 namespace mogp {
+bool lean_seam() {
+    const char* e = std::getenv("MOGP_LEAN_SEAM");
+    return !(e && std::atoi(e) == 0);
+}
+
+int seam_reset(mogp_model* m) {
+    Spd& w = m->k;
+    mogp_model::ResetKey key;
+    if (w.flow_cur == &w.flow && w.flow.nflags > 0 && w.flow_flags.p && w.chain_flags.p && m->d_zz.p && !m->replay_flow) {
+        key.cf = w.chain_flags.p; key.ncf = (size_t)(w.flow.nouter + 1) * MOGP_CHAIN_FLAGS;
+        key.ff = w.flow_flags.p; key.nff = (size_t)w.flow.nflags;
+        key.zz = m->d_zz.p; key.nzz = (size_t)((w.Npad + 3) / 4);
+        if (key.ncf > w.chain_flags.n || key.nff > w.flow_flags.n || key.nzz > m->d_zz.n) key = mogp_model::ResetKey();
+    }
+    int rc;
+    if ((rc = launch_seam_reset(w.chain_flags.p, key.ncf, w.flow_flags.p, key.nff, m->d_zz.p, key.nzz, m->d_info.p, m->st))) return rc;
+    m->reset_key = key;
+    m->reset_armed = true;
+    return 0;
+}
+
 int begin_call(mogp_model* m, int64_t* info, bool one_gpu) {
     m->mean_w = nullptr;
+    m->lean = false; m->reset_armed = false;
     if (int rc = use_device(m->ctx)) return rc;
     if (info) *info = 0;
     if (one_gpu) one_gpu_call(m);
@@ -146,18 +169,49 @@
         HIP_TRY(hipMemcpyAsync(m->d_dvar.p, dv.data(), Npad * sizeof(double), hipMemcpyHostToDevice, m->st));
     }
     jabs = jitter * dsum / (double)N;
-    HIP_TRY(hipMemcpyAsync(m->d_noise.p, noise_var, C * sizeof(double), hipMemcpyHostToDevice, m->st));
-    static const unsigned long long big = std::numeric_limits<unsigned long long>::max();
-    HIP_TRY(hipMemcpyAsync(m->d_info.p, &big, sizeof(big), hipMemcpyHostToDevice, m->st));
     int rc;
+    const double* d_noise = m->d_noise.p;
+    if (m->lean) {
+        const size_t n = m->table.size();
+        if (m->d_table.n < n + (size_t)C) return fail(MOGP_EINVAL, "exact_begin: the term table on the device has no room for the noise variances");
+        if (m->h_par_n < n + (size_t)C) {
+            if (m->h_par) { HIP_TRY(hipStreamSynchronize(m->st)); hipError_t e = hipHostFree(m->h_par); (void)e; m->h_par = nullptr; m->h_par_n = 0; }
+            HIP_TRY(hipHostMalloc(reinterpret_cast<void**>(&m->h_par), (n + (size_t)C) * sizeof(double), hipHostMallocDefault));
+            m->h_par_n = n + (size_t)C;
+        }
+        if (m->par_in_flight) HIP_TRY(hipStreamSynchronize(m->st));
+        std::memcpy(m->h_par + n, noise_var, C * sizeof(double));
+        m->par_in_flight = true;
+        if (m->table_pending) {
+            std::memcpy(m->h_par, m->table.data(), n * sizeof(double));
+            HIP_TRY(hipMemcpyAsync(m->d_table.p, m->h_par, (n + (size_t)C) * sizeof(double), hipMemcpyHostToDevice, m->st));
+            m->table_pending = false;
+        } else
+            HIP_TRY(hipMemcpyAsync(m->d_table.p + n, m->h_par + n, C * sizeof(double), hipMemcpyHostToDevice, m->st));
+        d_noise = m->d_table.p + n;
+        if (!m->reset_armed && (rc = seam_reset(m))) return rc;
+    } else {
+        if (m->table_pending) {
+            HIP_TRY(hipMemcpyAsync(m->d_table.p, m->table.data(), m->table.size() * sizeof(double), hipMemcpyHostToDevice, m->st));
+            m->table_pending = false;
+        }
+        HIP_TRY(hipMemcpyAsync(m->d_noise.p, noise_var, C * sizeof(double), hipMemcpyHostToDevice, m->st));
+        static const unsigned long long big = std::numeric_limits<unsigned long long>::max();
+        HIP_TRY(hipMemcpyAsync(m->d_info.p, &big, sizeof(big), hipMemcpyHostToDevice, m->st));
+    }
     if ((rc = mark(m, 0))) return rc;
     ga = GramArgs{};
     ga.tiles = m->d_tiles.p; ga.xr = m->d_x.p; ga.xc = m->d_x.p; ga.ldxr = ga.ldxc = Npad; ga.nrows = ga.ncols = N;
     if ((rc = m->ph_xx.prepare(m->sx.off, m->sx.off, C, m->T, Npad, Npad, m->st, ga.ph))) return rc;
     ga.table = m->d_table.p; ga.T = m->T; ga.D = m->D; ga.C = C; ga.W = m->Wt;
-    ga.out = m->k.A.p; ga.ldo = Npad; ga.noise = m->d_noise.p; ga.dvar = data_var ? m->d_dvar.p : nullptr;
+    ga.out = m->k.A.p; ga.ldo = Npad; ga.noise = d_noise; ga.dvar = data_var ? m->d_dvar.p : nullptr;
     ga.jitter_abs = jabs; ga.mirror = 0;
     if (m->radial) { ga.kind = m->d_kind.p; ga.shape = m->d_shape.p; }
+    if (m->lean && m->ph_xx.symmetric(Npad, Npad)) {
+        const bool centres = m->ph_xx.centres_missing(m->d_x.p, Npad, C, m->T, m->D);
+        if ((rc = launch_phase_tables_sym(ga.ph, m->d_x.p, Npad, N, m->d_table.p, m->T, m->D, C, m->Wt, centres, m->st))) return rc;
+        ga.phases_ready = 1;
+    }
     return 0;
 }
 }
@@ -347,8 +401,10 @@
         HIP_TRY(hipMemcpyAsync(m->h_pin + pl.zz + o, m->d_zz.p + o, std::min(zz_piece, nzz - o) * sizeof(double), hipMemcpyDeviceToHost, m->st));
     HIP_TRY(hipMemcpyAsync(m->h_pin + pl.info, m->d_info.p, sizeof(unsigned long long), hipMemcpyDeviceToHost, m->st));
     if (ga_out) *ga_out = ga;
+    m->reset_armed = false;
     if (plan.defer) return 0;
     HIP_TRY(hipStreamSynchronize(m->st));
+    m->par_in_flight = false;
     return factorize_finish(m, ga, lml, info);
 }
 
@@ -372,7 +428,7 @@
     m->ms[MOGP_ST_GEMM_KERNEL] = gsum;
 }
 
-int moment_pass_device(mogp_model* m, const double* kinv, double ksign) {
+int moment_pass_device(mogp_model* m, const double* kinv, double ksign, double* pin_mom, double* pin_dg) {
     const int C = m->C, D = m->D, W = m->Wt, T = m->T, P = C * (C + 1) / 2;
     const int64_t Npad = m->Npad;
     const int rm = m->sh_n > 1 ? m->sh_n : 0;
@@ -389,8 +445,13 @@
     ma.phases_ready = 1;
     ma.ev0 = prof_event(m, 9); ma.ev1 = prof_event(m, 10);
     if ((rc = launch_moments(ma, m->st, m->radial ? m->gate_kinds : 0))) return rc;
-    if ((rc = launch_moment_reduce(m->d_partial.p, own ? m->d_pair_start_own.p : m->d_pair_start.p, P, T, W, D, m->d_moments.p, m->st))) return rc;
-    if ((rc = launch_diagG(kinv, Npad, m->d_alpha.p, m->d_chan_off.p, C, m->d_diagG.p, m->st, ksign, rm, m->sh_rank))) return rc;
+    if (pin_mom && pin_dg) {
+        if ((rc = launch_moment_tail(m->d_partial.p, own ? m->d_pair_start_own.p : m->d_pair_start.p, P, T, W, D, m->d_moments.p, kinv, Npad, m->d_alpha.p,
+                                     m->d_chan_off.p, C, m->d_diagG.p, ksign, rm, m->sh_rank, pin_mom, pin_dg, m->st))) return rc;
+    } else {
+        if ((rc = launch_moment_reduce(m->d_partial.p, own ? m->d_pair_start_own.p : m->d_pair_start.p, P, T, W, D, m->d_moments.p, m->st))) return rc;
+        if ((rc = launch_diagG(kinv, Npad, m->d_alpha.p, m->d_chan_off.p, C, m->d_diagG.p, m->st, ksign, rm, m->sh_rank))) return rc;
+    }
     if ((rc = mean_grad_enqueue(m, m->d_alpha.p, -1.0))) return rc;
     return mark(m, 6);
 }
@@ -539,9 +600,12 @@
                     double* lml, double* moments, double* diagG, double* trG, double* jitter_abs, int64_t* info) {
     if (!m) return fail(MOGP_EINVAL, "mogp_exact_eval: model is null");
     int rc;
+    const bool armed = m->reset_armed;
     if ((rc = begin_call(m, info, true))) return rc;
     const std::string& grad_path = grad_path_env();
     const bool sweep = grad_path == "sweep" && (flags & MOGP_EVAL_GRAD);
+    m->lean = lean_seam() && !sweep && m->ctx->comm.n <= 1;
+    m->reset_armed = armed && m->lean;
     const bool grad = (flags & MOGP_EVAL_GRAD) != 0;
     GramArgs ga{};
     auto again = [&]() { return mogp_exact_eval(m, noise_var, data_var, jitter, flags, lml, moments, diagG, trG, jitter_abs, info); };
@@ -562,9 +626,13 @@
     if (sweep) {
         if ((rc = moment_pass(m, kinv, ksign, moments, diagG))) return rc;
     } else {
-        if ((rc = moment_pass_device(m, kinv, ksign))) return rc;
-        if ((rc = grad_enqueue(m, pl))) return rc;
+        if (m->lean) { if ((rc = moment_pass_device(m, kinv, ksign, m->d_pin + pl.moments, m->d_pin + pl.diagG))) return rc; }
+        else {
+            if ((rc = moment_pass_device(m, kinv, ksign))) return rc;
+            if ((rc = grad_enqueue(m, pl))) return rc;
+        }
         if ((rc = wait_stream(m->st))) return rc;
+        m->par_in_flight = false;
         if ((rc = factorize_finish(m, ga, lml, info))) return retry_on_streams(m, rc, again);
     }
     m->have_Kinv = true;
diff --git a/mogptk_amd/csrc/flow.hip b/mogptk_amd/csrc/flow.hip
--- a/mogptk_amd/csrc/flow.hip
+++ b/mogptk_amd/csrc/flow.hip
@@ -735,15 +735,22 @@
     const FlowPlan& p = plan;
     const int nouter = p.nouter;
     if ((rc = w.chain_flags.ensure((size_t)(nouter + 1) * MOGP_CHAIN_FLAGS))) return rc;
-    HIP_TRY(hipMemsetAsync(w.chain_flags.p, 0, (size_t)(nouter + 1) * MOGP_CHAIN_FLAGS * sizeof(unsigned), crit));
+    const size_t n_cf = (size_t)(nouter + 1) * MOGP_CHAIN_FLAGS, n_zz = (size_t)((ld + 3) / 4);
+    const bool want_zz = !rhs && w.want_vec && w.vec_zz;
+    const mogp_model::ResetKey& rk = m->reset_key;
+    const bool reset_done = m->reset_armed && !rhs && !replay && &w == &m->k && want_zz && rk.cf == w.chain_flags.p && rk.ncf == n_cf &&
+                            rk.ff == w.flow_flags.p && rk.nff == (size_t)p.nflags && rk.zz == w.vec_zz && rk.nzz == n_zz;
+    if (!reset_done) {
+    HIP_TRY(hipMemsetAsync(w.chain_flags.p, 0, n_cf * sizeof(unsigned), crit));
     HIP_TRY(hipMemsetAsync(w.flow_flags.p, 0, (size_t)p.nflags * sizeof(unsigned), crit));
+    }
     if (replay) {
         std::vector<unsigned> preset((size_t)p.nflags, 0u);
         for (const FlowPlan::Chain& c : p.chain) preset[c.done_idx] = c.expect;
         HIP_TRY(hipMemcpyAsync(w.flow_flags.p, preset.data(), preset.size() * sizeof(unsigned), hipMemcpyHostToDevice, crit));
         HIP_TRY(hipStreamSynchronize(crit));
     }
-    if (!rhs && w.want_vec && w.vec_zz) HIP_TRY(hipMemsetAsync(w.vec_zz, 0, (size_t)((ld + 3) / 4) * sizeof(double), crit));
+    if (want_zz && !reset_done) HIP_TRY(hipMemsetAsync(w.vec_zz, 0, n_zz * sizeof(double), crit));
     static const bool want_trace = std::getenv("MOGP_FLOW_TRACE") && std::atoi(std::getenv("MOGP_FLOW_TRACE")) != 0;
     if (want_trace) {
         if ((rc = w.flow_trace.ensure(FLOW_TRACE_W * p.tasks.size() + 4 * (size_t)nouter))) return rc;
diff --git a/mogptk_amd/csrc/gram.hip b/mogptk_amd/csrc/gram.hip
--- a/mogptk_amd/csrc/gram.hip
+++ b/mogptk_amd/csrc/gram.hip
@@ -59,10 +59,9 @@
 struct PhaseArgs {
     const double* x; int64_t ld; const int* off; const double* table; int T, D, C, W, role; double* cs; double* sn;
 };
-__global__ __launch_bounds__(256) void k_phase_table(PhaseArgs a) {
-    const int64_t pt = (int64_t)blockIdx.x * 256 + threadIdx.x;
+__device__ __forceinline__ void phase_table_point(const PhaseArgs& a, int64_t pt, int o, int t) {
     if (pt >= a.off[a.C]) return;
-    const int o = blockIdx.y, t = blockIdx.z, D = a.D, W = a.W;
+    const int D = a.D, W = a.W;
     int c = 0;
     while (pt >= a.off[c + 1]) ++c;
     const int pair = a.role == 0 ? c * a.C + o : o * a.C + c;
@@ -77,6 +76,14 @@
     const size_t idx = ((size_t)o * a.T + t) * a.ld + pt;
     a.cs[idx] = cs;
     a.sn[idx] = sn;
+}
+__global__ __launch_bounds__(256) void k_phase_table(PhaseArgs a) {
+    phase_table_point(a, (int64_t)blockIdx.x * 256 + threadIdx.x, blockIdx.y, blockIdx.z);
+}
+__global__ __launch_bounds__(256) void k_phase_table_sym(PhaseArgs a, double* ccs, double* csn) {
+    int t = blockIdx.z;
+    if (t >= a.T) { t -= a.T; a.role = 1; a.cs = ccs; a.sn = csn; }
+    phase_table_point(a, (int64_t)blockIdx.x * 256 + threadIdx.x, blockIdx.y, t);
 }
 
 struct CentreArgs { const double* x; int64_t ld; const int* off; int C, D; double* cen; double* half; };
@@ -129,6 +136,27 @@
     if (nr > 0) hipLaunchKernelGGL(k_block_centres, dim3((unsigned)((nr + MOGP_GT - 1) / MOGP_GT + C)), dim3(64), 0, s, c);
     c.x = xc; c.ld = ldxc; c.off = ph.offc; c.cen = const_cast<double*>(v.ccen); c.half = const_cast<double*>(v.chalf);
     if (nc > 0) hipLaunchKernelGGL(k_block_centres, dim3((unsigned)((nc + MOGP_GT - 1) / MOGP_GT + C)), dim3(64), 0, s, c);
+    HIP_TRY(hipGetLastError());
+    return 0;
+}
+
+int launch_phase_tables_sym(const PhaseRef& ph, const double* x, int64_t ldx, int64_t n, const double* table, int T, int D, int C, int W, bool centres,
+                            hipStream_t s) {
+    if (!ph.ws || !ph.offr || !ph.offc) { set_error("Gram / moment launch without a phase workspace"); return -1; }
+    if (n <= 0) return 0;
+    const PhaseView v = phase_view(ph.ws, C, T, D, ldx, ldx);
+    PhaseArgs a;
+    a.table = table; a.T = T; a.D = D; a.C = C; a.W = W;
+    a.x = x; a.ld = ldx; a.off = ph.offr; a.role = 0; a.cs = const_cast<double*>(v.rcs); a.sn = const_cast<double*>(v.rsn);
+    hipLaunchKernelGGL(k_phase_table_sym, dim3((unsigned)((n + 255) / 256), C, 2 * T), dim3(256), 0, s, a, const_cast<double*>(v.ccs), const_cast<double*>(v.csn));
+    if (centres) {
+        CentreArgs c;
+        c.C = C; c.D = D; c.x = x; c.ld = ldx; c.off = ph.offr;
+        c.cen = const_cast<double*>(v.rcen); c.half = const_cast<double*>(v.rhalf);
+        hipLaunchKernelGGL(k_block_centres, dim3((unsigned)((n + MOGP_GT - 1) / MOGP_GT + C)), dim3(64), 0, s, c);
+        c.cen = const_cast<double*>(v.ccen); c.half = const_cast<double*>(v.chalf);
+        hipLaunchKernelGGL(k_block_centres, dim3((unsigned)((n + MOGP_GT - 1) / MOGP_GT + C)), dim3(64), 0, s, c);
+    }
     HIP_TRY(hipGetLastError());
     return 0;
 }
@@ -2174,11 +2202,9 @@
     return env ? launch_moments_t<true, false, true>(a, s) : launch_moments_t<true, false, false>(a, s);
 }
 
-__global__ __launch_bounds__(256) void k_moment_reduce(const double* __restrict__ partial, const int* __restrict__ pair_start,
-                                                       int TW, int W, int D, int lower_pairs, double* __restrict__ out) {
-    const int p = blockIdx.x, tw = blockIdx.y;
+__device__ __forceinline__ double moment_reduce_block(const double* __restrict__ partial, const int* __restrict__ pair_start, int p, int tw,
+                                                      int TW, int W, int D, int lower_pairs, double* red) {
     const int b = pair_start[p], e = pair_start[p + 1];
-    __shared__ double red[256];
     double s = 0.0;
     for (int t = b + threadIdx.x; t < e; t += 256) s += partial[(size_t)t * TW + tw];
     red[threadIdx.x] = s;
@@ -2187,16 +2213,24 @@
         if (threadIdx.x < off) red[threadIdx.x] += red[threadIdx.x + off];
         __syncthreads();
     }
+    double v = 0.0;
     if (threadIdx.x == 0) {
         int i = (int)((sqrt(8.0 * (double)p + 1.0) - 1.0) * 0.5);
         while ((i + 1) * (i + 2) / 2 <= p) ++i;
         while (i * (i + 1) / 2 > p) --i;
         const bool diag = lower_pairs && (p - i * (i + 1) / 2) == i;
         const int w = tw % W;
-        double v = red[0];
+        v = red[0];
         if (diag && (w == 1 || (w >= 2 + D && w < 2 + 2 * D))) v = 0.0;
-        out[(size_t)p * TW + tw] = v;
-    }
+    }
+    return v;
+}
+__global__ __launch_bounds__(256) void k_moment_reduce(const double* __restrict__ partial, const int* __restrict__ pair_start,
+                                                       int TW, int W, int D, int lower_pairs, double* __restrict__ out) {
+    const int p = blockIdx.x, tw = blockIdx.y;
+    __shared__ double red[256];
+    const double v = moment_reduce_block(partial, pair_start, p, tw, TW, W, D, lower_pairs, red);
+    if (threadIdx.x == 0) out[(size_t)p * TW + tw] = v;
 }
 
 int launch_moment_reduce(const double* partial, const int* pair_start, int npairs, int T, int W, int D, double* out, hipStream_t s, int lower_pairs) {
@@ -2205,10 +2239,8 @@
     return 0;
 }
 
-__global__ void k_diagG(const double* __restrict__ kinv, int64_t ld, const double* __restrict__ alpha,
-                        const int* __restrict__ chan_off, double* __restrict__ out, double kinv_sign, int row_mod, int row_rem) {
-    const int c = blockIdx.x;
-    __shared__ double red[256];
+__device__ __forceinline__ double diagG_block(const double* __restrict__ kinv, int64_t ld, const double* __restrict__ alpha,
+                                              const int* __restrict__ chan_off, int c, double kinv_sign, int row_mod, int row_rem, double* red) {
     double s = 0.0;
     for (int64_t k = chan_off[c] + threadIdx.x; k < chan_off[c + 1]; k += 256)
         if (row_mod <= 1 || (int)((k / MOGP_TILE) % row_mod) == row_rem) s += 0.5 * (alpha[k] * alpha[k] - kinv_sign * kinv[k * ld + k]);
@@ -2218,7 +2250,14 @@
         if (threadIdx.x < off) red[threadIdx.x] += red[threadIdx.x + off];
         __syncthreads();
     }
-    if (threadIdx.x == 0) out[c] = red[0];
+    return threadIdx.x == 0 ? red[0] : 0.0;
+}
+__global__ void k_diagG(const double* __restrict__ kinv, int64_t ld, const double* __restrict__ alpha,
+                        const int* __restrict__ chan_off, double* __restrict__ out, double kinv_sign, int row_mod, int row_rem) {
+    const int c = blockIdx.x;
+    __shared__ double red[256];
+    const double v = diagG_block(kinv, ld, alpha, chan_off, c, kinv_sign, row_mod, row_rem, red);
+    if (threadIdx.x == 0) out[c] = v;
 }
 
 int launch_diagG(const double* kinv, int64_t ld, const double* alpha, const int* chan_off, int C, double* out, hipStream_t s,
@@ -2228,4 +2267,54 @@
     return 0;
 }
 
-}
+struct TailArgs {
+    const double* partial; const int* pair_start; int npairs, TW, W, D, lower_pairs;
+    const double* kinv; int64_t ld; const double* alpha; const int* chan_off; int C; double kinv_sign; int row_mod, row_rem;
+    double *mom, *dg, *pin_mom, *pin_dg;
+};
+__global__ __launch_bounds__(256) void k_moment_tail(TailArgs a) {
+    __shared__ double red[256];
+    const int b = blockIdx.x, nred = a.npairs * a.TW;
+    if (b < nred) {
+        const int p = b % a.npairs, tw = b / a.npairs;
+        const double v = moment_reduce_block(a.partial, a.pair_start, p, tw, a.TW, a.W, a.D, a.lower_pairs, red);
+        if (threadIdx.x == 0) {
+            a.mom[(size_t)p * a.TW + tw] = v;
+            if (a.pin_mom) { a.pin_mom[(size_t)p * a.TW + tw] = v; __threadfence_system(); }
+        }
+    } else if (b - nred < a.C) {
+        const int c = b - nred;
+        const double v = diagG_block(a.kinv, a.ld, a.alpha, a.chan_off, c, a.kinv_sign, a.row_mod, a.row_rem, red);
+        if (threadIdx.x == 0) {
+            a.dg[c] = v;
+            if (a.pin_dg) { a.pin_dg[c] = v; __threadfence_system(); }
+        }
+    }
+}
+int launch_moment_tail(const double* partial, const int* pair_start, int npairs, int T, int W, int D, double* mom, const double* kinv, int64_t ld,
+                       const double* alpha, const int* chan_off, int C, double* dg, double kinv_sign, int row_mod, int row_rem, double* pin_mom,
+                       double* pin_dg, hipStream_t s) {
+    TailArgs a;
+    a.partial = partial; a.pair_start = pair_start; a.npairs = npairs; a.TW = T * W; a.W = W; a.D = D; a.lower_pairs = 1;
+    a.kinv = kinv; a.ld = ld; a.alpha = alpha; a.chan_off = chan_off; a.C = C; a.kinv_sign = kinv_sign; a.row_mod = row_mod; a.row_rem = row_rem;
+    a.mom = mom; a.dg = dg; a.pin_mom = pin_mom; a.pin_dg = pin_dg;
+    hipLaunchKernelGGL(k_moment_tail, dim3((unsigned)(npairs * T * W + C)), dim3(256), 0, s, a);
+    HIP_TRY(hipGetLastError());
+    return 0;
+}
+
+__global__ __launch_bounds__(256) void k_seam_reset(unsigned* z32, size_t n32, unsigned* z32b, size_t n32b, double* z64, size_t n64, unsigned long long* info) {
+    const size_t i0 = (size_t)blockIdx.x * 256 + threadIdx.x, step = (size_t)gridDim.x * 256;
+    for (size_t i = i0; i < n32; i += step) z32[i] = 0u;
+    for (size_t i = i0; i < n32b; i += step) z32b[i] = 0u;
+    for (size_t i = i0; i < n64; i += step) z64[i] = 0.0;
+    if (i0 == 0 && info) *info = ~0ull;
+}
+int launch_seam_reset(unsigned* z32, size_t n32, unsigned* z32b, size_t n32b, double* z64, size_t n64, unsigned long long* info, hipStream_t s) {
+    const size_t most = std::max(std::max(n32, n32b), std::max(n64, (size_t)1));
+    hipLaunchKernelGGL(k_seam_reset, dim3((unsigned)std::min<size_t>((most + 255) / 256, 64)), dim3(256), 0, s, z32, n32, z32b, n32b, z64, n64, info);
+    HIP_TRY(hipGetLastError());
+    return 0;
+}
+
+}
diff --git a/mogptk_amd/csrc/mogp_api.hip b/mogptk_amd/csrc/mogp_api.hip
--- a/mogptk_amd/csrc/mogp_api.hip
+++ b/mogptk_amd/csrc/mogp_api.hip
@@ -710,6 +710,7 @@
     m->d_Kss.release(); m->d_parts.release(); m->d_ptiles.release(); m->d_pred_tasks.release();
     m->ph_xx.release(); m->ph_sx.release(); m->ph_ss.release();
     if (m->h_pin) { hipError_t e = hipHostFree(m->h_pin); (void)e; m->h_pin = nullptr; }
+    if (m->h_par) { hipError_t e = hipHostFree(m->h_par); (void)e; m->h_par = nullptr; }
     mean_release(m);
 
     delete m;
@@ -733,7 +734,8 @@
     return MOGP_OK;
 }
 
-int mogp_model_set_terms_ex(mogp_model* m, int T, int width, const double* table) {
+}
+namespace mogp { int set_terms_host(mogp_model* m, int T, int width, const double* table, bool upload) {
     if (!m || !table || T <= 0) return fail(MOGP_EINVAL, "mogp_model_set_terms: bad argument");
     if (width != 2 + 3 * m->D && width != 2 + 5 * m->D) return fail(MOGP_EINVAL, "mogp_model_set_terms: the row width must be 2 + 3 D or 2 + 5 D");
     int rc;
@@ -747,11 +749,15 @@
     m->Wt = W;
     if (m->tw) m->tw->pred_valid = false;
     m->table.assign(table, table + n);
-    if ((rc = m->d_table.ensure(n))) return rc;
+    if ((rc = m->d_table.ensure(n + (size_t)m->C))) return rc;
     if ((rc = m->d_moments.ensure((size_t)(m->C * (m->C + 1) / 2) * T * W))) return rc;
-    HIP_TRY(hipMemcpyAsync(m->d_table.p, m->table.data(), n * sizeof(double), hipMemcpyHostToDevice, m->st));
-    return MOGP_OK;
-}
+    m->table_pending = !upload;
+    if (upload) HIP_TRY(hipMemcpyAsync(m->d_table.p, m->table.data(), n * sizeof(double), hipMemcpyHostToDevice, m->st));
+    return MOGP_OK;
+} }
+extern "C" {
+
+int mogp_model_set_terms_ex(mogp_model* m, int T, int width, const double* table) { return set_terms_host(m, T, width, table, true); }
 
 int mogp_model_set_terms(mogp_model* m, int T, const double* table) {
     if (!m) return fail(MOGP_EINVAL, "mogp_model_set_terms: bad argument");
diff --git a/mogptk_amd/csrc/mogp_internal.h b/mogptk_amd/csrc/mogp_internal.h
--- a/mogptk_amd/csrc/mogp_internal.h
+++ b/mogptk_amd/csrc/mogp_internal.h
@@ -163,6 +163,12 @@
                          int lower_pairs = 1);
 int launch_diagG(const double* kinv, int64_t ld, const double* alpha, const int* chan_off, int C, double* out, hipStream_t s,
                  double kinv_sign = 1.0, int row_mod = 0, int row_rem = 0);
+int launch_moment_tail(const double* partial, const int* pair_start, int npairs, int T, int W, int D, double* mom, const double* kinv, int64_t ld,
+                       const double* alpha, const int* chan_off, int C, double* dg, double kinv_sign, int row_mod, int row_rem, double* pin_mom,
+                       double* pin_dg, hipStream_t s);
+int launch_phase_tables_sym(const PhaseRef& ph, const double* x, int64_t ldx, int64_t n, const double* table, int T, int D, int C, int W, bool centres,
+                            hipStream_t s);
+int launch_seam_reset(unsigned* z32, size_t n32, unsigned* z32b, size_t n32b, double* z64, size_t n64, unsigned long long* info, hipStream_t s);
 
 enum GemmMode { GM_RECT = 0,
                 GM_LOWER = 1,
diff --git a/mogptk_amd/csrc/mogp_model.h b/mogptk_amd/csrc/mogp_model.h
--- a/mogptk_amd/csrc/mogp_model.h
+++ b/mogptk_amd/csrc/mogp_model.h
@@ -101,18 +101,27 @@
         if ((rc = ws.ensure(phase_ws_doubles(C, T, ldr, ldc)))) return rc;
         if (hr != r) {
             if ((rc = offr.ensure(r.size()))) return rc;
-            hr = r;
+            hr = r; cen.ws = nullptr;
             HIP_TRY(hipMemcpyAsync(offr.p, hr.data(), hr.size() * sizeof(int), hipMemcpyHostToDevice, s));
         }
         if (hc != c) {
             if ((rc = offc.ensure(c.size()))) return rc;
-            hc = c;
+            hc = c; cen.ws = nullptr;
             HIP_TRY(hipMemcpyAsync(offc.p, hc.data(), hc.size() * sizeof(int), hipMemcpyHostToDevice, s));
         }
         out.offr = offr.p; out.offc = offc.p; out.ws = ws.p;
         return 0;
     }
-    void release() { ws.release(); offr.release(); offc.release(); hr.clear(); hc.clear(); }
+    struct CentreKey { const double* ws; const double* x; int64_t ld; int C, T, D; };
+    CentreKey cen{nullptr, nullptr, 0, 0, 0, 0};
+    bool symmetric(int64_t ldr, int64_t ldc) const { return ldr == ldc && hr == hc; }
+    bool centres_missing(const double* x, int64_t ld, int C, int T, int D) {
+        const CentreKey k{ws.p, x, ld, C, T, D};
+        const bool same = cen.ws == k.ws && cen.x == k.x && cen.ld == k.ld && cen.C == k.C && cen.T == k.T && cen.D == k.D;
+        cen = k;
+        return !same;
+    }
+    void release() { ws.release(); offr.release(); offc.release(); hr.clear(); hc.clear(); cen = CentreKey{nullptr, nullptr, 0, 0, 0, 0}; }
 };
 
 struct SortedX {
@@ -377,6 +386,11 @@
     DevBuf<GemmTask> d_pred_tasks;
     PhaseWs ph_xx, ph_sx, ph_ss;
 
+    bool lean = false, reset_armed = false, table_pending = false, par_in_flight = false;
+    struct ResetKey { const void* cf = nullptr; size_t ncf = 0; const void* ff = nullptr; size_t nff = 0; const void* zz = nullptr; size_t nzz = 0; } reset_key;
+    double* h_par = nullptr; size_t h_par_n = 0;
+    double* d_pin = nullptr;
+
     double* h_pin = nullptr;
     size_t h_pin_n = 0;
 
@@ -460,12 +474,15 @@
                           const double* kss_diag, double* mu, double* var);
 #define MOGP_RETRY_NO_CHAIN 0x7e7e
 int begin_call(mogp_model* m, int64_t* info, bool one_gpu);
+bool lean_seam();
+int seam_reset(mogp_model* m);
+int set_terms_host(mogp_model* m, int T, int width, const double* table, bool upload);
 int exact_begin(mogp_model* m, const double* noise_var, const double* data_var, double jitter, GramArgs& ga, double& jabs);
 int report_not_pd(unsigned long long hinfo, int64_t* info);
 struct TestSide { SortedX ss; int64_t Spad = 0; int ntiles = 0; };
 int test_side(mogp_model* m, int64_t S, const double* Xs, const double* kss_diag, int64_t extra_rows, hipStream_t st, TestSide& ts, GramArgs& ga, int R = 1, bool point_diag = false);
 inline void scatter_by_perm(const SortedX& ss, const double* sorted, double* out) { for (int64_t pos = 0; pos < ss.M; ++pos) out[ss.perm[pos]] = sorted[pos]; }
-int moment_pass_device(mogp_model* m, const double* kinv, double ksign);
+int moment_pass_device(mogp_model* m, const double* kinv, double ksign, double* pin_mom = nullptr, double* pin_dg = nullptr);
 int moment_pass(mogp_model* m, const double* kinv, double ksign, double* moments, double* diagG);
 void collect_timing(mogp_model* m, int last_mark);
 enum { LOO_MU = 0, LOO_VAR, LOO_A, LOO_B, LOO_SA, LOO_TERM, LOO_RHO, LOO_SUM, LOO_COUNT };
diff --git a/mogptk_amd/csrc/step.hip b/mogptk_amd/csrc/step.hip
--- a/mogptk_amd/csrc/step.hip
+++ b/mogptk_amd/csrc/step.hip
@@ -12,11 +12,22 @@
     if (!m || !out5) return fail(MOGP_EINVAL, "mogp_exact_step: null argument");
     if (C != m->C || D != m->D) return fail(MOGP_EINVAL, "mogp_exact_step: C and D must be the model's");
     int rc;
+    const bool lean = lean_seam() && m->ctx->comm.n <= 1;
+    if (lean) {
+        if ((rc = use_device(m->ctx))) return rc;
+        if ((rc = seam_reset(m))) return rc;
+    }
     if ((rc = mogp_mosm_step_forward(C, Q, D, nscale, raw, tkind, lower, upper, beta, threshold, lp, en, twopi, phase_scale, cons, dcons, table, noise_var)))
         return fail(rc, "mogp_exact_step: bad argument (forward)");
-    if ((rc = mogp_model_set_terms(m, Q, table))) return rc;
+    if ((rc = set_terms_host(m, Q, 2 + 3 * m->D, table, !lean))) { m->reset_armed = false; return rc; }
     double lml = 0.0, trG = 0.0, jit = 0.0;
-    if ((rc = mogp_exact_eval(m, noise_var, data_var, jitter, MOGP_EVAL_GRAD, &lml, moments, diagG, &trG, &jit, info))) return rc;
+    rc = mogp_exact_eval(m, noise_var, data_var, jitter, MOGP_EVAL_GRAD, &lml, moments, diagG, &trG, &jit, info);
+    m->reset_armed = false;
+    if (m->table_pending) {
+        m->table_pending = false;
+        HIP_TRY(hipMemcpyAsync(m->d_table.p, m->table.data(), m->table.size() * sizeof(double), hipMemcpyHostToDevice, m->st));
+    }
+    if (rc) return rc;
     out5[0] = lml; out5[1] = trG; out5[2] = jit;
     out5[3] = m->pivot_min; out5[4] = m->pivot_max;
     if ((rc = mogp_mosm_step_backward(C, Q, D, nscale, cons, dcons, table, moments, diagG, trG, jitter, counts, m->N, twopi, phase_scale, trained, graw)))
```

Result: no change. 98.09 (median of 6 runs) (+0.3%).
